# joejep/FOCNeRF

Hardware: AMD Instinct MI355X
Metric: train_samples_per_sec (higher is better)
Workload: dtype f16

## Files before the change

### focnerf_amd/backend.py

```python
import math

import torch

from . import _lib
from ._lib import lib, ptr, stream_of, check, require_cuda, dtype_code, raw_stream


def _f32(*ts):
    for t in ts:
        if t is not None and t.dtype != torch.float32:
            raise RuntimeError(f"focnerf_amd: expected float32 tensor, got {t.dtype}")


def _contig(*ts):
    for t in ts:
        if t is not None and not t.is_contiguous():
            raise RuntimeError("focnerf_amd: tensor must be contiguous")


class _Scratch:

    def __init__(self):
        self._bufs = {}
        self._pinned = []
# ... 66 lines not shown
                                                   ptr(image), stream_of(sigmas)), "composite_rays_train_forward")

    @staticmethod
    def composite_rays_train_backward(grad_weights_sum, grad_image, sigmas, rgbs, deltas, rays, weights_sum, image, M, N, T_thresh, grad_sigmas, grad_rgbs):
        ts = (grad_weights_sum, grad_image, sigmas, rgbs, deltas, weights_sum, image, grad_sigmas, grad_rgbs)
        require_cuda(*ts, rays); _f32(*ts); _contig(*ts, rays)
        check(lib.foc_composite_rays_train_backward(ptr(grad_weights_sum), ptr(grad_image), ptr(sigmas), ptr(rgbs), ptr(deltas), ptr(rays),
                                                    ptr(weights_sum), ptr(image), M, N, T_thresh, ptr(grad_sigmas), ptr(grad_rgbs),
                                                    stream_of(sigmas)), "composite_rays_train_backward")

    @staticmethod
    def march_rays(n_alive, n_step, rays_alive, rays_t, rays_o, rays_d, bound, dt_gamma, max_steps, C, H, grid, nears, fars, xyzs, dirs, deltas, noises):
        ts = (rays_t, rays_o, rays_d, nears, fars, xyzs, dirs, deltas, noises)
        require_cuda(*ts, rays_alive, grid); _f32(*ts); _contig(*ts, rays_alive, grid)
        check(lib.foc_march_rays(n_alive, n_step, ptr(rays_alive), ptr(rays_t), ptr(rays_o), ptr(rays_d), bound, dt_gamma, max_steps, C, H,
                                 ptr(grid), ptr(nears), ptr(fars), ptr(xyzs), ptr(dirs), ptr(deltas), ptr(noises), stream_of(rays_o)), "march_rays")

    @staticmethod
    def composite_rays(n_alive, n_step, T_thresh, rays_alive, rays_t, sigmas, rgbs, deltas, weights_sum, depth, image):
        ts = (rays_t, sigmas, rgbs, deltas, weights_sum, depth, image)
        require_cuda(*ts, rays_alive); _f32(*ts); _contig(*ts, rays_alive)
        check(lib.foc_composite_rays(n_alive, n_step, T_thresh, ptr(rays_alive), ptr(rays_t), ptr(sigmas), ptr(rgbs), ptr(deltas),
                                     ptr(weights_sum), ptr(depth), ptr(image), stream_of(sigmas)), "composite_rays")

    @staticmethod
    def compact_alive(rays_alive, n_alive, out, n_out):
        require_cuda(rays_alive, out, n_out)
        scratch = _scratch.get("compact", 4 * (n_alive // 1024 + 2), rays_alive.device)
        check(lib.foc_compact_alive(ptr(rays_alive), n_alive, ptr(out), ptr(n_out), ptr(scratch), stream_of(rays_alive)), "compact_alive")


class _gridencoder:
    @staticmethod
    def _common(inputs, embeddings, offsets):
        require_cuda(inputs, embeddings, offsets)
        _contig(inputs, embeddings, offsets)
        if inputs.dtype != torch.float32:
            raise RuntimeError("inputs must be a float32 tensor")
        if offsets.dtype != torch.int32:
            raise RuntimeError("offsets must be an int tensor")

    @staticmethod
    def grid_encode_forward(inputs, embeddings, offsets, outputs, B, D, C, L, S, H, dy_dx, gridtype, align_corners, interp, out_bl=False):
        _gridencoder._common(inputs, embeddings, offsets)
        require_cuda(outputs, dy_dx); _contig(outputs, dy_dx)
        dt = dtype_code(embeddings)
        if outputs.dtype != embeddings.dtype or (dy_dx is not None and dy_dx.dtype != embeddings.dtype):
            raise RuntimeError("grid_encode_forward: outputs/dy_dx must share the embeddings dtype")
        fn = lib.foc_grid_encode_forward_bl if out_bl else lib.foc_grid_encode_forward
        check(fn(ptr(inputs), ptr(embeddings), ptr(offsets), ptr(outputs), B, D, C, L, float(S), H, ptr(dy_dx), gridtype, int(bool(align_corners)),
                 interp, dt, None, stream_of(inputs)), "grid_encode_forward")

    @staticmethod
    def planes_to_rows(planes, rows, B, L, unit_bytes):
        require_cuda(planes, rows); _contig(planes, rows)
        check(lib.foc_grid_planes_to_rows(ptr(planes), ptr(rows), B, L, unit_bytes, stream_of(planes)), "grid_planes_to_rows")

    @staticmethod
    def rows_to_planes(rows, planes, B, L, unit_bytes):
        require_cuda(planes, rows); _contig(planes, rows)
        check(lib.foc_grid_rows_to_planes(ptr(rows), ptr(planes), B, L, unit_bytes, stream_of(rows)), "grid_rows_to_planes")

    @staticmethod
    def _host_entry(offsets):
        h = getattr(offsets, "_foc_host", None)
        if h is None or h[0] != offsets._version:
            import ctypes
            arr = offsets.detach().cpu().numpy().astype("int32")
            h = (offsets._version, arr, arr.ctypes.data_as(ctypes.c_void_p), int((arr[1:] - arr[:-1]).max()) if arr.size > 1 else 0)
            offsets._foc_host = h
        return h

    @staticmethod
    def _host_offsets(offsets):
        return _gridencoder._host_entry(offsets)[2]

    @staticmethod
    def _binned_ok(offsets, S, H, L, gridtype):
        finest = math.ceil(2.0 ** (float(S) * (L - 1)) * H - 1.0) + 1
        return gridtype == 0 and finest <= 8190 and _gridencoder._host_entry(offsets)[3] <= 8192 * 64

    _pre = {}

    @staticmethod
    def _pre_state(device):
        idx = device.index if device.index is not None else torch.cuda.current_device()
        st = _gridencoder._pre.get(idx)
        if st is None:
            st = _gridencoder._pre[idx] = dict(ticket=0, key=None)
        return idx, st

    @staticmethod
    def _invalidate_precount(device):
        _, st = _gridencoder._pre_state(device)
        st["ticket"] += 1
        st["key"] = None

    @staticmethod
    def binned_workspace_bytes(offsets, B, D, C, L, S, H, gridtype, dt, count_ahead=False):
        import os
        if os.environ.get("FOCNERF_GRID_ATOMIC", "0") == "1" or (count_ahead and (B == 0 or os.environ.get("FOC_GRID_PRECOUNT", "1") == "0")):
            return 0
        ws_bytes = lib.foc_grid_encode_backward_workspace_bytes(B, D, C, L, dt)
        if not ws_bytes or B * 8 * L >= 2 ** 32 or not _gridencoder._binned_ok(offsets, S, H, L, gridtype):
            return 0
        return ws_bytes

    @staticmethod
    def precount_standalone():
        import os
        return os.environ.get("FOC_GRID_PRECOUNT", "1") == "2"

    @staticmethod
    def _precount_key(inputs, B, L, dt, ws):
        return (inputs.data_ptr(), B, L, dt, ws.data_ptr())

    @staticmethod
    def issue_precount_ticket(inputs, B, L, dt, ws):
        idx, st = _gridencoder._pre_state(inputs.device)
        st["ticket"] += 1
        st["key"] = _gridencoder._precount_key(inputs, B, L, dt, ws)
        return (idx, st["ticket"], st["key"])

    @staticmethod
    def grid_encode_forward_counted(inputs, embeddings, offsets, outputs, B, D, C, L, S, H, gridtype, align_corners, interp, standalone=False):
        _gridencoder._common(inputs, embeddings, offsets)
        require_cuda(outputs); _contig(outputs)
        dt = dtype_code(embeddings)
        ws_bytes = _gridencoder.binned_workspace_bytes(offsets, B, D, C, L, S, H, gridtype, dt, count_ahead=True)
        if not ws_bytes:
            return None
        if outputs.dtype != embeddings.dtype or outputs.numel() != L * B * C:
            raise RuntimeError("grid_encode_forward_counted: outputs must be [L,B,C] of the embeddings' dtype")
        ws = _scratch.get("grid_bwd", ws_bytes, inputs.device)
        host = _gridencoder._host_offsets(offsets)
        if standalone:
            check(lib.foc_grid_encode_backward_count(ptr(inputs), ptr(offsets), B, D, C, L, float(S), H, gridtype, int(bool(align_corners)), interp, dt,
                                                     host, ptr(ws), ws_bytes, stream_of(inputs)), "grid_encode_backward_count")
            check(lib.foc_grid_encode_forward(ptr(inputs), ptr(embeddings), ptr(offsets), ptr(outputs), B, D, C, L, float(S), H, None, gridtype,
                                              int(bool(align_corners)), interp, dt, None, stream_of(inputs)), "grid_encode_forward")
        else:
            check(lib.foc_grid_encode_forward_counted(ptr(inputs), ptr(embeddings), ptr(offsets), ptr(outputs), B, D, C, L, float(S), H, gridtype,
                                                      int(bool(align_corners)), interp, dt, host, ptr(ws), ws_bytes, stream_of(inputs)),
                  "grid_encode_forward_counted")
        return _gridencoder.issue_precount_ticket(inputs, B, L, dt, ws)

    @staticmethod
    def _precount_valid(ticket, inputs, B, L, dt, ws):
        if ticket is None:
            return False
        idx, number, key = ticket
        st = _gridencoder._pre.get(idx)
        return st is not None and st["ticket"] == number and st["key"] == key == _gridencoder._precount_key(inputs, B, L, dt, ws)

    @staticmethod
    def grid_encode_backward(grad, inputs, embeddings, offsets, grad_embeddings, B, D, C, L, S, H, dy_dx, grad_inputs, gridtype, align_corners, interp, grad_bl=False,
                             precount=None):
        _gridencoder._common(inputs, embeddings, offsets)
        require_cuda(grad, grad_embeddings, dy_dx, grad_inputs); _contig(grad, grad_embeddings, dy_dx, grad_inputs)
        dt = dtype_code(grad)
        if grad_embeddings.dtype != grad.dtype:
            raise RuntimeError("grid_encode_backward: grad_embeddings must share grad's dtype")
        ws_bytes = _gridencoder.binned_workspace_bytes(offsets, B, D, C, L, S, H, gridtype, dt)
        if ws_bytes:
            ws = _scratch.get("grid_bwd", ws_bytes, grad.device)
            counted = _gridencoder._precount_valid(precount, inputs, B, L, dt, ws)
            fn = lib.foc_grid_encode_backward_binned_counted if counted else lib.foc_grid_encode_backward_binned
            check(fn(ptr(grad), ptr(inputs), ptr(embeddings), ptr(offsets), ptr(grad_embeddings), B, D, C, L, float(S), H,
                     ptr(dy_dx), ptr(grad_inputs), gridtype, int(bool(align_corners)), interp, dt, int(bool(grad_bl)),
                     _gridencoder._host_offsets(offsets), ptr(ws), ws_bytes, stream_of(inputs)), "grid_encode_backward_binned")
            _gridencoder._invalidate_precount(grad.device)
            return
        check(lib.foc_grid_encode_backward(ptr(grad), ptr(inputs), ptr(embeddings), ptr(offsets), ptr(grad_embeddings), B, D, C, L, float(S), H,
                                           ptr(dy_dx), ptr(grad_inputs), gridtype, int(bool(align_corners)), interp, dt, int(bool(grad_bl)),
                                           None, stream_of(inputs)), "grid_encode_backward")

    @staticmethod
    def grad_total_variation(inputs, embeddings, grad, offsets, weight, B, D, C, L, S, H, gridtype, align_corners):
        require_cuda(inputs, embeddings, grad, offsets); _contig(inputs, embeddings, grad, offsets)
        dt = dtype_code(embeddings)
        if inputs.dtype != embeddings.dtype or grad.dtype != embeddings.dtype:
            raise RuntimeError("grad_total_variation: inputs/grad must share the embeddings dtype")
        check(lib.foc_grad_total_variation(ptr(inputs), ptr(embeddings), ptr(grad), ptr(offsets), weight, B, D, C, L, float(S), H, gridtype,
                                           int(bool(align_corners)), dt, stream_of(inputs)), "grad_total_variation")


class _freqencoder:
    @staticmethod
    def freq_encode_forward(inputs, B, D, deg, C, outputs):
        require_cuda(inputs, outputs); _f32(inputs, outputs); _contig(inputs, outputs)
        check(lib.foc_freq_encode_forward(ptr(inputs), B, D, deg, C, ptr(outputs), stream_of(inputs)), "freq_encode_forward")

    @staticmethod
    def freq_encode_backward(grad, outputs, B, D, deg, C, grad_inputs):
        require_cuda(grad, outputs, grad_inputs); _f32(grad, outputs, grad_inputs); _contig(grad, outputs, grad_inputs)
        check(lib.foc_freq_encode_backward(ptr(grad), ptr(outputs), B, D, deg, C, ptr(grad_inputs), stream_of(grad)), "freq_encode_backward")


def _half(*ts):
    for t in ts:
        if t is not None and t.dtype != torch.float16:
            raise RuntimeError("focnerf_amd: tensor must be a half tensor")


class _ffmlp:
    @staticmethod
    def ffmlp_forward(inputs, weights, B, input_dim, output_dim, hidden_dim, num_layers, activation, output_activation, forward_buffer, outputs):
        require_cuda(inputs, weights, forward_buffer, outputs); _half(inputs, weights, forward_buffer, outputs); _contig(inputs, weights, forward_buffer, outputs)
        check(lib.foc_ffmlp_forward(ptr(inputs), ptr(weights), B, input_dim, output_dim, hidden_dim, num_layers, activation, output_activation,
                                    ptr(forward_buffer), ptr(outputs), stream_of(inputs)), "ffmlp_forward")

    @staticmethod
    def ffmlp_inference(inputs, weights, B, input_dim, output_dim, hidden_dim, num_layers, activation, output_activation, inference_buffer, outputs):
        require_cuda(inputs, weights, outputs); _half(inputs, weights, outputs); _contig(inputs, weights, outputs)
        check(lib.foc_ffmlp_inference(ptr(inputs), ptr(weights), B, input_dim, output_dim, hidden_dim, num_layers, activation, output_activation,
                                      ptr(inference_buffer), ptr(outputs), stream_of(inputs)), "ffmlp_inference")

    @staticmethod
    def ffmlp_backward(grad, inputs, weights, forward_buffer, B, input_dim, output_dim, hidden_dim, num_layers, activation, output_activation,
                       calc_grad_inputs, backward_buffer, grad_inputs, grad_weights):
        ts = (grad, inputs, weights, forward_buffer, backward_buffer, grad_inputs, grad_weights)
        require_cuda(*ts); _half(*ts); _contig(*ts)
        ws_bytes = lib.foc_ffmlp_backward_workspace_bytes(input_dim, hidden_dim, num_layers)
        ws = _scratch.get("ffmlp_ws", ws_bytes, grad.device)
        check(lib.foc_ffmlp_backward(ptr(grad), ptr(inputs), ptr(weights), ptr(forward_buffer), B, input_dim, output_dim, hidden_dim, num_layers,
                                     activation, output_activation, int(bool(calc_grad_inputs)), ptr(backward_buffer), ptr(grad_inputs),
                                     ptr(grad_weights), ptr(ws), ws.numel(), stream_of(grad)), "ffmlp_backward")

    @staticmethod
    def ffmlp_forward_planar(inputs_planar, weights, B, input_dim, output_dim, hidden_dim, num_layers, activation, output_activation, outputs):
        require_cuda(inputs_planar, weights, outputs); _half(inputs_planar, weights, outputs); _contig(inputs_planar, weights, outputs)
        check(lib.foc_ffmlp_forward_planar(ptr(inputs_planar), ptr(weights), B, input_dim, output_dim, hidden_dim, num_layers, activation,
                                           output_activation, ptr(outputs), stream_of(inputs_planar)), "ffmlp_forward_planar")

    @staticmethod
    def ffmlp_backward_planar(grad, inputs_planar, weights, B, input_dim, output_dim, hidden_dim, num_layers, activation, output_activation,
                              calc_grad_inputs, grad_inputs_planar, grad_weights):
        ts = (grad, inputs_planar, weights, grad_inputs_planar, grad_weights)
        require_cuda(*ts); _half(*ts); _contig(*ts)
        ws = _scratch.get("ffmlp_ws", lib.foc_ffmlp_backward_workspace_bytes(input_dim, hidden_dim, num_layers), grad.device)
        check(lib.foc_ffmlp_backward_planar(ptr(grad), ptr(inputs_planar), ptr(weights), B, input_dim, output_dim, hidden_dim, num_layers,
                                            activation, output_activation, int(bool(calc_grad_inputs)), ptr(grad_inputs_planar),
                                            ptr(grad_weights), ptr(ws), ws.numel(), stream_of(grad)), "ffmlp_backward_planar")

    @staticmethod
    def allocate_splitk(size):
        check(lib.foc_allocate_splitk(int(size)), "allocate_splitk")

    @staticmethod
    def free_splitk():
        check(lib.foc_free_splitk(), "free_splitk")
```

### focnerf_amd/csrc/fixedstep.hip

```cpp
#include "common.h"
#include "fs_common.h"
#include <float.h>

__global__ void __launch_bounds__(256) k_fs_sample(const float *__restrict__ rays_o, const float *__restrict__ rays_d, const float *__restrict__ nears,
                                                   const float *__restrict__ fars, const float *__restrict__ aabb, const float *__restrict__ noise,
                                                   uint32_t N, uint32_t T, float bound, float *__restrict__ xyzs, float *__restrict__ enc_in,
                                                   _Float16 *__restrict__ ray_sh, uint32_t ray_block) {
    const uint64_t total = ray_block ? (uint64_t)((N + FS_RAY_BLOCK - 1) / FS_RAY_BLOCK) * FS_RAY_BLOCK * T : (uint64_t)N * T;
    const FsBox box = fs_box(aabb);
    const float two_b = 2 * bound;
    for (uint64_t s = (uint64_t)blockIdx.x * 256 + threadIdx.x; s < total; s += (uint64_t)gridDim.x * 256) {
        uint32_t n, i;
        bool own = true;
        if (ray_block) {
            const uint32_t blk = (uint32_t)(s / ((uint64_t)FS_RAY_BLOCK * T)), in = (uint32_t)(s - (uint64_t)blk * FS_RAY_BLOCK * T);
            i = in / FS_RAY_BLOCK;
            n = blk * FS_RAY_BLOCK + in % FS_RAY_BLOCK;
            own = n < N;
            n = own ? n : N - 1;
        } else {
            n = (uint32_t)(s / T); i = (uint32_t)(s - (uint64_t)n * T);
        }
        const FsGeom g = fs_geom(nears, fars, n, T);
        const float z = fs_z(g, i, T, noise, (uint64_t)n * T + i);
        float x, y, w;
        fs_point(rays_o[n * 3], rays_o[n * 3 + 1], rays_o[n * 3 + 2], rays_d[n * 3], rays_d[n * 3 + 1], rays_d[n * 3 + 2], z, box, x, y, w);
        if (xyzs) { xyzs[s * 3] = x; xyzs[s * 3 + 1] = y; xyzs[s * 3 + 2] = w; }
        if (enc_in) { enc_in[s * 3] = fs_norm(x, bound, two_b); enc_in[s * 3 + 1] = fs_norm(y, bound, two_b); enc_in[s * 3 + 2] = fs_norm(w, bound, two_b); }
        if (ray_sh && i == 0 && own) {
            h8 lo, hi;
            foc_sh16_h(rays_d[n * 3], rays_d[n * 3 + 1], rays_d[n * 3 + 2], lo, hi);
            h8 *dst = reinterpret_cast<h8 *>(ray_sh + (uint64_t)n * 16);
            dst[0] = lo; dst[1] = hi;
        }
    }
}

__global__ void __launch_bounds__(256) k_fs_head_fwd(const _Float16 *__restrict__ h, const float *__restrict__ rays_d, const float *__restrict__ nears,
                                                     const float *__restrict__ fars, const float *__restrict__ noise, uint32_t N, uint32_t T,
                                                     float density_scale, float *__restrict__ sigma_out, float *__restrict__ trans_out,
                                                     float *__restrict__ weights_out, float *__restrict__ weights_sum, float *__restrict__ depth,
                                                     _Float16 *__restrict__ cin, const _Float16 *__restrict__ obj, uint32_t cin_ld) {
    const uint32_t lane = threadIdx.x & 63;
    const uint32_t n = blockIdx.x * 4 + (threadIdx.x >> 6);
    if (n >= N) return;
    const FsGeom g = fs_geom(nears, fars, n, T);
    h8 shlo, shhi;
    h8 ob1 = {0, 0, 0, 0, 0, 0, 0, 0}, ob2 = {0, 0, 0, 0, 0, 0, 0, 0};
    _Float16 ob0 = (_Float16)0;
    if (cin) {
        foc_sh16_h(rays_d[n * 3], rays_d[n * 3 + 1], rays_d[n * 3 + 2], shlo, shhi);
        if (obj) {
            ob0 = obj[0];
#pragma unroll
            for (int k = 0; k < 8; k++) ob1[k] = obj[1 + k];
#pragma unroll
            for (int k = 0; k < 7; k++) ob2[k] = obj[9 + k];
        }
    }
    float Tc = 1.0f, ws = 0, dp = 0;
    for (uint32_t base = 0; base < T; base += 64) {
        const uint32_t i = base + lane;
        const bool valid = i < T;
        const uint64_t s = (uint64_t)n * T + (valid ? i : T - 1);
        h8 r0, r1;
        if (cin) { r0 = *reinterpret_cast<const h8 *>(h + s * 16); r1 = *reinterpret_cast<const h8 *>(h + s * 16 + 8); }
        else r0[0] = h[s * 16];
        const float sigma = expf((float)r0[0]);
        const FsSample p = fs_sample_ld(g, i, valid ? i : T - 1, T, noise, s);
        const float alpha = valid ? 1 - expf((-p.delta * density_scale) * sigma) : 0.0f;
        const float om = valid ? (1 - alpha + 1e-15f) : 1.0f;
        const float Tb = fs_trans_scan(om, lane, Tc);
        const float w = alpha * Tb;
        if (valid) {
            sigma_out[s] = sigma; trans_out[s] = Tb; weights_out[s] = w;
            ws += w; dp += w * p.oz;
            if (cin) {
                h8 c2, c3;
#pragma unroll
                for (int k = 0; k < 7; k++) { c2[k] = r0[k + 1]; c3[k] = r1[k + 1]; }
                c2[7] = r1[0]; c3[7] = ob0;
                h8 *dst = reinterpret_cast<h8 *>(cin + s * cin_ld);
                dst[0] = shlo; dst[1] = shhi; dst[2] = c2; dst[3] = c3;
                if (cin_ld == 48) { dst[4] = ob1; dst[5] = ob2; }
            }
        }
    }
    ws = wave_sum(ws); dp = wave_sum(dp);
    if (lane == 0) { weights_sum[n] = ws; depth[n] = dp; }
}

__global__ void __launch_bounds__(256) k_fs_head_bwd(const _Float16 *__restrict__ h, const float *__restrict__ sigma_in, const float *__restrict__ trans_in,
                                                     const float *__restrict__ nears, const float *__restrict__ fars, const float *__restrict__ noise,
                                                     const float *__restrict__ grad_w, const float *__restrict__ grad_ws, const float *__restrict__ grad_depth,
                                                     const _Float16 *__restrict__ grad_cin, uint32_t N, uint32_t T, float density_scale,
                                                     _Float16 *__restrict__ grad_h, uint32_t cin_ld) {
    const uint32_t lane = threadIdx.x & 63;
    const uint32_t n = blockIdx.x * 4 + (threadIdx.x >> 6);
    if (n >= N) return;
    const FsGeom g = fs_geom(nears, fars, n, T);
    const float gws = grad_ws ? grad_ws[n] : 0.0f, gdp = grad_depth ? grad_depth[n] : 0.0f;
    float S_carry = 0.0f;
    const uint32_t n_chunks = (T + 63) / 64;
    for (uint32_t cidx = n_chunks; cidx-- > 0;) {
        const uint32_t i = cidx * 64 + lane;
        const bool valid = i < T;
        const uint64_t s = (uint64_t)n * T + (valid ? i : T - 1);
        const float sigma = sigma_in[s], Tb = trans_in[s];
        const FsSample p = fs_sample_ld(g, i, valid ? i : T - 1, T, noise, s);
        const float dsigma = fs_head_bwd_step(p, valid, sigma, Tb, (grad_w ? grad_w[s] : 0.0f) + gws, gdp, density_scale, lane, S_carry);
        const float dh0 = dsigma * foc_trunc_exp_bwd((float)h[s * 16]);
        if (valid) {
            h8 o0, o1;
            if (grad_cin) {
                const h8 c2 = *reinterpret_cast<const h8 *>(grad_cin + s * cin_ld + 16), c3 = *reinterpret_cast<const h8 *>(grad_cin + s * cin_ld + 24);
#pragma unroll
                for (int k = 0; k < 7; k++) { o0[k + 1] = c2[k]; o1[k + 1] = c3[k]; }
// ... 206 lines not shown
    const uint32_t n0 = blockIdx.x * FS_BLK_RAYS;
    const uint64_t row0 = fs_block_row(n0, 0, T);
    const bool is_s = tid < 256;
    const uint32_t li = is_s ? tid : tid - 256;
    const uint32_t l_step = is_s ? li >> 2 : li / 12, l_part = is_s ? (li & 3) : li % 12;
    const float *src = is_s ? sigma_in + row0 + l_part * 4 : rgb_in + row0 * 3 + l_part * 4;
    const uint32_t src_ld = is_s ? FS_RAY_BLOCK : FS_RAY_BLOCK * 3;
    float *dst = is_s ? &tile_s[l_step][l_part * 4] : &tile_c[l_step][l_part * 4];
    float4 nx = make_float4(0, 0, 0, 0);
    if (l_step < T) nx = *reinterpret_cast<const float4 *>(src + (uint64_t)l_step * src_ld);
    const uint32_t n = n0 + wv;
    const bool own = n < N;
    const FsGeom g = fs_geom(nears, fars, own ? n : N - 1, T);
    FsRayAcc a = {1.0f, 0, 0, 0, 0, 0};
    for (uint32_t base = 0; base < T; base += 64) {
        dst[0] = nx.x; dst[1] = nx.y; dst[2] = nx.z; dst[3] = nx.w;
        __syncthreads();
        if (base + 64 + l_step < T) nx = *reinterpret_cast<const float4 *>(src + (uint64_t)(base + 64 + l_step) * src_ld);
        if (own)
            fs_infer_tile<PACK>(a, g, n, base + lane, lane, T, tile_s[lane][wv], tile_c[lane][wv * 3], tile_c[lane][wv * 3 + 1], tile_c[lane][wv * 3 + 2],
                                noise, density_scale, thresh, rgb_masked, field4, sigma_rm);
        __syncthreads();
    }
    if (own) fs_infer_finish<PACK>(a, n, lane, bg_ray, bg_scalar, image, depth, weights_sum);
}

struct VtState { uint32_t count, first_enc, bad, pad; };

__device__ __forceinline__ bool vt_turn(const float *__restrict__ d, uint32_t i) {
    const float ax = d[(i + 1) * 3] - d[i * 3], ay = d[(i + 1) * 3 + 1] - d[i * 3 + 1], az = d[(i + 1) * 3 + 2] - d[i * 3 + 2];
    const float bx = d[(i + 2) * 3] - d[(i + 1) * 3], by = d[(i + 2) * 3 + 1] - d[(i + 1) * 3 + 1], bz = d[(i + 2) * 3 + 2] - d[(i + 1) * 3 + 2];
    return (bx * ax + by * ay) + bz * az < 0.0f;
}

__global__ void __launch_bounds__(256) k_vt_find(const float *__restrict__ d, uint32_t N, VtState *__restrict__ st) {
    for (uint32_t i = blockIdx.x * 256 + threadIdx.x; i + 2 < N; i += gridDim.x * 256)
        if (vt_turn(d, i)) { atomicAdd(&st->count, 1u); atomicMax(&st->first_enc, N - i); }
}

__global__ void __launch_bounds__(256) k_vt_check(const float *__restrict__ d, uint32_t N, VtState *__restrict__ st) {
    const uint32_t fe = st->first_enc;
    if (fe == 0u) return;
    const uint32_t W = N - fe + 2u;
    for (uint32_t i = blockIdx.x * 256 + threadIdx.x; i + 2 < N; i += gridDim.x * 256) {
        const bool expect = (i + 2u) % W == 0u || (i + 1u) % W == 0u;
        if (vt_turn(d, i) != expect) st->bad = 1u;
    }
}

__global__ void __launch_bounds__(256) k_vt_perm(uint32_t N, uint32_t th, uint32_t tw, const VtState *__restrict__ st, int64_t *__restrict__ perm) {
    const uint32_t fe = st->first_enc, W = fe ? N - fe + 2u : 0u;
    const uint32_t H = W ? N / W : 0u;
    const bool grid = W >= 16u && N % W == 0u && H >= 8u && st->count == 2u * (H - 1u) && st->bad == 0u;
    for (uint32_t p = blockIdx.x * 256 + threadIdx.x; p < N; p += gridDim.x * 256) {
        uint32_t src = p;
        if (grid) {
            const uint64_t wt = (uint64_t)W * th;
            const uint32_t ty = (uint32_t)(p / wt), rem = (uint32_t)(p - ty * wt);
            const uint32_t rows_here = min(th, H - ty * th);
            const uint32_t tx = min(rem / (rows_here * tw), (W - 1u) / tw), r2 = rem - tx * rows_here * tw;
            const uint32_t cols_here = min(tw, W - tx * tw);
            src = (ty * th + r2 / cols_here) * W + tx * tw + r2 % cols_here;
        }
        perm[p] = (int64_t)src;
    }
}

extern "C" {

int foc_fixed_sample(const float *rays_o, const float *rays_d, const float *nears, const float *fars, const float *aabb, const float *noise,
                     uint32_t N, uint32_t T, float bound, float *xyzs, float *enc_in, void *ray_sh, uint32_t ray_block, void *stream) {
    FocDeviceGuard foc_guard_(stream, rays_o);
    if (N == 0) return FOC_OK;
    FOC_REQUIRE(rays_o && rays_d && nears && fars && aabb && (xyzs || enc_in), FOC_E_INVALID, "fixed_sample: null pointer");
    FOC_REQUIRE(T >= 2, FOC_E_INVALID, "fixed_sample: T must be >= 2");
    FOC_REQUIRE(ray_block == 0 || ray_block == FS_RAY_BLOCK, FOC_E_INVALID, "fixed_sample: ray_block must be 0 (ray-major) or %u (got %u)", FS_RAY_BLOCK, ray_block);
    const uint64_t rows = ray_block ? (uint64_t)foc_div_up(N, FS_RAY_BLOCK) * FS_RAY_BLOCK * T : (uint64_t)N * T;
    hipLaunchKernelGGL(k_fs_sample, dim3(foc_grid_1d(rows, 256, 256 * 16)), dim3(256), 0, (hipStream_t)stream, rays_o, rays_d, nears, fars, aabb,
                       noise, N, T, bound, xyzs, enc_in, (_Float16 *)ray_sh, ray_block);
    FOC_CHECK_LAUNCH("fixed_sample");
    return FOC_OK;
}

int foc_fixed_head_forward(const void *h, const float *rays_d, const float *nears, const float *fars, const float *noise, uint32_t N, uint32_t T,
                           float density_scale, float *sigma, float *trans, float *weights, float *weights_sum, float *depth, void *cin,
                           const void *obj_feat, uint32_t cin_width, void *stream) {
    FocDeviceGuard foc_guard_(stream, h);
    if (N == 0) return FOC_OK;
    FOC_REQUIRE(h && rays_d && nears && fars && sigma && trans && weights && weights_sum && depth, FOC_E_INVALID, "fixed_head_forward: null pointer");
    FOC_REQUIRE(T >= 2, FOC_E_INVALID, "fixed_head_forward: T must be >= 2");
    FOC_REQUIRE(cin_width == 32 || cin_width == 48, FOC_E_INVALID, "fixed_head_forward: cin_width must be 32 or 48 (got %u)", cin_width);
    FOC_REQUIRE(!obj_feat || cin_width == 48, FOC_E_INVALID, "fixed_head_forward: an object feature needs the 48-wide colour input");
    hipLaunchKernelGGL(k_fs_head_fwd, dim3(foc_div_up(N, 4)), dim3(256), 0, (hipStream_t)stream, (const _Float16 *)h, rays_d, nears, fars, noise, N, T,
                       density_scale, sigma, trans, weights, weights_sum, depth, (_Float16 *)cin, (const _Float16 *)obj_feat, cin_width);
    FOC_CHECK_LAUNCH("fixed_head_forward");
    return FOC_OK;
}

int foc_fixed_head_backward(const void *h, const float *sigma, const float *trans, const float *nears, const float *fars, const float *noise,
                            const float *grad_w, const float *grad_ws, const float *grad_depth, const void *grad_cin, uint32_t N, uint32_t T,
                            float density_scale, void *grad_h, uint32_t cin_width, void *stream) {
    FocDeviceGuard foc_guard_(stream, h);
    if (N == 0) return FOC_OK;
    FOC_REQUIRE(h && sigma && trans && nears && fars && grad_h, FOC_E_INVALID, "fixed_head_backward: null pointer");
    FOC_REQUIRE(T >= 2, FOC_E_INVALID, "fixed_head_backward: T must be >= 2");
    FOC_REQUIRE(cin_width == 32 || cin_width == 48, FOC_E_INVALID, "fixed_head_backward: cin_width must be 32 or 48 (got %u)", cin_width);
    hipLaunchKernelGGL(k_fs_head_bwd, dim3(foc_div_up(N, 4)), dim3(256), 0, (hipStream_t)stream, (const _Float16 *)h, sigma, trans, nears, fars, noise,
                       grad_w, grad_ws, grad_depth, (const _Float16 *)grad_cin, N, T, density_scale, (_Float16 *)grad_h, cin_width);
    FOC_CHECK_LAUNCH("fixed_head_backward");
    return FOC_OK;
}

int foc_fixed_composite_forward(const void *c, const float *weights, const float *bg_ray, float bg_scalar, uint32_t N, uint32_t T, float thresh,
                                float *image, void *stream) {
    FocDeviceGuard foc_guard_(stream, c);
    if (N == 0) return FOC_OK;
    FOC_REQUIRE(c && weights && image, FOC_E_INVALID, "fixed_composite_forward: null pointer");
    hipLaunchKernelGGL(k_fs_composite_fwd, dim3(foc_div_up(N, 4)), dim3(256), 0, (hipStream_t)stream, (const _Float16 *)c, weights, bg_ray, bg_scalar, N, T,
                       thresh, image);
    FOC_CHECK_LAUNCH("fixed_composite_forward");
    return FOC_OK;
}

int foc_fixed_composite_backward(const float *grad_image, const void *c, const float *weights, const float *bg_ray, float bg_scalar, uint32_t N,
                                 uint32_t T, float thresh, void *grad_c, float *grad_w, void *stream) {
    FocDeviceGuard foc_guard_(stream, grad_image);
    if (N == 0) return FOC_OK;
    FOC_REQUIRE(grad_image && c && weights && grad_c && grad_w, FOC_E_INVALID, "fixed_composite_backward: null pointer");
    hipLaunchKernelGGL(k_fs_composite_bwd, dim3(foc_grid_1d((uint64_t)N * T, 256, 256 * 16)), dim3(256), 0, (hipStream_t)stream, grad_image,
                       (const _Float16 *)c, weights, bg_ray, bg_scalar, N, T, thresh, (_Float16 *)grad_c, grad_w);
    FOC_CHECK_LAUNCH("fixed_composite_backward");
    return FOC_OK;
}

static int fixed_tail_forward(const char *who, const void *h, const void *c, const float *nears, const float *fars, const float *noise, const float *bg_ray,
                              float bg_scalar, uint32_t N, uint32_t T, float density_scale, float thresh, float *sigma, float *trans, float *weights,
                              float *weights_sum, float *depth, float *image, uint32_t c_width, float *ray_sumsq, float *ray_dist, float *ray_wm, void *stream) {
    FocDeviceGuard foc_guard_(stream, h);
    if (N == 0) return FOC_OK;
    FOC_REQUIRE(c_width == 16 || c_width == 4, FOC_E_INVALID, "%s: c_width must be 16 or 4 (got %u)", who, c_width);
    FOC_REQUIRE(h && c && nears && fars && sigma && trans && weights && weights_sum && depth && image, FOC_E_INVALID, "%s: null pointer", who);
    FOC_REQUIRE(T >= 2, FOC_E_INVALID, "%s: T must be >= 2", who);
    auto kern = ray_dist ? (noise ? k_fs_tail_fwd<true, true> : k_fs_tail_fwd<false, true>) : (noise ? k_fs_tail_fwd<true, false> : k_fs_tail_fwd<false, false>);
    hipLaunchKernelGGL(kern, dim3(foc_div_up(N, 4)), dim3(256), 0, (hipStream_t)stream, (const _Float16 *)h, (const _Float16 *)c, nears, fars, noise,
                       bg_ray, bg_scalar, N, T, density_scale, thresh, sigma, trans, weights, weights_sum, depth, image, c_width, ray_sumsq, ray_dist, ray_wm);
    FOC_CHECK_LAUNCH(who);
    return FOC_OK;
}

int foc_fixed_tail_forward(const void *h, const void *c, const float *nears, const float *fars, const float *noise, const float *bg_ray, float bg_scalar,
                           uint32_t N, uint32_t T, float density_scale, float thresh, float *sigma, float *trans, float *weights, float *weights_sum,
                           float *depth, float *image, uint32_t c_width, float *ray_sumsq, void *stream) {
    return fixed_tail_forward("fixed_tail_forward", h, c, nears, fars, noise, bg_ray, bg_scalar, N, T, density_scale, thresh, sigma, trans, weights, weights_sum,
                              depth, image, c_width, ray_sumsq, nullptr, nullptr, stream);
}

int foc_fixed_tail_forward_dist(const void *h, const void *c, const float *nears, const float *fars, const float *noise, const float *bg_ray, float bg_scalar,
                                uint32_t N, uint32_t T, float density_scale, float thresh, float *sigma, float *trans, float *weights, float *weights_sum,
                                float *depth, float *image, uint32_t c_width, float *ray_sumsq, float *ray_dist, float *ray_wm, void *stream) {
    FOC_REQUIRE((ray_dist && ray_wm) || N == 0, FOC_E_INVALID, "fixed_tail_forward_dist: null ray_dist / ray_wm");
    return fixed_tail_forward("fixed_tail_forward_dist", h, c, nears, fars, noise, bg_ray, bg_scalar, N, T, density_scale, thresh, sigma, trans, weights,
                              weights_sum, depth, image, c_width, ray_sumsq, ray_dist, ray_wm, stream);
}

static int fixed_tail_backward(const char *who, const float *grad_image, const float *grad_ws, const float *grad_depth, const void *c, const float *sigma,
                               const float *trans, const float *weights, const float *nears, const float *fars, const float *noise, const float *bg_ray,
// ... 99 lines not shown
```

### focnerf_amd/csrc/fs_common.h

```cpp
#pragma once
#include "common.h"
#include "sample_math.h"

struct FsGeom { float near, far, span, sample_dist, step; };

#define FS_RAY_BLOCK 64u
__host__ __device__ __forceinline__ uint64_t fs_block_row(uint32_t n, uint32_t i, uint32_t T) {
    return (uint64_t)(n / FS_RAY_BLOCK) * FS_RAY_BLOCK * T + (uint64_t)i * FS_RAY_BLOCK + n % FS_RAY_BLOCK;
}

__device__ __forceinline__ FsGeom fs_geom(const float *__restrict__ nears, const float *__restrict__ fars, uint32_t n, uint32_t T) {
    FsGeom g;
    g.near = nears[n]; g.far = fars[n];
    g.span = g.far - g.near;
    g.sample_dist = g.span / (float)T;
    g.step = 1.0f / (float)(T - 1);
    return g;
}
__device__ __forceinline__ float fs_z0(const FsGeom &g, uint32_t i, uint32_t T) {
    const float lin = (i < T / 2) ? (g.step * (float)i) : fmaf(-g.step, (float)(T - 1 - i), 1.0f);
    return g.near + g.span * lin;
}
__device__ __forceinline__ float fs_jitter(const FsGeom &g, float z, float u) { return z + (u - 0.5f) * g.sample_dist; }
__device__ __forceinline__ float fs_z(const FsGeom &g, uint32_t i, uint32_t T, const float *__restrict__ noise, uint64_t s) {
    float z = fs_z0(g, i, T);
    if (noise) z = fs_jitter(g, z, noise[s]);
    return z;
}
__device__ __forceinline__ float fs_zu(const FsGeom &g, uint32_t i, uint32_t T, bool jitter, float u) {
    float z = fs_z0(g, i, T);
    if (jitter) z = fs_jitter(g, z, u);
    return z;
}

struct FsSample { float z, delta, oz; };
__device__ __forceinline__ FsSample fs_sample(const FsGeom &g, uint32_t i, uint32_t ic, uint32_t T, bool jitter, float u0, float u1) {
    FsSample p;
    p.z = fs_zu(g, ic, T, jitter, u0);
    p.delta = g.sample_dist;
    if (i + 1 < T) p.delta = fs_zu(g, i + 1, T, jitter, u1) - p.z;
    p.oz = (p.z - g.near) / g.span;
    p.oz = p.oz < 0.0f ? 0.0f : (p.oz > 1.0f ? 1.0f : p.oz);
    return p;
}
__device__ __forceinline__ FsSample fs_sample_ld(const FsGeom &g, uint32_t i, uint32_t ic, uint32_t T, const float *__restrict__ noise, uint64_t s) {
    const bool jitter = noise != nullptr;
    return fs_sample(g, i, ic, T, jitter, jitter ? noise[s] : 0.0f, jitter && i + 1 < T ? noise[s + 1] : 0.0f);
}

__device__ __forceinline__ float fs_trans_scan(float om, uint32_t lane, float &Tc) {
    float P;
    const float Tb = Tc * wave_prod_scan(om, lane, P);
    Tc *= __shfl(P, 63, 64);
    return Tb;
}

__device__ __forceinline__ float wave_suffix_incl_sum(float v, int lane) {
#pragma unroll
    for (int o = 1; o < 64; o <<= 1) {
        const float u = __shfl_down(v, o, 64);
        if (lane + o < 64) v += u;
    }
    return v;
}
__device__ __forceinline__ float fs_head_bwd_step(const FsSample &p, bool valid, float sigma, float Tb, float gi, float gdp, float density_scale, uint32_t lane,
                                                  float &S_carry) {
    const float ex = expf((-p.delta * density_scale) * sigma);
    const float alpha = 1 - ex;
    const float om = 1 - alpha + 1e-15f;
    if (gdp != 0.0f) gi += gdp * p.oz;
    const float gw_i = valid ? gi * (alpha * Tb) : 0.0f;
    const float incl = wave_suffix_incl_sum(gw_i, (int)lane);
    const float S_i = S_carry + (incl - gw_i);
    const float dalpha = gi * Tb - S_i / om;
    S_carry += __shfl(incl, 0, 64);
    return dalpha * (p.delta * density_scale) * ex;
}

struct FsDist { float W, WM, acc; };
__device__ __forceinline__ float fs_dist_m(const FsGeom &g, const FsSample &p) { return (p.z - g.near) + 0.5f * p.delta; }
__device__ __forceinline__ void fs_dist_fwd_step(FsDist &d, float w, float m, float delta, uint32_t lane) {
    const float wm = w * m;
    const float iw = wave_incl_sum(w, (int)lane), iwm = wave_incl_sum(wm, (int)lane);
    float ew = __shfl_up(iw, 1, 64), ewm = __shfl_up(iwm, 1, 64);
    if (lane == 0) { ew = 0.0f; ewm = 0.0f; }
    const float Wb = d.W + ew, WMb = d.WM + ewm;
    d.acc += (1.0f / 3.0f) * delta * (w * w) + 2.0f * (w * (m * Wb - WMb));
    d.W += __shfl(iw, 63, 64); d.WM += __shfl(iwm, 63, 64);
}
__device__ __forceinline__ float fs_dist_bwd_step(FsDist &d, float w, float m, float delta, float W_total, float WM_total, uint32_t lane) {
    const float wm = w * m;
    const float iw = wave_suffix_incl_sum(w, (int)lane), iwm = wave_suffix_incl_sum(wm, (int)lane);
    float ew = __shfl_down(iw, 1, 64), ewm = __shfl_down(iwm, 1, 64);
    if (lane == 63) { ew = 0.0f; ewm = 0.0f; }
    const float Wa = d.W + ew, WMa = d.WM + ewm;
    const float Wb = (W_total - Wa) - w, WMb = (WM_total - WMa) - wm;
    d.W += __shfl(iw, 0, 64); d.WM += __shfl(iwm, 0, 64);
    return (2.0f / 3.0f) * delta * w + 2.0f * (m * (Wb - Wa) + (WMa - WMb));
}

// ... 52 lines not shown
```

### focnerf_amd/csrc/gridencoder.hip

```cpp
#include "common.h"
#include <math.h>
#include <stdlib.h>

#include "ge_common.h"

#define GB_SEG_SHIFT 13u
#define GB_SEG (1u << GB_SEG_SHIFT)
#define GB_MAX_SEGS 64u
#define GB_CHUNK 32768u

struct GbHeader {
    uint32_t counts[GE_MAX_LEVELS * GB_MAX_SEGS];
    uint32_t base[GE_MAX_LEVELS * GB_MAX_SEGS + 1];
    uint32_t cursor[GE_MAX_LEVELS * GB_MAX_SEGS];
    uint32_t chunk_prefix[GE_MAX_LEVELS * GB_MAX_SEGS + 1];
};

struct GbSizes { uint32_t size[GE_MAX_LEVELS]; };

template <typename T> struct GbRec;
template <> struct GbRec<__half> { static constexpr uint32_t bytes = 8; };
template <> struct GbRec<float> { static constexpr uint32_t bytes = 12; };

__device__ __forceinline__ void gb_weighted_grads(const uint32_t (&pg)[3], const float (&pf)[3], float g0, float g1, float (&pv)[16]) {
    float ws[8];
#pragma unroll
    for (uint32_t i = 0; i < 8; i++) {
        float w = 1;
        uint32_t pgl[3];
        ge_corner(GeDimCT<3>(), i, pf, pg, w, pgl);
        ws[i] = w;
    }
#pragma unroll
    for (int i = 0; i < 8; i++) { pv[2 * i] = ws[i] * g0; pv[2 * i + 1] = ws[i] * g1; }
}

#define GB_MERGE_MAX_RES 480u
template <int CTRL>
__device__ __forceinline__ uint32_t gb_dpp(uint32_t v) { return (uint32_t)__builtin_amdgcn_update_dpp(0, (int)v, CTRL, 0xf, 0xf, true); }
struct GbRun { uint32_t f0, f1, f2, f3; float k0, k1, k2, k3; bool tail; };
__device__ __forceinline__ GbRun gb_run_flags(bool inside, const uint32_t (&pos_grid)[3]) {
    const uint32_t r = threadIdx.x & 15u;
    const uint32_t key = inside ? (pos_grid[0] | (pos_grid[1] << 10) | (pos_grid[2] << 20)) : 0xFFFFFFFFu;
    const uint32_t prev = gb_dpp<0x111>(key);
    const uint32_t head = (r == 0u || key != prev || !inside) ? 1u : 0u;
    GbRun run;
    run.f0 = head;
    run.f1 = run.f0 | gb_dpp<0x111>(run.f0);
    run.f2 = run.f1 | gb_dpp<0x112>(run.f1);
    run.f3 = run.f2 | gb_dpp<0x114>(run.f2);
    const uint32_t next_head = gb_dpp<0x101>(head);
    run.tail = inside && (r == 15u || next_head != 0u);
    run.k0 = run.f0 ? 0.0f : 1.0f; run.k1 = run.f1 ? 0.0f : 1.0f; run.k2 = run.f2 ? 0.0f : 1.0f; run.k3 = run.f3 ? 0.0f : 1.0f;
    return run;
}
__device__ __forceinline__ float gb_run_sum(float v, const GbRun &run) {
    float u;
#ifdef FOC_GB_MERGE_SELECT
    u = __uint_as_float(gb_dpp<0x111>(__float_as_uint(v))); v = run.f0 ? v : v + u;
    u = __uint_as_float(gb_dpp<0x112>(__float_as_uint(v))); v = run.f1 ? v : v + u;
    u = __uint_as_float(gb_dpp<0x114>(__float_as_uint(v))); v = run.f2 ? v : v + u;
    u = __uint_as_float(gb_dpp<0x118>(__float_as_uint(v))); v = run.f3 ? v : v + u;
#else
    u = __uint_as_float(gb_dpp<0x111>(__float_as_uint(v))); v = fmaf(u, run.k0, v);
    u = __uint_as_float(gb_dpp<0x112>(__float_as_uint(v))); v = fmaf(u, run.k1, v);
    u = __uint_as_float(gb_dpp<0x114>(__float_as_uint(v))); v = fmaf(u, run.k2, v);
    u = __uint_as_float(gb_dpp<0x118>(__float_as_uint(v))); v = fmaf(u, run.k3, v);
#endif
    return v;
}
#ifndef FOC_GB_MERGE_SELECT
#define GB_FMAC16(CTRL)                                                                                                                  \
    asm volatile("s_nop 1\n\t"                                                                                                           \
                 "v_fmac_f32_dpp %0, %0, %16 " CTRL " row_mask:0xf bank_mask:0xf bound_ctrl:1\n\t"                                       \
                 "v_fmac_f32_dpp %1, %1, %16 " CTRL " row_mask:0xf bank_mask:0xf bound_ctrl:1\n\t"                                       \
                 "v_fmac_f32_dpp %2, %2, %16 " CTRL " row_mask:0xf bank_mask:0xf bound_ctrl:1\n\t"                                       \
                 "v_fmac_f32_dpp %3, %3, %16 " CTRL " row_mask:0xf bank_mask:0xf bound_ctrl:1\n\t"                                       \
                 "v_fmac_f32_dpp %4, %4, %16 " CTRL " row_mask:0xf bank_mask:0xf bound_ctrl:1\n\t"                                       \
                 "v_fmac_f32_dpp %5, %5, %16 " CTRL " row_mask:0xf bank_mask:0xf bound_ctrl:1\n\t"                                       \
                 "v_fmac_f32_dpp %6, %6, %16 " CTRL " row_mask:0xf bank_mask:0xf bound_ctrl:1\n\t"                                       \
                 "v_fmac_f32_dpp %7, %7, %16 " CTRL " row_mask:0xf bank_mask:0xf bound_ctrl:1\n\t"                                       \
                 "v_fmac_f32_dpp %8, %8, %16 " CTRL " row_mask:0xf bank_mask:0xf bound_ctrl:1\n\t"                                       \
                 "v_fmac_f32_dpp %9, %9, %16 " CTRL " row_mask:0xf bank_mask:0xf bound_ctrl:1\n\t"                                       \
                 "v_fmac_f32_dpp %10, %10, %16 " CTRL " row_mask:0xf bank_mask:0xf bound_ctrl:1\n\t"                                     \
                 "v_fmac_f32_dpp %11, %11, %16 " CTRL " row_mask:0xf bank_mask:0xf bound_ctrl:1\n\t"                                     \
                 "v_fmac_f32_dpp %12, %12, %16 " CTRL " row_mask:0xf bank_mask:0xf bound_ctrl:1\n\t"                                     \
                 "v_fmac_f32_dpp %13, %13, %16 " CTRL " row_mask:0xf bank_mask:0xf bound_ctrl:1\n\t"                                     \
                 "v_fmac_f32_dpp %14, %14, %16 " CTRL " row_mask:0xf bank_mask:0xf bound_ctrl:1\n\t"                                     \
                 "v_fmac_f32_dpp %15, %15, %16 " CTRL " row_mask:0xf bank_mask:0xf bound_ctrl:1"                                          \
                 : "+v"(v[0]), "+v"(v[1]), "+v"(v[2]), "+v"(v[3]), "+v"(v[4]), "+v"(v[5]), "+v"(v[6]), "+v"(v[7]), "+v"(v[8]), "+v"(v[9]),   \
                   "+v"(v[10]), "+v"(v[11]), "+v"(v[12]), "+v"(v[13]), "+v"(v[14]), "+v"(v[15])                                           \
                 : "v"(k))
#endif
__device__ __forceinline__ void gb_run_sum16(float (&v)[16], const GbRun &run) {
#ifdef FOC_GB_MERGE_SELECT
#pragma unroll
    for (int i = 0; i < 16; i++) v[i] = gb_run_sum(v[i], run);
#else
    float k;
    if (__builtin_amdgcn_ballot_w64(run.f0 == 0u) != 0ull) {
        k = run.k0; GB_FMAC16("row_shr:1");
        if (__builtin_amdgcn_ballot_w64(run.f1 == 0u) != 0ull) {
            k = run.k1; GB_FMAC16("row_shr:2");
            if (__builtin_amdgcn_ballot_w64(run.f2 == 0u) != 0ull) {
                k = run.k2; GB_FMAC16("row_shr:4");
                if (__builtin_amdgcn_ballot_w64(run.f3 == 0u) != 0ull) { k = run.k3; GB_FMAC16("row_shr:8"); }
            }
        }
    }
#endif
}

#define GB_PM_TILE 1024u
#define GB_PMS_WG 1024u

__global__ void __launch_bounds__(256) k_gbin_scans(GbHeader *__restrict__ hdr, uint32_t *__restrict__ wg_hist, uint32_t n_wg, uint32_t L) {
    __shared__ uint32_t s_wave[2][4];
    const uint32_t lane = threadIdx.x & 63, wave = threadIdx.x >> 6;
    const uint32_t n = L * GB_MAX_SEGS;
    if (blockIdx.x == n) {
        const uint32_t per = (n + 255) / 256;
        const uint32_t lo = threadIdx.x * per, hi = min(n, lo + per);
        uint32_t recs = 0, chks = 0;
        for (uint32_t i = lo; i < hi; i++) { const uint32_t c = hdr->counts[i]; recs += c; chks += (c + GB_CHUNK - 1) / GB_CHUNK; }
        const uint32_t ir = (uint32_t)wave_incl_sum_i((int)recs, (int)lane), ic = (uint32_t)wave_incl_sum_i((int)chks, (int)lane);
        if (lane == 63) { s_wave[0][wave] = ir; s_wave[1][wave] = ic; }
        __syncthreads();
        uint32_t r = ir - recs, k = ic - chks;
        for (uint32_t w = 0; w < wave; w++) { r += s_wave[0][w]; k += s_wave[1][w]; }
        for (uint32_t i = lo; i < hi; i++) {
            const uint32_t c = hdr->counts[i];
            hdr->base[i] = r; hdr->chunk_prefix[i] = k;
            r += c; k += (c + GB_CHUNK - 1) / GB_CHUNK;
        }
        if (threadIdx.x == 255) { hdr->base[n] = r; hdr->chunk_prefix[n] = k; }
        return;
    }
    const uint32_t slot = blockIdx.x;
    uint32_t *col = wg_hist + (uint64_t)slot * n_wg;
    const uint32_t per = (n_wg + 255) / 256;
    const uint32_t lo = min(n_wg, threadIdx.x * per), hi = min(n_wg, lo + per);
    uint32_t local = 0;
    for (uint32_t i = lo; i < hi; i++) local += col[i];
    const uint32_t incl = (uint32_t)wave_incl_sum_i((int)local, (int)lane);
    if (lane == 63) s_wave[0][wave] = incl;
    __syncthreads();
    uint32_t run = incl - local;
    for (uint32_t k = 0; k < wave; k++) run += s_wave[0][k];
    for (uint32_t i = lo; i < hi; i++) { const uint32_t c = col[i]; col[i] = run; run += c; }
}

template <uint32_t THREADS>
__device__ __forceinline__ void gb_count_tile(uint32_t *hist, uint32_t tile, uint32_t n_wg, const float *__restrict__ inputs, const int32_t *__restrict__ offsets,
                                              GbHeader *__restrict__ hdr, uint32_t *__restrict__ wg_hist, uint32_t B, uint32_t L, const GeLevels &lv,
                                              uint32_t gridtype, bool align_corners, uint32_t interp, uint32_t l_begin, uint32_t l_end) {
    static_assert(GB_PM_TILE % THREADS == 0 && THREADS % 64 == 0, "whole waves, whole tile");
    const uint32_t slot_lo = l_begin * GB_MAX_SEGS, slot_hi = l_end * GB_MAX_SEGS;
    for (uint32_t i = slot_lo + threadIdx.x; i < slot_hi; i += THREADS) hist[i] = 0;
    __syncthreads();
    for (uint32_t it = 0; it < GB_PM_TILE / THREADS; it++) {
        const uint32_t b = tile * GB_PM_TILE + it * THREADS + threadIdx.x;
        float x[3] = {0.f, 0.f, 0.f};
        const bool inside = b < B && !ge_load_point(GeDimCT<3>(), inputs, b, x);
        for (uint32_t level = l_begin; level < l_end; level++) {
            const uint32_t resolution = lv.resolution[level];
            uint32_t pg[3]; float pf[3];
            ge_cell(GeDimCT<3>(), x, lv.scale[level], align_corners, interp, pg, pf);
            bool emit = inside;
            if (resolution <= lv.merge_max_res) emit = gb_run_flags(inside, pg).tail;
            if (emit) {
                const uint32_t hashmap_size = (uint32_t)offsets[level + 1] - (uint32_t)offsets[level];
                uint32_t rows[8];
                bool hashed;
                ge_rows3(pg, hashmap_size, resolution, gridtype, align_corners, rows, &hashed);
                if (hashed) {
#pragma unroll
                    for (int j = 0; j < 4; j++) atomicAdd(&hist[level * GB_MAX_SEGS + (rows[2 * j] >> GB_SEG_SHIFT)], 1u);
                } else {
#pragma unroll
                    for (int j = 0; j < 4; j++) {
                        const uint32_t s0 = rows[2 * j] >> GB_SEG_SHIFT, s1 = rows[2 * j + 1] >> GB_SEG_SHIFT;
                        atomicAdd(&hist[level * GB_MAX_SEGS + s0], 1u);
                        if (s0 != s1) atomicAdd(&hist[level * GB_MAX_SEGS + s1], 1u);
                    }
                }
            }
        }
    }
    __syncthreads();
    for (uint32_t i = slot_lo + threadIdx.x; i < slot_hi; i += THREADS) {
        const uint32_t hcount = hist[i];
        if (hcount) (void)__hip_atomic_fetch_add(&hdr->counts[i], hcount, __ATOMIC_RELAXED, __HIP_MEMORY_SCOPE_AGENT);
        wg_hist[(uint64_t)i * n_wg + tile] = hcount;
    }
}

__global__ void __launch_bounds__(GB_PMS_WG) k_gbin_count_pt(const float *__restrict__ inputs, const int32_t *__restrict__ offsets, GbHeader *__restrict__ hdr,
                                                             uint32_t *__restrict__ wg_hist, uint32_t B, uint32_t L, GeLevels lv, uint32_t gridtype,
                                                             bool align_corners, uint32_t interp) {
    __shared__ uint32_t hist[GE_MAX_LEVELS * GB_MAX_SEGS];
    gb_count_tile<GB_PMS_WG>(hist, blockIdx.x, gridDim.x, inputs, offsets, hdr, wg_hist, B, L, lv, gridtype, align_corners, interp, 0u, L);
}

template <typename T>
__global__ void __launch_bounds__(256) k_grid_fwd_counted(const float *__restrict__ inputs, const T *__restrict__ grid, const int32_t *__restrict__ offsets,
                                                          T *__restrict__ outputs, uint32_t B, uint32_t L, GeLevels lv, uint32_t gridtype, bool align_corners,
                                                          uint32_t interp, uint32_t chunks, uint32_t pairs, GbHeader *__restrict__ hdr,
                                                          uint32_t *__restrict__ wg_hist, uint32_t n_tiles, uint32_t period, uint32_t w0, uint32_t lc, uint32_t csplit) {
    __shared__ uint32_t hist[GE_MAX_LEVELS * GB_MAX_SEGS];
    const uint32_t n_count = n_tiles * csplit;
    uint32_t f = blockIdx.x;
    if (blockIdx.x >= w0) {
        const uint32_t g = blockIdx.x - w0, q = g / period, r = g - q * period;
        if (r == period - 1u && q < n_count) {
            const uint32_t part = q % csplit;
            gb_count_tile<256>(hist, q / csplit, n_tiles, inputs, offsets, hdr, wg_hist, B, L, lv, gridtype, align_corners, interp, (part * L) / csplit, ((part + 1u) * L) / csplit);
            return;
        }
        f = blockIdx.x - min(q, n_count);
    }
    uint32_t chunk, l0, l1;
    ge_walk(f, chunks, lc, chunk, l0, l1);
    const uint32_t b = chunk * 256 + threadIdx.x;
    if (l0 >= L || b >= B) return;
    float x[3];
    const bool oob = ge_load_point(GeDimCT<3>(), inputs, b, x);
    for (uint32_t level = l0; level < l1; level++) {
        const uint32_t off0 = (uint32_t)offsets[level];
        const uint32_t hashmap_size = (uint32_t)offsets[level + 1] - off0;
        ge_forward_level<T, GeDimCT<3>, 2>(GeDimCT<3>(), x, oob, grid, off0, hashmap_size, lv.scale[level], lv.resolution[level], outputs + ((uint64_t)level * B + b) * 2,
                                  (T *)nullptr, gridtype, align_corners, interp, pairs);
    }
}

template <typename T>
__global__ void __launch_bounds__(GB_PMS_WG, (sizeof(T) == 2 ? 8 : 4)) k_gbin_scatter_pms(
    const T *__restrict__ grad, const float *__restrict__ inputs, const int32_t *__restrict__ offsets, const GbHeader *__restrict__ hdr,
    const uint32_t *__restrict__ wg_base, void *__restrict__ recs, uint64_t max_recs, uint32_t B, uint32_t L, GeLevels lv, uint32_t gridtype,
    bool align_corners, uint32_t interp, bool grad_bl, uint32_t fact_mask, GbSizes sz, uint32_t n_tiles, uint32_t n_whole, uint32_t split) {
    uint32_t tile = blockIdx.x, l_begin = 0u, l_end = L;
    if (blockIdx.x >= n_whole) {
        const uint32_t r = blockIdx.x - n_whole, part = r % split;
        tile = n_whole + r / split;
        l_begin = (part * L) / split; l_end = ((part + 1u) * L) / split;
    }
    static_assert(GB_PM_TILE == GB_PMS_WG, "one point per thread");
    constexpr uint32_t NREC = GB_PM_TILE * 5u;
    constexpr uint32_t VW = sizeof(T) == 2 ? 1 : 2;
    __shared__ uint32_t cur[2][GB_MAX_SEGS];
    __shared__ uint32_t pre[2][GB_MAX_SEGS + 1];
    __shared__ uint32_t gb[2][GB_MAX_SEGS];
    __shared__ uint32_t s_rows[NREC];
    __shared__ uint32_t s_val[2 * VW][NREC];
    const uint32_t n_wg = n_tiles;
    const uint32_t b = tile * GB_PM_TILE + threadIdx.x;
    float x[3] = {0.f, 0.f, 0.f};
    const bool inside = b < B && !ge_load_point(GeDimCT<3>(), inputs, b, x);
    constexpr uint32_t GW = sizeof(T) == 2 ? 1 : 2;
    __shared__ uint32_t s_grad[2][GW][GB_PM_TILE];
    auto fetch_grad = [&](uint32_t level) {
        if (level < l_end) {
            const uint32_t *gbase = reinterpret_cast<const uint32_t *>(grad);
#pragma unroll 4
            for (uint32_t k = 0; k < GB_PM_TILE / 64u; k++) {
                const uint32_t pt = tile * GB_PM_TILE + k * 64u + threadIdx.x;
                const uint32_t pq = pt < B ? pt : 0u;
                const uint32_t *src = grad_bl ? gbase + ((uint64_t)pq * L + level) * GW : gbase + ((uint64_t)level * B + pq) * GW;
#pragma unroll
                for (uint32_t w = 0; w < GW; w++) {
                    const uint32_t dst = (uint32_t)__builtin_amdgcn_readfirstlane(
                        (int)(uint32_t)(uintptr_t)(__attribute__((address_space(3))) uint32_t *)&s_grad[level & 1u][w][k * 64u]);
                    uint32_t keep;
                    asm volatile("s_mov_b32 %0, m0\n\ts_mov_b32 m0, %2\n\ts_nop 0\n\tglobal_load_lds_dword %1, off\n\ts_mov_b32 m0, %0"
                                 : "=&s"(keep) : "v"(src + w), "s"(dst) : "memory");
                }
            }
        }
    };
    uint32_t nsb = 0, nw0 = 0, nw1 = 0;
    auto fetch_bases = [&](uint32_t level) {
        if (threadIdx.x < GB_MAX_SEGS && level < l_end) {
            const uint32_t slot = level * GB_MAX_SEGS + threadIdx.x;
            const uint32_t sb = hdr->base[slot];
            const uint32_t wi = slot * n_wg + tile;
            nsb = sb;
            nw0 = wg_base[wi];
            nw1 = *(tile + 1 < n_wg ? &wg_base[wi + 1u] : &hdr->counts[slot]);
        }
    };
    auto setup_tables = [&](uint32_t pbn) {
        const uint32_t nb0 = nsb + nw0;
        const uint32_t hc = nw1 - nw0;
        const uint32_t incl = (uint32_t)wave_incl_sum_i((int)hc, (int)threadIdx.x);
        pre[pbn][threadIdx.x] = incl - hc;
        cur[pbn][threadIdx.x] = incl - hc;
        gb[pbn][threadIdx.x] = nb0 - (incl - hc);
        if (threadIdx.x == GB_MAX_SEGS - 1) pre[pbn][GB_MAX_SEGS] = incl;
    };
    fetch_bases(l_begin);
    if (threadIdx.x < GB_MAX_SEGS) { if (l_begin < l_end) setup_tables(l_begin & 1u); fetch_bases(l_begin + 1u); fetch_grad(l_begin); }
    for (uint32_t level_v = l_begin; level_v < l_end; level_v++) {
        {
        const uint32_t level = (uint32_t)__builtin_amdgcn_readfirstlane((int)level_v);
        const uint32_t pb = level & 1u;
        if (threadIdx.x < GB_MAX_SEGS) __builtin_amdgcn_s_waitcnt(0x0F70);
        foc_lds_barrier();
        if (threadIdx.x < GB_MAX_SEGS && level + 1u < l_end) { setup_tables(pb ^ 1u); fetch_bases(level + 2u); fetch_grad(level + 1u); }
        float g[2];
        if constexpr (sizeof(T) == 2) {
            const uint32_t gw = s_grad[pb][0][threadIdx.x];
            g[0] = __half2float(__ushort_as_half((unsigned short)(gw & 0xFFFFu)));
            g[1] = __half2float(__ushort_as_half((unsigned short)(gw >> 16)));
        } else {
            g[0] = __uint_as_float(s_grad[pb][0][threadIdx.x]); g[1] = __uint_as_float(s_grad[pb][GW - 1][threadIdx.x]);
        }
        if (!inside) { g[0] = 0.0f; g[1] = 0.0f; }
        const bool fact = sizeof(T) == 2 && ((fact_mask >> level) & 1u) != 0u;
        if (fact) {
            uint32_t pg[3]; float pf[3];
            ge_cell(GeDimCT<3>(), x, lv.scale[level], align_corners, interp, pg, pf);
            if (inside) {
                const uint32_t mask = sz.size[level] - 1u;
                const uint32_t ty0 = pg[1] * 2654435761u, ty1 = ty0 + 2654435761u, tz0 = pg[2] * 805459861u, tz1 = tz0 + 805459861u;
                const uint32_t jb = (uint32_t)__builtin_ctz(~pg[0]);
                const uint32_t fxq = min((uint32_t)rintf(pf[0] * 32768.0f), 32767u);
                const uint32_t meta = (jb << 13) | (fxq << 17);
#pragma unroll 1
                for (int j = 0; j < 4; j++) {
                    const uint32_t row = (pg[0] ^ ((j & 1) ? ty1 : ty0) ^ ((j >> 1) ? tz1 : tz0)) & mask;
                    const float w = ((j & 1) ? pf[1] : 1 - pf[1]) * ((j >> 1) ? pf[2] : 1 - pf[2]);
                    typedef _Float16 gb_h2 __attribute__((ext_vector_type(2)));
                    const gb_h2 hv = {(_Float16)ge_opaque(w * g[0]), (_Float16)ge_opaque(w * g[1])};
                    const uint32_t seg = row >> GB_SEG_SHIFT;
                    const uint32_t pos = atomicAdd(&cur[pb][seg], 1u);
                    if (pos < NREC) {
                        s_rows[pos] = (row & (GB_SEG - 1u)) | meta;
                        s_val[0][pos] = *reinterpret_cast<const uint32_t *>(&hv);
                        s_val[VW][pos] = seg;
                    }
                }
            }
        } else {
            const uint32_t resolution = lv.resolution[level];
            uint32_t pg[3]; float pf[3];
            ge_cell(GeDimCT<3>(), x, lv.scale[level], align_corners, interp, pg, pf);
            uint32_t pv0[8], pv1[8];
            bool emit = inside;
            float pv[16];
            gb_weighted_grads(pg, pf, g[0], g[1], pv);
            if (resolution <= lv.merge_max_res) {
                const GbRun run = gb_run_flags(inside, pg);
                emit = run.tail;
                gb_run_sum16(pv, run);
            }
#pragma unroll
            for (int i = 0; i < 8; i++) {
                const float v0 = pv[2 * i], v1 = pv[2 * i + 1];
                if constexpr (sizeof(T) == 2) {
                    typedef _Float16 gb_h2 __attribute__((ext_vector_type(2)));
                    const gb_h2 hv = {(_Float16)ge_opaque(v0), (_Float16)ge_opaque(v1)};
                    pv0[i] = *reinterpret_cast<const uint32_t *>(&hv);
                } else { pv0[i] = __float_as_uint(v0); pv1[i] = __float_as_uint(v1); }
            }
            if (emit) {
                const uint32_t hashmap_size = sz.size[level];
                uint32_t rows[8];
                bool hashed;
                ge_rows3(pg, hashmap_size, resolution, gridtype, align_corners, rows, &hashed);
                auto place = [&](uint32_t seg, uint32_t r0, uint32_t r1, int i0, int i1) {
                    const uint32_t pos = atomicAdd(&cur[pb][seg], 1u);
                    if (pos >= NREC) return;
                    s_rows[pos] = (r0 & (GB_SEG - 1u)) | ((r1 & (GB_SEG - 1u)) << 13) | (seg << 26);
                    s_val[0][pos] = pv0[i0];
                    s_val[VW][pos] = i1 >= 0 ? pv0[i1 >= 0 ? i1 : 0] : 0u;
                    if constexpr (sizeof(T) != 2) { s_val[1][pos] = pv1[i0]; s_val[VW + 1][pos] = i1 >= 0 ? pv1[i1 >= 0 ? i1 : 0] : 0u; }
                };
                if (hashed) {
#pragma unroll
                    for (int j = 0; j < 4; j++) place(rows[2 * j] >> GB_SEG_SHIFT, rows[2 * j], rows[2 * j + 1], 2 * j, 2 * j + 1);
                } else {
#pragma unroll
                    for (int j = 0; j < 4; j++) {
                        const uint32_t r0 = rows[2 * j], r1 = rows[2 * j + 1];
                        const uint32_t s0 = r0 >> GB_SEG_SHIFT, s1 = r1 >> GB_SEG_SHIFT;
                        if (s0 == s1) place(s0, r0, r1, 2 * j, 2 * j + 1);
                        else { place(s0, r0, r0, 2 * j, -1); place(s1, r1, r1, 2 * j + 1, -1); }
                    }
                }
            }
        }
        foc_lds_barrier();
        const uint32_t total = min(pre[pb][GB_MAX_SEGS], NREC);
        uint32_t *rec_rows = reinterpret_cast<uint32_t *>(recs);
        uint32_t *rec_vals = rec_rows + ((max_recs + 3) & ~(uint64_t)3);
        if (fact) {
            if constexpr (sizeof(T) == 2) {
                for (uint32_t j = threadIdx.x - 64u; j < total; j += GB_PMS_WG - 64u) {
                    const uint32_t at = gb[pb][s_val[1][j] & (GB_MAX_SEGS - 1u)] + j;
                    if (at >= max_recs) continue;
                    reinterpret_cast<uint2 *>(rec_vals)[at] = make_uint2(s_rows[j], s_val[0][j]);
                }
            }
        } else
        for (uint32_t j = threadIdx.x - 64u; j < total; j += GB_PMS_WG - 64u) {
            const uint32_t rw = s_rows[j];
            const uint32_t at = gb[pb][rw >> 26] + j;
            if (at >= max_recs) continue;
            rec_rows[at] = rw;
            if constexpr (sizeof(T) == 2) reinterpret_cast<uint2 *>(rec_vals)[at] = make_uint2(s_val[0][j], s_val[1][j]);
            else reinterpret_cast<uint4 *>(rec_vals)[at] = make_uint4(s_val[0][j], s_val[1][j], s_val[2][j], s_val[3][j]);
        }
        }
    }
}

__device__ __forceinline__ unsigned long long gb_half_to_fixed(uint32_t h) {
    const uint32_t e = (h >> 10) & 31u, m = h & 1023u;
    const unsigned long long mag = e ? ((unsigned long long)(1024u | m) << (e - 1u)) : (unsigned long long)m;
    return (h & 0x8000u) ? (0ull - mag) : mag;
}

#define GB_RTHREADS 1024u
template <typename T, int DET>
__global__ void __launch_bounds__(GB_RTHREADS) k_gbin_reduce(const GbHeader *__restrict__ hdr, const void *__restrict__ recs, uint64_t max_recs,
                                                             const int32_t *__restrict__ offsets, T *__restrict__ grad_grid, uint32_t L, uint32_t fact_mask,
                                                             unsigned long long *__restrict__ det_sum, uint32_t *__restrict__ det_bad) {
    __shared__ double acc[GB_SEG * 2];
    unsigned long long *acci = reinterpret_cast<unsigned long long *>(acc);
    __shared__ uint32_t s_bad[GB_SEG / 32];
    __shared__ uint32_t s_slot, s_lo, s_hi, s_multi;
    const uint32_t n = L * GB_MAX_SEGS;
    const uint32_t total_chunks = hdr->chunk_prefix[n];
    const uint32_t chunk_id = blockIdx.x;
    if (chunk_id >= total_chunks) return;
    {
    if (threadIdx.x == 0) { s_slot = 0u; s_lo = 0u; s_hi = 0u; s_multi = 0u; }
    __syncthreads();
    for (uint32_t i = threadIdx.x; i < n; i += GB_RTHREADS) {
        const uint32_t p0 = hdr->chunk_prefix[i], p1 = hdr->chunk_prefix[i + 1];
        const uint32_t cnt = hdr->counts[i];
        const uint64_t b0 = hdr->base[i];
        if (p0 <= chunk_id && chunk_id < p1) {
            const uint32_t c = chunk_id - p0;
            s_slot = i;
            if constexpr (DET != 0) s_multi = p1 - p0 > 1u ? 1u : 0u;
            s_lo = (uint32_t)min(b0 + (uint64_t)c * GB_CHUNK, max_recs);
            s_hi = (uint32_t)min(b0 + min(cnt, (c + 1) * GB_CHUNK), max_recs);
        }
    }
    for (uint32_t i = threadIdx.x; i < GB_SEG * 2; i += GB_RTHREADS) acc[i] = 0.0;
    if (threadIdx.x < GB_SEG / 32) s_bad[threadIdx.x] = 0u;
    __syncthreads();
    const uint32_t slot = s_slot, lo = s_lo, hi = s_hi;
    constexpr uint32_t UNR = 4;
    const uint32_t *rec_rows = reinterpret_cast<const uint32_t *>(recs);
    const uint32_t *rec_vals = rec_rows + ((max_recs + 3) & ~(uint64_t)3);
    constexpr uint32_t NONE = 0xFFFFFFFFu;
    if constexpr (sizeof(T) == 2) {
        const uint2 *vv = reinterpret_cast<const uint2 *>(rec_vals);
        auto fixed = [](float f, uint32_t &wlo, uint32_t &whi) {
            const float sc = f * 16.0f;
            int32_t Hi;
            asm("v_cvt_flr_i32_f32 %0, %1" : "=v"(Hi) : "v"(sc));
            wlo = ((uint32_t)Hi << 20) | (uint32_t)(__builtin_amdgcn_fractf(sc) * 1048576.0f);
            whi = (uint32_t)(Hi >> 12);
        };
        auto add_fast = [&](uint32_t row, uint32_t hv) {
            const __half2 h2 = *reinterpret_cast<const __half2 *>(&hv);
            uint32_t l0, h0, l1, h1;
            fixed(__low2float(h2), l0, h0);
            fixed(__high2float(h2), l1, h1);
            atomicAdd(&acci[row], ((unsigned long long)h0 << 32) | l0);
            atomicAdd(&acci[GB_SEG + row], ((unsigned long long)h1 << 32) | l1);
        };
        auto add_slow = [&](uint32_t row, uint32_t hv) {
            if ((hv & 0x7C00u) == 0x7C00u || (hv & 0x7C000000u) == 0x7C000000u) {
                atomicOr(&s_bad[row >> 5], 1u << (row & 31u));
                return;
            }
            add_fast(row, hv);
        };
        constexpr uint32_t BATCH = GB_RTHREADS * UNR;
        auto pipeline = [&](auto load_full, auto load_tail, auto process) {
            uint32_t cr[UNR], nr[UNR]; uint2 cv[UNR], nv[UNR];
            uint32_t base = lo;
            if (base + BATCH <= hi) load_full(base, cr, cv); else load_tail(base, cr, cv);
            while (base + 3u * BATCH <= hi) {
                load_full(base + BATCH, nr, nv);
                process(cr, cv);
                load_full(base + 2u * BATCH, cr, cv);
                process(nr, nv);
                base += 2u * BATCH;
            }
            while (base + 2u * BATCH <= hi) {
                load_full(base + BATCH, nr, nv);
                process(cr, cv);
#pragma unroll
                for (uint32_t u = 0; u < UNR; u++) { cr[u] = nr[u]; cv[u] = nv[u]; }
                base += BATCH;
            }
            if (base + BATCH < hi) { load_tail(base + BATCH, nr, nv); process(cr, cv); process(nr, nv); }
            else if (base < hi) process(cr, cv);
        };
        if ((fact_mask >> (slot / GB_MAX_SEGS)) & 1u) {
            auto fixedf = [](float f, uint32_t &wlo, uint32_t &whi) {
                const float sc = f * 16.0f;
                int32_t Hi;
                asm("v_cvt_flr_i32_f32 %0, %1" : "=v"(Hi) : "v"(sc));
                wlo = ((uint32_t)Hi << 20) | (uint32_t)(__builtin_amdgcn_fractf(sc) * 1048576.0f);
                whi = (uint32_t)(Hi >> 12);
            };
            auto add2 = [&](uint32_t row, float a, float b) {
                uint32_t l0, h0, l1, h1;
                fixedf(a, l0, h0);
                fixedf(b, l1, h1);
                atomicAdd(&acci[row], ((unsigned long long)h0 << 32) | l0);
                atomicAdd(&acci[GB_SEG + row], ((unsigned long long)h1 << 32) | l1);
            };
            pipeline(
                [&](uint32_t base, uint32_t (&)[UNR], uint2 (&v)[UNR]) {
#pragma unroll
                    for (uint32_t u = 0; u < UNR; u++) v[u] = vv[base + threadIdx.x + u * GB_RTHREADS];
                },
// ... 171 lines not shown
#pragma unroll
        for (uint32_t l = 0; l < GE_MAX_LEVELS; l++) if (l < L) rows[(uint64_t)b * L + l] = v[l];
    }
}

template <typename U>
__global__ void __launch_bounds__(256) k_rows_to_planes(const U *__restrict__ rows, U *__restrict__ planes, uint32_t B, uint32_t L) {
    for (uint32_t b = blockIdx.x * 256 + threadIdx.x; b < B; b += gridDim.x * 256) {
        U v[GE_MAX_LEVELS];
#pragma unroll
        for (uint32_t l = 0; l < GE_MAX_LEVELS; l++) if (l < L) v[l] = rows[(uint64_t)b * L + l];
#pragma unroll
        for (uint32_t l = 0; l < GE_MAX_LEVELS; l++) if (l < L) planes[(uint64_t)l * B + b] = v[l];
    }
}

static int ge_call(GeOp op, const GeCall &a) {
    switch (a.D) {
        case 2: return ge_dispatch<GeDimCT<2>>(op, a);
        case 3: return ge_dispatch<GeDimCT<3>>(op, a);
        case 4: case 5: return ge_nd_dispatch(op, a);
        default: foc_set_error("GridEncoding: D must be 2, 3, 4 or 5 (got %u)", a.D); return FOC_E_INVALID;
    }
}

static int ge_forward(const float *inputs, const void *embeddings, const int32_t *offsets, void *outputs, uint32_t B, uint32_t D,
                      uint32_t C, uint32_t L, float S, uint32_t H, void *dy_dx, uint32_t gridtype, int align_corners, uint32_t interp,
                      int dtype, bool bl, void *stream) {
    if (B == 0) return FOC_OK;
    FOC_REQUIRE(inputs && embeddings && offsets && outputs, FOC_E_INVALID, "grid_encode_forward: null pointer");
    FOC_REQUIRE(dtype == FOC_F32 || dtype == FOC_F16, FOC_E_DTYPE, "grid_encode_forward: dtype must be FOC_F32 or FOC_F16");
    FOC_REQUIRE(L >= 1 && L <= GE_MAX_LEVELS, FOC_E_INVALID, "grid_encode_forward: L must be in [1,%d]", GE_MAX_LEVELS);
    FOC_REQUIRE(gridtype <= 1 && interp <= 1, FOC_E_INVALID, "grid_encode_forward: bad gridtype/interp");
    GeCall a = {};
    a.dtype = dtype; a.D = D; a.C = C; a.B = B; a.L = L; a.gridtype = gridtype; a.interp = interp; a.ac = align_corners != 0; a.bl = bl;
    a.inputs = inputs; a.emb = embeddings; a.offsets = offsets; a.out = outputs; a.dy_dx = dy_dx; a.st = (hipStream_t)stream;
    ge_make_levels(L, S, H, a.lv);
    return ge_call(GE_FORWARD, a);
}


static uint64_t gb_max_recs(uint32_t B, uint32_t L) { return (uint64_t)B * 5u * L; }
static uint64_t gb_rec_array_bytes(uint64_t m, int dtype) { return ((m + 3) & ~(uint64_t)3) * 4 + m * (dtype == FOC_F16 ? 8 : 16); }
static uint32_t gb_max_chunks(uint32_t B, uint32_t L) { return (uint32_t)(((uint64_t)B * 5u * L + GB_CHUNK - 1) / GB_CHUNK) + L * GB_MAX_SEGS; }
static int gb_det_mode(int dtype) {
    const int det = foc_opt(FOC_OPT_DETERMINISTIC);
    return dtype == FOC_F16 && det ? (det == 2 ? 2 : 1) : 0;
}
static uint64_t gb_det_images(uint32_t B, uint32_t L, int det) { return det == 2 ? gb_max_chunks(B, L) : det ? L * GB_MAX_SEGS : 0u; }
static uint64_t gb_base_workspace_bytes(uint32_t B, uint32_t L, int dtype) {
    const uint64_t hdr = (sizeof(GbHeader) + 255) & ~(uint64_t)255;
    const uint64_t m = gb_max_recs(B, L);
    const uint64_t wg = (uint64_t)foc_div_up(B, GB_PM_TILE) * L * GB_MAX_SEGS * 4;
    return (hdr + gb_rec_array_bytes(m, dtype) + 256 + wg + 256 + 255) & ~(uint64_t)255;
}
static uint64_t gb_workspace_bytes(uint32_t B, uint32_t L, int dtype, int det) {
    const uint64_t hdr = (sizeof(GbHeader) + 255) & ~(uint64_t)255;
    const uint64_t m = gb_max_recs(B, L);
    const uint64_t wg = (uint64_t)foc_div_up(B, GB_PM_TILE) * L * GB_MAX_SEGS * 4;
    if (det) return gb_base_workspace_bytes(B, L, dtype) + gb_det_images(B, L, det) * (GB_SEG * 2 * 8 + GB_SEG / 8);
    return hdr + gb_rec_array_bytes(m, dtype) + 256 + wg + 256;
}
static uint64_t gb_recs_bytes(uint32_t B, uint32_t L, int dtype) {
    const uint64_t m = gb_max_recs(B, L);
    return (gb_rec_array_bytes(m, dtype) + 255) & ~(uint64_t)255;
}

static int gb_count(const float *inputs, const int32_t *offsets, uint32_t B, uint32_t L, const GeLevels &lv, uint32_t gridtype, bool ac, uint32_t interp,
                    int dtype, void *workspace, hipStream_t st) {
    GbHeader *hdr = reinterpret_cast<GbHeader *>(workspace);
    void *recs = reinterpret_cast<char *>(workspace) + ((sizeof(GbHeader) + 255) & ~(uint64_t)255);
    if (foc_zero_async(hdr->counts, sizeof(hdr->counts), st) != hipSuccess) { foc_set_error("grid_encode_backward: memset failed"); return FOC_E_LAUNCH; }
    const uint32_t n_wg = foc_div_up(B, GB_PM_TILE);
    uint32_t *wg_hist = reinterpret_cast<uint32_t *>(reinterpret_cast<char *>(recs) + gb_recs_bytes(B, L, dtype));
    hipLaunchKernelGGL(k_gbin_count_pt, dim3(n_wg), dim3(GB_PMS_WG), 0, st, inputs, offsets, hdr, wg_hist, B, L, lv, gridtype, ac, interp);
    FOC_CHECK_LAUNCH("grid_encode_backward(count)");
    hipLaunchKernelGGL(k_gbin_scans, dim3(L * GB_MAX_SEGS + 1), dim3(256), 0, st, hdr, wg_hist, n_wg, L);
    FOC_CHECK_LAUNCH("grid_encode_backward(scans)");
    return FOC_OK;
}

template <typename T>
static int gb_forward_counted(const float *inputs, const void *emb, const int32_t *offsets, void *outputs, uint32_t B, uint32_t L, const GeLevels &lv,
                              uint32_t gridtype, bool ac, uint32_t interp, void *workspace, hipStream_t st) {
    GbHeader *hdr = reinterpret_cast<GbHeader *>(workspace);
    void *recs = reinterpret_cast<char *>(workspace) + ((sizeof(GbHeader) + 255) & ~(uint64_t)255);
    if (foc_zero_async(hdr->counts, sizeof(hdr->counts), st) != hipSuccess) { foc_set_error("grid_encode_forward_counted: memset failed"); return FOC_E_LAUNCH; }
    const uint32_t n_tiles = foc_div_up(B, GB_PM_TILE), chunks = foc_div_up(B, 256);
    const uint32_t lc = ge_small_levels(L, lv);
    const uint32_t groups = lc >= 2u ? L - lc + 1u : L;
    const uint32_t fwd_blocks = chunks * groups;
    const uint32_t lo = groups >= 4 ? groups / 2 : 0, hi = groups >= 4 ? groups - 1 : groups;
    const uint32_t csplit = L >= 4u ? 4u : 1u, n_count = n_tiles * csplit;
    const uint32_t w0 = lo * chunks, fit = ((hi - lo) * chunks) / n_count + 1u, period = (fit & 1u) ? fit : fit - 1u;
    uint32_t *wg_hist = reinterpret_cast<uint32_t *>(reinterpret_cast<char *>(recs) + gb_recs_bytes(B, L, sizeof(T) == 2 ? FOC_F16 : FOC_F32));
    hipLaunchKernelGGL((k_grid_fwd_counted<T>), dim3(fwd_blocks + n_count), dim3(256), 0, st, inputs, (const T *)emb, offsets, (T *)outputs, B, L, lv, gridtype, ac,
                       interp, chunks, sizeof(T) == 2 ? ge_pairs_mode(emb, nullptr, sizeof(T), 3, 2, gridtype, ac, interp) : 0u, hdr, wg_hist, n_tiles, period, w0, lc, csplit);
    FOC_CHECK_LAUNCH("grid_encode_forward_counted");
    hipLaunchKernelGGL(k_gbin_scans, dim3(L * GB_MAX_SEGS + 1), dim3(256), 0, st, hdr, wg_hist, n_tiles, L);
    FOC_CHECK_LAUNCH("grid_encode_forward_counted(scans)");
    return FOC_OK;
}

static uint32_t gb_fact_mask(uint32_t L, const GeLevels &lv, const int32_t *offsets_host, uint32_t gridtype, bool ac, int dtype) {
    const int on = foc_opt(FOC_OPT_GB_FACTORED);
    if (!on || dtype != FOC_F16 || gridtype != 0u) return 0u;
    uint32_t m = 0;
    for (uint32_t l = 0; l < L && l < 32u; l++) {
        const uint32_t size = (uint32_t)(offsets_host[l + 1] - offsets_host[l]);
        const uint32_t r1 = ac ? lv.resolution[l] : lv.resolution[l] + 1u;
        uint32_t stride = 1u;
        for (int d = 0; d < 3; d++) if (stride <= size) stride *= r1;
        const bool hashed = stride > size;
        if (hashed && (size & (size - 1u)) == 0u && size >= GB_SEG && lv.resolution[l] > lv.merge_max_res) m |= 1u << l;
    }
    return m;
}

static uint32_t gb_scatter_resident(size_t elem) { return foc_num_cus() * (elem == 2 ? 2u : 1u); }

template <typename T>
static int gb_run(const void *grad, const float *inputs, const int32_t *offsets, void *grad_emb, uint32_t B, uint32_t L, const GeLevels &lv,
                  uint32_t gridtype, bool ac, uint32_t interp, bool bl, void *workspace, bool counted, uint32_t fact_mask, const GbSizes &sz, int det, hipStream_t st) {
    GbHeader *hdr = reinterpret_cast<GbHeader *>(workspace);
    void *recs = reinterpret_cast<char *>(workspace) + ((sizeof(GbHeader) + 255) & ~(uint64_t)255);
    const uint64_t max_recs = gb_max_recs(B, L);
    const uint32_t n_tiles = foc_div_up(B, GB_PM_TILE);
    uint32_t *wg_hist = reinterpret_cast<uint32_t *>(reinterpret_cast<char *>(recs) + gb_recs_bytes(B, L, sizeof(T) == 2 ? FOC_F16 : FOC_F32));
    if (!counted) {
        const int rc = gb_count(inputs, offsets, B, L, lv, gridtype, ac, interp, sizeof(T) == 2 ? FOC_F16 : FOC_F32, workspace, st);
        if (rc) return rc;
    }
    const uint32_t resident = gb_scatter_resident(sizeof(T));
    const uint32_t n_tail = n_tiles % resident, n_whole = n_tiles - n_tail;
    uint32_t split = 1u;
    const uint32_t split_max = (uint32_t)max(1, foc_opt(FOC_OPT_GB_TAIL_SPLIT));
    while (n_tail && split * 2u <= L && n_tail * split * 2u <= resident && split * 2u <= split_max) split *= 2u;
    hipLaunchKernelGGL((k_gbin_scatter_pms<T>), dim3(n_whole + n_tail * split), dim3(GB_PMS_WG), 0, st, (const T *)grad, inputs, offsets, hdr, wg_hist, recs, max_recs, B, L, lv,
                       gridtype, ac, interp, bl, fact_mask, sz, n_tiles, n_whole, split);
    FOC_CHECK_LAUNCH("grid_encode_backward(scatter)");
    const uint32_t ub = gb_max_chunks(B, L);
    if constexpr (sizeof(T) == 2) {
        if (det) {
            const uint64_t images = gb_det_images(B, L, det);
            unsigned long long *det_sum = reinterpret_cast<unsigned long long *>(reinterpret_cast<char *>(workspace) + gb_base_workspace_bytes(B, L, FOC_F16));
            uint32_t *det_bad = reinterpret_cast<uint32_t *>(det_sum + images * (GB_SEG * 2));
            const uint32_t fin = L * GB_MAX_SEGS * GB_DET_PARTS;
            if (det == 1) {
                hipLaunchKernelGGL(k_gbin_det_zero, dim3(fin), dim3(GB_RTHREADS), 0, st, hdr, det_sum, det_bad, L);
                FOC_CHECK_LAUNCH("grid_encode_backward(deterministic zero)");
                hipLaunchKernelGGL((k_gbin_reduce<T, 1>), dim3(ub), dim3(GB_RTHREADS), 0, st, hdr, recs, max_recs, offsets, (T *)grad_emb, L, fact_mask, det_sum, det_bad);
                FOC_CHECK_LAUNCH("grid_encode_backward(reduce)");
                hipLaunchKernelGGL((k_gbin_det_finish<1>), dim3(fin), dim3(GB_RTHREADS), 0, st, hdr, det_sum, det_bad, ub, offsets, (__half *)grad_emb, L);
            } else {
                hipLaunchKernelGGL((k_gbin_reduce<T, 2>), dim3(ub), dim3(GB_RTHREADS), 0, st, hdr, recs, max_recs, offsets, (T *)grad_emb, L, fact_mask, det_sum, det_bad);
                FOC_CHECK_LAUNCH("grid_encode_backward(reduce)");
                hipLaunchKernelGGL((k_gbin_det_finish<2>), dim3(fin), dim3(GB_RTHREADS), 0, st, hdr, det_sum, det_bad, ub, offsets, (__half *)grad_emb, L);
            }
            FOC_CHECK_LAUNCH("grid_encode_backward(deterministic finish)");
            return FOC_OK;
        }
    }
    hipLaunchKernelGGL((k_gbin_reduce<T, 0>), dim3(ub), dim3(GB_RTHREADS), 0, st, hdr, recs, max_recs, offsets, (T *)grad_emb, L, fact_mask,
                       (unsigned long long *)nullptr, (uint32_t *)nullptr);
    FOC_CHECK_LAUNCH("grid_encode_backward(reduce)");
    return FOC_OK;
}

extern "C" {

// ... 24 lines not shown
int foc_grid_planes_to_rows(const void *planes, void *rows, uint32_t B, uint32_t L, uint32_t unit_bytes, void *stream) {
    FocDeviceGuard foc_guard_(stream, planes);
    if (B == 0) return FOC_OK;
    FOC_REQUIRE(planes && rows, FOC_E_INVALID, "grid_planes_to_rows: null pointer");
    FOC_REQUIRE(L >= 1 && L <= GE_MAX_LEVELS && (unit_bytes == 4 || unit_bytes == 8), FOC_E_INVALID, "grid_planes_to_rows: L in [1,%d], 4- or 8-byte units", GE_MAX_LEVELS);
    hipStream_t st = (hipStream_t)stream;
    if (unit_bytes == 4) hipLaunchKernelGGL((k_planes_to_rows<uint32_t>), dim3(foc_grid_1d(B, 256)), dim3(256), 0, st, (const uint32_t *)planes, (uint32_t *)rows, B, L);
    else hipLaunchKernelGGL((k_planes_to_rows<uint2>), dim3(foc_grid_1d(B, 256)), dim3(256), 0, st, (const uint2 *)planes, (uint2 *)rows, B, L);
    FOC_CHECK_LAUNCH("grid_planes_to_rows");
    return FOC_OK;
}

int foc_grid_rows_to_planes(const void *rows, void *planes, uint32_t B, uint32_t L, uint32_t unit_bytes, void *stream) {
    FocDeviceGuard foc_guard_(stream, rows);
    if (B == 0) return FOC_OK;
    FOC_REQUIRE(planes && rows, FOC_E_INVALID, "grid_rows_to_planes: null pointer");
    FOC_REQUIRE(L >= 1 && L <= GE_MAX_LEVELS && (unit_bytes == 4 || unit_bytes == 8), FOC_E_INVALID, "grid_rows_to_planes: L in [1,%d], 4- or 8-byte units", GE_MAX_LEVELS);
    hipStream_t st = (hipStream_t)stream;
    if (unit_bytes == 4) hipLaunchKernelGGL((k_rows_to_planes<uint32_t>), dim3(foc_grid_1d(B, 256)), dim3(256), 0, st, (const uint32_t *)rows, (uint32_t *)planes, B, L);
    else hipLaunchKernelGGL((k_rows_to_planes<uint2>), dim3(foc_grid_1d(B, 256)), dim3(256), 0, st, (const uint2 *)rows, (uint2 *)planes, B, L);
    FOC_CHECK_LAUNCH("grid_rows_to_planes");
    return FOC_OK;
}

int foc_grid_encode_backward(const void *grad, const float *inputs, const void *embeddings, const int32_t *offsets, void *grad_embeddings,
                             uint32_t B, uint32_t D, uint32_t C, uint32_t L, float S, uint32_t H, const void *dy_dx, void *grad_inputs,
                             uint32_t gridtype, int align_corners, uint32_t interp, int dtype, int grad_is_bl,
                             const int32_t *offsets_host, void *stream) {
    FocDeviceGuard foc_guard_(stream, grad);
    (void)offsets_host; (void)embeddings;
    if (B == 0) return FOC_OK;
    FOC_REQUIRE(grad && inputs && offsets && grad_embeddings, FOC_E_INVALID, "grid_encode_backward: null pointer");
    FOC_REQUIRE(dtype == FOC_F32 || dtype == FOC_F16, FOC_E_DTYPE, "grid_encode_backward: dtype must be FOC_F32 or FOC_F16");
    FOC_REQUIRE(L >= 1 && L <= GE_MAX_LEVELS, FOC_E_INVALID, "grid_encode_backward: L must be in [1,%d]", GE_MAX_LEVELS);
    FOC_REQUIRE(gridtype <= 1 && interp <= 1, FOC_E_INVALID, "grid_encode_backward: bad gridtype/interp");
    FOC_REQUIRE(!foc_opt(FOC_OPT_DETERMINISTIC), FOC_E_INVALID, "grid_encode_backward: FOC_DETERMINISTIC is set and this entry point scatters with float atomics "
                "(arrival order); deterministic mode serves fp16 hash grids with D=3, C=2 through foc_grid_encode_backward_binned");
    GeCall a = {};
    a.dtype = dtype; a.D = D; a.C = C; a.B = B; a.L = L; a.gridtype = gridtype; a.interp = interp; a.ac = align_corners != 0; a.bl = grad_is_bl != 0;
    a.inputs = inputs; a.offsets = offsets; a.out = grad_embeddings; a.grad = grad; a.dy_dx = const_cast<void *>(dy_dx); a.grad_inputs = grad_inputs;
    a.st = (hipStream_t)stream;
    ge_make_levels(L, S, H, a.lv);
    return ge_call(GE_BACKWARD, a);
}

uint64_t foc_grid_encode_backward_workspace_bytes(uint32_t B, uint32_t D, uint32_t C, uint32_t L, int dtype) {
    if (D != 3 || C != 2 || L > GE_MAX_LEVELS) return 0;
    return gb_workspace_bytes(B, L, dtype, gb_det_mode(dtype));
}

static int gb_check(uint32_t B, uint32_t D, uint32_t C, uint32_t L, float S, uint32_t H, uint32_t gridtype, uint32_t interp, int dtype,
                    const int32_t *offsets_host, uint64_t workspace_bytes, int det = 0) {
    FOC_REQUIRE(dtype == FOC_F32 || dtype == FOC_F16, FOC_E_DTYPE, "grid_encode_backward_binned: dtype must be FOC_F32 or FOC_F16");
    FOC_REQUIRE(D == 3 && C == 2, FOC_E_INVALID, "grid_encode_backward_binned: only D=3, C=2 (got D=%u C=%u)", D, C);
    FOC_REQUIRE(L >= 1 && L <= GE_MAX_LEVELS && gridtype <= 1 && interp <= 1, FOC_E_INVALID, "grid_encode_backward_binned: bad L/gridtype/interp");
    FOC_REQUIRE(workspace_bytes >= gb_workspace_bytes(B, L, dtype, det), FOC_E_INVALID, det ? "grid_encode_backward_binned: workspace too small (FOC_DETERMINISTIC adds "
                "the int64 images: foc_grid_encode_backward_workspace_bytes)" : "grid_encode_backward_binned: workspace too small");
    FOC_REQUIRE((uint64_t)B * 8u * L < (1ull << 32), FOC_E_INVALID, "grid_encode_backward_binned: B*8*L must stay below 2^32 records");
    for (uint32_t l = 0; l < L; l++)
        FOC_REQUIRE((uint32_t)(offsets_host[l + 1] - offsets_host[l]) <= GB_SEG * GB_MAX_SEGS, FOC_E_INVALID,
                    "grid_encode_backward_binned: level %u has more than %u rows", l, GB_SEG * GB_MAX_SEGS);
    FOC_REQUIRE(gridtype == 0, FOC_E_INVALID, "grid_encode_backward_binned: hash grids only (gridtype 0); use foc_grid_encode_backward");
    GeLevels lv;
    ge_make_levels(L, S, H, lv);
    for (uint32_t l = 0; l < L; l++)
        FOC_REQUIRE(lv.resolution[l] <= GB_SEG - 2u, FOC_E_INVALID, "grid_encode_backward_binned: level %u has resolution %u (> %u)", l,
                    lv.resolution[l], GB_SEG - 2u);
    return FOC_OK;
}

int foc_grid_encode_backward_count(const float *inputs, const int32_t *offsets, uint32_t B, uint32_t D, uint32_t C, uint32_t L, float S, uint32_t H,
                                   uint32_t gridtype, int align_corners, uint32_t interp, int dtype, const int32_t *offsets_host, void *workspace,
                                   uint64_t workspace_bytes, void *stream) {
    FocDeviceGuard foc_guard_(stream, inputs);
    if (B == 0) return FOC_OK;
    FOC_REQUIRE(inputs && offsets && workspace && offsets_host, FOC_E_INVALID, "grid_encode_backward_count: null pointer");
    const int rc = gb_check(B, D, C, L, S, H, gridtype, interp, dtype, offsets_host, workspace_bytes);
    if (rc) return rc;
    GeLevels lv;
    ge_make_levels(L, S, H, lv);
    return gb_count(inputs, offsets, B, L, lv, gridtype, align_corners != 0, interp, dtype, workspace, (hipStream_t)stream);
}

int foc_grid_encode_forward_counted(const float *inputs, const void *embeddings, const int32_t *offsets, void *outputs, uint32_t B, uint32_t D, uint32_t C,
                                    uint32_t L, float S, uint32_t H, uint32_t gridtype, int align_corners, uint32_t interp, int dtype,
                                    const int32_t *offsets_host, void *workspace, uint64_t workspace_bytes, void *stream) {
    FocDeviceGuard foc_guard_(stream, inputs);
    if (B == 0) return FOC_OK;
    FOC_REQUIRE(inputs && embeddings && offsets && outputs && workspace && offsets_host, FOC_E_INVALID, "grid_encode_forward_counted: null pointer");
    const int rc = gb_check(B, D, C, L, S, H, gridtype, interp, dtype, offsets_host, workspace_bytes);
    if (rc) return rc;
    GeLevels lv;
    ge_make_levels(L, S, H, lv);
    hipStream_t st = (hipStream_t)stream;
    if (dtype == FOC_F32) return gb_forward_counted<float>(inputs, embeddings, offsets, outputs, B, L, lv, gridtype, align_corners != 0, interp, workspace, st);
    return gb_forward_counted<__half>(inputs, embeddings, offsets, outputs, B, L, lv, gridtype, align_corners != 0, interp, workspace, st);
}

static int gb_entry(const void *grad, const float *inputs, const int32_t *offsets, void *grad_embeddings,
                    uint32_t B, uint32_t D, uint32_t C, uint32_t L, float S, uint32_t H, const void *dy_dx, void *grad_inputs,
                    uint32_t gridtype, int align_corners, uint32_t interp, int dtype, int grad_is_bl,
                    const int32_t *offsets_host, void *workspace, uint64_t workspace_bytes, bool counted, void *stream) {
    if (B == 0) return FOC_OK;
    FOC_REQUIRE(grad && inputs && offsets && grad_embeddings && workspace && offsets_host, FOC_E_INVALID, "grid_encode_backward_binned: null pointer");
    const int det_on = foc_opt(FOC_OPT_DETERMINISTIC);
    FOC_REQUIRE(!(det_on && dtype == FOC_F32), FOC_E_INVALID, "grid_encode_backward_binned: FOC_DETERMINISTIC is set and the fp32-table reduce sums in an "
                "order that depends on timing (its LDS sum is a double atomic); deterministic mode serves fp16 tables");
    const int det = dtype == FOC_F16 && det_on ? (det_on == 2 ? 2 : 1) : 0;
    {
        const int rc0 = gb_check(B, D, C, L, S, H, gridtype, interp, dtype, offsets_host, workspace_bytes, det);
        if (rc0) return rc0;
    }
    GeLevels lv;
    ge_make_levels(L, S, H, lv);
    hipStream_t st = (hipStream_t)stream;
    const bool ac = align_corners != 0, bl = grad_is_bl != 0;
    const uint32_t fact_mask = gb_fact_mask(L, lv, offsets_host, gridtype, ac, dtype);
    GbSizes sz;
    for (uint32_t l = 0; l < GE_MAX_LEVELS; l++) sz.size[l] = l < L ? (uint32_t)(offsets_host[l + 1] - offsets_host[l]) : 0u;
    int rc = dtype == FOC_F32 ? gb_run<float>(grad, inputs, offsets, grad_embeddings, B, L, lv, gridtype, ac, interp, bl, workspace, counted, 0u, sz, 0, st)
                              : gb_run<__half>(grad, inputs, offsets, grad_embeddings, B, L, lv, gridtype, ac, interp, bl, workspace, counted, fact_mask, sz, det, st);
    if (rc) return rc;
    if (dy_dx && grad_inputs)
        return dtype == FOC_F32 ? ge_input_backward_launch<float, GeDimCT<3>, 2>(grad, dy_dx, grad_inputs, B, 3u, L, bl, st)
                                : ge_input_backward_launch<__half, GeDimCT<3>, 2>(grad, dy_dx, grad_inputs, B, 3u, L, bl, st);
    return FOC_OK;
}

int foc_grid_encode_backward_binned(const void *grad, const float *inputs, const void *embeddings, const int32_t *offsets, void *grad_embeddings,
                                    uint32_t B, uint32_t D, uint32_t C, uint32_t L, float S, uint32_t H, const void *dy_dx, void *grad_inputs,
                                    uint32_t gridtype, int align_corners, uint32_t interp, int dtype, int grad_is_bl,
                                    const int32_t *offsets_host, void *workspace, uint64_t workspace_bytes, void *stream) {
    FocDeviceGuard foc_guard_(stream, grad);
    (void)embeddings;
    return gb_entry(grad, inputs, offsets, grad_embeddings, B, D, C, L, S, H, dy_dx, grad_inputs, gridtype, align_corners, interp, dtype, grad_is_bl,
                    offsets_host, workspace, workspace_bytes, false, stream);
}

int foc_grid_encode_backward_binned_counted(const void *grad, const float *inputs, const void *embeddings, const int32_t *offsets, void *grad_embeddings,
                                            uint32_t B, uint32_t D, uint32_t C, uint32_t L, float S, uint32_t H, const void *dy_dx, void *grad_inputs,
                                            uint32_t gridtype, int align_corners, uint32_t interp, int dtype, int grad_is_bl,
                                            const int32_t *offsets_host, void *workspace, uint64_t workspace_bytes, void *stream) {
    FocDeviceGuard foc_guard_(stream, grad);
    (void)embeddings;
    return gb_entry(grad, inputs, offsets, grad_embeddings, B, D, C, L, S, H, dy_dx, grad_inputs, gridtype, align_corners, interp, dtype, grad_is_bl,
                    offsets_host, workspace, workspace_bytes, true, stream);
}

int foc_grad_total_variation(const void *inputs, const void *embeddings, void *grad, const int32_t *offsets, float weight, uint32_t B,
                             uint32_t D, uint32_t C, uint32_t L, float S, uint32_t H, uint32_t gridtype, int align_corners, int dtype,
                             void *stream) {
    FocDeviceGuard foc_guard_(stream, inputs);
    if (B == 0) return FOC_OK;
    FOC_REQUIRE(inputs && embeddings && grad && offsets, FOC_E_INVALID, "grad_total_variation: null pointer");
    FOC_REQUIRE(dtype == FOC_F32 || dtype == FOC_F16, FOC_E_DTYPE, "grad_total_variation: dtype must be FOC_F32 or FOC_F16");
    FOC_REQUIRE(L >= 1 && L <= GE_MAX_LEVELS, FOC_E_INVALID, "grad_total_variation: L must be in [1,%d]", GE_MAX_LEVELS);
    FOC_REQUIRE(!foc_opt(FOC_OPT_DETERMINISTIC), FOC_E_INVALID, "grad_total_variation: FOC_DETERMINISTIC is set and this entry point scatters with float atomics (arrival order)");
    GeCall a = {};
    a.dtype = dtype; a.D = D; a.C = C; a.B = B; a.L = L; a.gridtype = gridtype; a.ac = align_corners != 0;
    a.inputs = inputs; a.emb = embeddings; a.offsets = offsets; a.out = grad; a.weight = weight; a.st = (hipStream_t)stream;
    ge_make_levels(L, S, H, a.lv);
    return ge_call(GE_TV, a);
}

}
```

### focnerf_amd/csrc/raymarching.hip

```cpp
#include "common.h"
#include "occ_cell.h"
#include "sample_math.h"
#include "ragged.h"
#include <float.h>

#define RM_SQRT3 1.7320508075688772f
#define RM_RPI   0.3183098861837907f

__device__ __forceinline__ float rm_sign(float x) { return copysignf(1.0f, x); }

__device__ __forceinline__ void rm_near_far(float ox, float oy, float oz, float dx, float dy, float dz, float a0, float a1, float a2, float a3, float a4, float a5,
                                            float min_near, float &near_out, float &far_out) {
    const float rdx = 1 / dx, rdy = 1 / dy, rdz = 1 / dz;
    float near = (a0 - ox) * rdx, far = (a3 - ox) * rdx, t;
    if (near > far) { t = near; near = far; far = t; }
    float near_y = (a1 - oy) * rdy, far_y = (a4 - oy) * rdy;
    if (near_y > far_y) { t = near_y; near_y = far_y; far_y = t; }
    bool miss = (near > far_y || near_y > far);
    if (!miss) {
        if (near_y > near) near = near_y;
        if (far_y < far) far = far_y;
        float near_z = (a2 - oz) * rdz, far_z = (a5 - oz) * rdz;
        if (near_z > far_z) { t = near_z; near_z = far_z; far_z = t; }
        miss = (near > far_z || near_z > far);
        if (!miss) {
            if (near_z > near) near = near_z;
            if (far_z < far) far = far_z;
            if (near < min_near) near = min_near;
        }
    }
    near_out = miss ? FLT_MAX : near;
    far_out = miss ? FLT_MAX : far;
}

__global__ void __launch_bounds__(256) k_near_far_from_aabb(const float *__restrict__ rays_o, const float *__restrict__ rays_d,
                                     const float *__restrict__ aabb, uint32_t N, float min_near,
                                     float *__restrict__ nears, float *__restrict__ fars) {
    const float a0 = aabb[0], a1 = aabb[1], a2 = aabb[2], a3 = aabb[3], a4 = aabb[4], a5 = aabb[5];
    for (uint32_t n = blockIdx.x * blockDim.x + threadIdx.x; n < N; n += gridDim.x * blockDim.x) {
        float near, far;
        rm_near_far(rays_o[n * 3], rays_o[n * 3 + 1], rays_o[n * 3 + 2], rays_d[n * 3], rays_d[n * 3 + 1], rays_d[n * 3 + 2], a0, a1, a2, a3, a4, a5, min_near, near, far);
        nears[n] = near;
        fars[n] = far;
    }
}

__global__ void __launch_bounds__(256) k_sph_from_ray(const float *__restrict__ rays_o, const float *__restrict__ rays_d, float radius,
                               uint32_t N, float *__restrict__ coords) {
    for (uint32_t n = blockIdx.x * blockDim.x + threadIdx.x; n < N; n += gridDim.x * blockDim.x) {
        const float ox = rays_o[n * 3], oy = rays_o[n * 3 + 1], oz = rays_o[n * 3 + 2];
        const float dx = rays_d[n * 3], dy = rays_d[n * 3 + 1], dz = rays_d[n * 3 + 2];
        const float A = fmaf(dz, dz, fmaf(dy, dy, dx * dx));
        const float B = fmaf(oz, dz, fmaf(oy, dy, ox * dx));
        const float C = fmaf(-radius, radius, fmaf(oz, oz, fmaf(oy, oy, ox * ox)));
        const float t = (-B + sqrtf(fmaf(B, B, -(A * C)))) / A;
        const float x = fmaf(t, dx, ox), y = fmaf(t, dy, oy), z = fmaf(t, dz, oz);
        const float theta = atan2f(sqrtf(fmaf(z, z, x * x)), y);
        const float phi = atan2f(z, x);
        coords[n * 2] = fmaf(2 * theta, RM_RPI, -1.0f);
        coords[n * 2 + 1] = phi * RM_RPI;
    }
}

__global__ void __launch_bounds__(256) k_morton3D(const int32_t *__restrict__ coords, uint32_t N, int32_t *__restrict__ indices) {
    for (uint32_t n = blockIdx.x * blockDim.x + threadIdx.x; n < N; n += gridDim.x * blockDim.x)
        indices[n] = (int32_t)rm_morton3D((uint32_t)coords[n * 3], (uint32_t)coords[n * 3 + 1], (uint32_t)coords[n * 3 + 2]);
}
__global__ void __launch_bounds__(256) k_morton3D_invert(const int32_t *__restrict__ indices, uint32_t N, int32_t *__restrict__ coords) {
    for (uint32_t n = blockIdx.x * blockDim.x + threadIdx.x; n < N; n += gridDim.x * blockDim.x) {
        const int32_t ind = indices[n];
        coords[n * 3] = (int32_t)rm_morton3D_invert((uint32_t)(ind >> 0));
        coords[n * 3 + 1] = (int32_t)rm_morton3D_invert((uint32_t)(ind >> 1));
        coords[n * 3 + 2] = (int32_t)rm_morton3D_invert((uint32_t)(ind >> 2));
    }
}

__global__ void __launch_bounds__(256) k_packbits_x4(const float4 *__restrict__ grid4, uint32_t N4, float thresh,
                              uint32_t *__restrict__ bitfield4) {
    for (uint32_t n = blockIdx.x * blockDim.x + threadIdx.x; n < N4; n += gridDim.x * blockDim.x) {
        uint32_t bits = 0;
#pragma unroll
        for (int q = 0; q < 8; q++) {
            const float4 v = grid4[(uint64_t)n * 8 + q];
            bits |= (v.x > thresh ? 1u : 0u) << (q * 4 + 0);
            bits |= (v.y > thresh ? 1u : 0u) << (q * 4 + 1);
            bits |= (v.z > thresh ? 1u : 0u) << (q * 4 + 2);
            bits |= (v.w > thresh ? 1u : 0u) << (q * 4 + 3);
        }
        bitfield4[n] = bits;
    }
}
__global__ void __launch_bounds__(256) k_packbits_tail(const float *__restrict__ grid, uint32_t n0, uint32_t N, float thresh,
                                uint8_t *__restrict__ bitfield) {
    for (uint32_t n = n0 + blockIdx.x * blockDim.x + threadIdx.x; n < N; n += gridDim.x * blockDim.x) {
        uint32_t bits = 0;
#pragma unroll
        for (int i = 0; i < 8; i++) bits |= (grid[(uint64_t)n * 8 + i] > thresh ? 1u : 0u) << i;
        bitfield[n] = (uint8_t)bits;
    }
}

struct RmCell { float x, y, z, dt, mip_bound; int nx, ny, nz; };

struct RmParams {
    float bound, dt_gamma, dt_min, dt_max, rH, H3, Hf, Cf, Hm1;
    uint32_t H;
    float norm_inv;
    int rederive;
    int gamma_pow2;
};
__device__ __forceinline__ float rm_out(const RmParams &p, float x) { return p.norm_inv != 0.0f ? (x + p.bound) * p.norm_inv : x; }

struct RmRay { float ox, oy, oz, dx, dy, dz, rdx, rdy, rdz; };
template <typename I>
__device__ __forceinline__ RmRay rm_load_ray(const float *__restrict__ rays_o, const float *__restrict__ rays_d, I i) {
    RmRay r;
// ... 1152 lines not shown
```

### focnerf_amd/csrc/sample_math.h

```cpp
#pragma once
#include "common.h"

typedef _Float16 h8 __attribute__((ext_vector_type(8)));

__device__ __forceinline__ void foc_sh16(float x, float y, float z, float (&o)[16]) {
    const float xy = x * y, xz = x * z, yz = y * z, x2 = x * x, y2 = y * y, z2 = z * z;
    o[0] = 0.28209479177387814f;
    o[1] = -0.48860251190291987f * y;
    o[2] = 0.48860251190291987f * z;
    o[3] = -0.48860251190291987f * x;
    o[4] = 1.0925484305920792f * xy;
    o[5] = -1.0925484305920792f * yz;
    o[6] = 0.94617469575755997f * z2 - 0.31539156525251999f;
    o[7] = -1.0925484305920792f * xz;
    o[8] = 0.54627421529603959f * x2 - 0.54627421529603959f * y2;
    o[9] = 0.59004358992664352f * y * (-3.0f * x2 + y2);
    o[10] = 2.8906114426405538f * xy * z;
    o[11] = 0.45704579946446572f * y * (1.0f - 5.0f * z2);
    o[12] = 0.3731763325901154f * z * (5.0f * z2 - 3.0f);
    o[13] = 0.45704579946446572f * x * (1.0f - 5.0f * z2);
    o[14] = 1.4453057213202769f * z * (x2 - y2);
    o[15] = 0.59004358992664352f * x * (-x2 + 3.0f * y2);
}
__device__ __forceinline__ void foc_sh16_h(float x, float y, float z, h8 &lo, h8 &hi) {
    float sh[16];
    foc_sh16(x, y, z, sh);
#pragma unroll
    for (int k = 0; k < 8; k++) { lo[k] = foc_f2h(sh[k]); hi[k] = foc_f2h(sh[8 + k]); }
}

__device__ __forceinline__ float foc_sigmoid_h(float x) { return (float)(_Float16)(1.0f / (1.0f + expf(-x))); }

__device__ __forceinline__ float foc_clamp15(float x) { return x < -15.0f ? -15.0f : (x > 15.0f ? 15.0f : x); }
__device__ __forceinline__ float foc_trunc_exp_bwd(float x) { return expf(foc_clamp15(x)); }
__device__ __forceinline__ float foc_trunc_exp_bwd(float x, float e) {
    const float xc = foc_clamp15(x);
    return xc != x ? expf(xc) : e;
}
struct FocExp15 { float lo, hi; };
__device__ __forceinline__ FocExp15 foc_exp15() {
    float a = -15.0f, b = 15.0f;
    asm volatile("" : "+v"(a));
    asm volatile("" : "+v"(b));
    return FocExp15{expf(a), expf(b)};
}
__device__ __forceinline__ float foc_trunc_exp_bwd_of_sigma(float sigma, const FocExp15 &e) { return fminf(fmaxf(sigma, e.lo), e.hi); }

struct FocBg { float b0, b1, b2; };
__device__ __forceinline__ FocBg foc_bg(const float *__restrict__ bg_ray, float bg_scalar, uint32_t k) {
    return FocBg{bg_ray ? bg_ray[k * 3] : bg_scalar, bg_ray ? bg_ray[k * 3 + 1] : bg_scalar, bg_ray ? bg_ray[k * 3 + 2] : bg_scalar};
}
```

### focnerf_amd/field.py

```python
import os
from dataclasses import dataclass
from typing import Optional

import torch
from torch.autograd import Function
from torch.amp import custom_bwd, custom_fwd

from .backend import _gridencoder, _ffmlp
from .ffmlp import FFMLP, PackedMLP, single_pass_backward
from .gridencoder import GridEncoder, GridSpec


def fused_mlp(model, name):
    get = getattr(model, "fused_mlp", None)
    return get(name) if get is not None else getattr(model, name, None)


@dataclass(frozen=True)
class MlpShape:
    input_dim: int
    hidden_dim: int
    num_layers: int
    activation: int
    output_activation: int
# ... 103 lines not shown

def _raw_stream_of(device):
    from ._lib import raw_stream
    return raw_stream(device.index if device.index is not None else torch.cuda.current_device())


_half_scope = None


class half_cache_scope:

    def __enter__(self):
        global _half_scope
        self._outer = _half_scope
        if _half_scope is None:
            _half_scope = {}
        return self

    def __exit__(self, *exc):
        global _half_scope
        _half_scope = self._outer
        return False


def _half_of(param):
    if param.dtype == torch.half:
        return param.contiguous()
    if _half_scope is None:
        return param.detach().to(torch.half).contiguous()
    hit = _half_scope.get(id(param))
    if hit is not None and hit[0] is param and hit[1].device == param.device:
        if hit[2] is not None and _raw_stream_of(param.device) != hit[3]:
            torch.cuda.current_stream(param.device).wait_event(hit[2])
        return hit[1]
    h = param.detach().to(torch.half).contiguous()
    ev = st = None
    if h.is_cuda:
        st = _raw_stream_of(h.device)
        ev = torch.cuda.Event()
        ev.record(torch.cuda.current_stream(h.device))
    _half_scope[id(param)] = (param, h, ev, st)
    return h


def scope_cached(key, owner, make):
    if _half_scope is None:
        return make()
    hit = _half_scope.get(key)
    if hit is not None and hit[0] is owner:
        if hit[2] is not None and _raw_stream_of(hit[1].device) != hit[3]:
            torch.cuda.current_stream(hit[1].device).wait_event(hit[2])
        return hit[1]
    v = make()
    ev = st = None
    if v.is_cuda:
        st = _raw_stream_of(v.device)
        ev = torch.cuda.Event()
        ev.record(torch.cuda.current_stream(v.device))
    _half_scope[key] = (owner, v, ev, st)
    return v


def _check_colour_branch(colour, B):
    cweights, shape, ray_sh, T, c_width, obj_feat = colour[:6]
    T = int(T)
    if not (ray_sh.dtype == torch.half and ray_sh.dim() == 2 and ray_sh.shape[1] == 16 and ray_sh.is_contiguous() and T > 0
            and B == ray_sh.shape[0] * T):
        raise RuntimeError(f"hashgrid_mlp colour branch: ray_sh must be a contiguous half [B / T, 16] tensor with B = {B}, T = {T}; got "
                           f"{tuple(ray_sh.shape)} {ray_sh.dtype}{'' if ray_sh.is_contiguous() else ' (strided)'}")
    if c_width not in (4, 16):
        raise RuntimeError(f"hashgrid_mlp colour branch: c_width must be 4 or 16, got {c_width}")
    if shape.input_dim not in (32, 48) or (obj_feat is not None) != (shape.input_dim == 48) or (obj_feat is not None and obj_feat.numel() != 16):
        raise RuntimeError(f"hashgrid_mlp colour branch: a {shape.input_dim}-wide colour input takes "
                           f"{'a 16-element object feature' if shape.input_dim == 48 else 'no object feature'}, got "
                           f"{'none' if obj_feat is None else f'{obj_feat.numel()} elements'}")
    if cweights.numel() != 64 * (shape.input_dim + 64 * (shape.num_layers - 1) + 16):
        raise RuntimeError(f"hashgrid_mlp colour branch: the colour weights hold {cweights.numel()} elements, a {shape.input_dim}-wide "
                           f"{shape.num_layers}-layer network has {64 * (shape.input_dim + 64 * (shape.num_layers - 1) + 16)}")


class _hashgrid_mlp(Function):
    @staticmethod
    @custom_fwd(device_type="cuda")
    def forward(ctx, x, embeddings, weights, offsets, grid, sigma, training, colour=None):
        x = x.contiguous().float()
        B = x.shape[0]
        if colour is not None:
            _check_colour_branch(colour, B)
        S, H, (gridtype, align_corners, interp) = grid.log2_scale, grid.base_resolution, grid.tail()
        L = offsets.shape[0] - 1
        emb = _half_of(embeddings)
        w = _half_of(weights)
        enc = torch.empty(L, B, 2, device=x.device, dtype=torch.half)
        ticket = _gridencoder.grid_encode_forward_counted(x, emb, offsets, enc, B, 3, 2, L, S, H, gridtype, align_corners, interp,
                                                          standalone=_gridencoder.precount_standalone()) if training else None
        if ticket is None:
            _gridencoder.grid_encode_forward(x, emb, offsets, enc, B, 3, 2, L, S, H, None, gridtype, align_corners, interp)
        h = torch.empty(B, 16, device=x.device, dtype=torch.half)
        c = None
        if colour is not None:
            from ._lib import ptr, stream_of, check
            cweights, cshape, ray_sh, T, c_width, obj_feat = colour[:6]
            pad = float(colour[6]) if len(colour) > 6 else 0.0
            wc = _half_of(cweights)
            obj16 = object_feature_half(obj_feat, "hashgrid_mlp colour branch")
            c = torch.empty(B, c_width, device=x.device, dtype=torch.half)
            args = (ptr(enc), ptr(w), sigma.num_layers, ptr(ray_sh), int(T), ptr(wc), int(cshape.num_layers), 64, int(sigma.activation), B, ptr(h),
                    ptr(c), int(c_width), ptr(obj16))
            fn, extra = pad_twin("foc_field_forward_train", pad, obj16 is not None)
            check(fn(*args, *extra, stream_of(enc)), "field_forward_train")
        else:
            _ffmlp.ffmlp_forward_planar(enc, w, B, sigma.input_dim, 16, sigma.hidden_dim, sigma.num_layers, sigma.activation, sigma.output_activation, h)
        if training:
            ctx.save_for_backward(x, emb, w, offsets, enc)
            ctx.cfg = (grid, sigma, B, L)
            ctx.ticket = ticket
        if c is None:
            return h
        ctx.mark_non_differentiable(c)
        ctx.set_materialize_grads(False)
        return h, c

    @staticmethod
    @custom_bwd(device_type="cuda")
    def backward(ctx, grad_h, _grad_c=None):
        x, emb, w, offsets, enc = ctx.saved_tensors
        grid, sigma, B, L = ctx.cfg
        if grad_h is None:
            return (None,) * 8
        grad_h = grad_h.contiguous().half()
        g_enc = torch.empty_like(enc)
        g_w = torch.empty_like(w)
        _ffmlp.ffmlp_backward_planar(grad_h, enc, w, B, sigma.input_dim, 16, sigma.hidden_dim, sigma.num_layers, sigma.activation,
                                     sigma.output_activation, True, g_enc, g_w)
        g_emb = torch.zeros_like(emb)
        _gridencoder.grid_encode_backward(g_enc, x, emb, offsets, g_emb, B, 3, 2, L, grid.log2_scale, grid.base_resolution, None, None, *grid.tail(),
                                          grad_bl=False, precount=ctx.ticket)
        return None, g_emb, g_w, None, None, None, None, None


@torch.no_grad()
def field_infer(model, xn, dirs, dir_div=1, dir_block=0, obj_feat=None):
    from ._lib import ptr, stream_of, check
    enc, sn, cn = model.encoder, fused_mlp(model, "sigma_net"), fused_mlp(model, "color_net")
    grid = enc.spec()
    xn = xn.contiguous().float()
    dirs = dirs.contiguous().float()
    M = xn.shape[0]
    L = enc.offsets.shape[0] - 1
    emb, ws, wc = _half_of(enc.embeddings), _half_of(sn.weights), _half_of(cn.weights)
    planes = torch.empty(L, M, 2, device=xn.device, dtype=torch.half)
    _gridencoder.grid_encode_forward(xn, emb, enc.offsets, planes, M, 3, 2, L, grid.log2_scale, grid.base_resolution, None, *grid.tail())
    sigma = torch.empty(M, dtype=torch.float32, device=xn.device)
    rgb = torch.empty(M, 3, dtype=torch.float32, device=xn.device)
    obj16 = None
    if getattr(model, "uses_object_feature", False):
        if obj_feat is None:
            raise RuntimeError("field_infer: an object-conditioned network needs its encoded object feature")
        obj16 = object_feature_half(obj_feat, "field_infer")
    args = (ptr(planes), 1, ptr(dirs), int(dir_div), int(dir_block), dirs.shape[0], ptr(ws), sn.num_layers, ptr(wc), cn.num_layers, 64, sn.activation, M,
            ptr(sigma), ptr(rgb), ptr(obj16))
    fn, extra = pad_twin("foc_nerf_field_inference", float(getattr(model, "colour_input_pad", 0.0)), obj16 is not None)
    check(fn(*args, *extra, stream_of(xn)), "nerf_field_inference")
    return sigma, rgb


def hashgrid_mlp(encoder, mlp, x, bound=1, colour=None):
    prefix = list(x.shape[:-1])
    xn = (x if bound is None else (x + bound) / (2 * bound)).view(-1, 3)
    h = _hashgrid_mlp.apply(xn, encoder.embeddings, mlp.weights, encoder.offsets, encoder.spec(), MlpShape.of(mlp), mlp.training and torch.is_grad_enabled(),
                            colour)
    if colour is not None:
        h, c = h
        return h.view(prefix + [16]), c
    return h.view(prefix + [16])
```

### focnerf_amd/fixedstep.py

```python
import torch
from torch.autograd import Function

from . import raymarching
from ._lib import lib, ptr, stream_of, check
from .gridencoder import grid_encode


RAY_BLOCK = 64


def ray_block_default():
    import os
    return RAY_BLOCK if os.environ.get("FOC_RAY_BLOCK", str(RAY_BLOCK)) != "0" else 0


def blocked_rows(N, T, ray_block):
    return N * T if not ray_block else -(-N // ray_block) * ray_block * T


def fixed_sample(rays_o, rays_d, nears, fars, aabb, noise, T, bound, want_xyzs=False, want_ray_sh=False, ray_block=0):
    N = rays_o.shape[0]
    dev = rays_o.device
    rows = blocked_rows(N, T, ray_block)
    enc_in = torch.empty(rows, 3, dtype=torch.float32, device=dev)
    xyzs = torch.empty(rows, 3, dtype=torch.float32, device=dev) if want_xyzs else None
    ray_sh = torch.empty(N, 16, dtype=torch.float16, device=dev) if want_ray_sh else None
    check(lib.foc_fixed_sample(ptr(rays_o), ptr(rays_d), ptr(nears), ptr(fars), ptr(aabb), ptr(noise), N, T, float(bound), ptr(xyzs), ptr(enc_in),
                               ptr(ray_sh), int(ray_block), stream_of(rays_o)), "fixed_sample")
    if want_ray_sh:
        return enc_in, xyzs, ray_sh
    return enc_in, xyzs


def ray_sh_rows(rays_d):
    rays_d = rays_d.contiguous().float()
    N, dev = rays_d.shape[0], rays_d.device
    zeros, ones = torch.zeros(N, device=dev), torch.ones(N, device=dev)
    aabb = torch.tensor([-1., -1., -1., 1., 1., 1.], device=dev)
    return fixed_sample(torch.zeros_like(rays_d), rays_d, zeros, ones, aabb, None, 2, 1.0, want_ray_sh=True)[2]


class _density_head(Function):

    @staticmethod
    def forward(ctx, h, rays_d, nears, fars, noise, N, T, density_scale, obj_feat=None):
        from .field import object_feature_half
        h = h.contiguous()
        assert h.dtype == torch.float16 and h.shape == (N * T, 16)
        dev = h.device
        M = N * T
        sigma = torch.empty(M, dtype=torch.float32, device=dev)
        trans = torch.empty(M, dtype=torch.float32, device=dev)
        weights = torch.empty(M, dtype=torch.float32, device=dev)
        ws = torch.empty(N, dtype=torch.float32, device=dev)
        depth = torch.empty(N, dtype=torch.float32, device=dev)
        width = 32 if obj_feat is None else 48
        obj_feat = object_feature_half(obj_feat, "_density_head")
        cin = torch.empty(M, width, dtype=torch.float16, device=dev)
        check(lib.foc_fixed_head_forward(ptr(h), ptr(rays_d), ptr(nears), ptr(fars), ptr(noise), N, T, float(density_scale), ptr(sigma), ptr(trans),
                                         ptr(weights), ptr(ws), ptr(depth), ptr(cin), ptr(obj_feat), width, stream_of(h)), "fixed_head_forward")
        ctx.save_for_backward(h, sigma, trans, nears, fars, noise if noise is not None else torch.empty(0, device=dev))
        ctx.has_noise = noise is not None
        ctx.dims = (N, T, float(density_scale))
        ctx.width = width
        ctx.mark_non_differentiable(sigma)
        ctx.set_materialize_grads(False)
        return weights, ws, depth, sigma, cin

    @staticmethod
    def backward(ctx, g_weights, g_ws, g_depth, g_sigma, g_cin):
        h, sigma, trans, nears, fars, noise = ctx.saved_tensors
        N, T, ds = ctx.dims
        noise = noise if ctx.has_noise else None
        g_weights = g_weights.contiguous().float() if g_weights is not None else None
        g_ws = g_ws.contiguous().float() if g_ws is not None else None
        g_depth = g_depth.contiguous().float() if g_depth is not None else None
        g_cin = g_cin.contiguous().half() if g_cin is not None else None
        grad_h = torch.empty_like(h)
        check(lib.foc_fixed_head_backward(ptr(h), ptr(sigma), ptr(trans), ptr(nears), ptr(fars), ptr(noise), ptr(g_weights), ptr(g_ws), ptr(g_depth),
                                          ptr(g_cin), N, T, ds, ptr(grad_h), ctx.width, stream_of(h)), "fixed_head_backward")
        g_obj = None
        if ctx.width == 48 and ctx.needs_input_grad[8] and g_cin is not None:
            g_obj = g_cin[:, 31:47].float().sum(0)
        return grad_h, None, None, None, None, None, None, None, g_obj


class _fixed_composite(Function):

    @staticmethod
    def forward(ctx, c, weights, bg_ray, bg_scalar, N, T, thresh, weights_sum=None):
        c = c.contiguous()
        weights = weights.contiguous()
        assert c.dtype == torch.float16 and c.shape == (N * T, 16) and weights.dtype == torch.float32
        image = torch.empty(N, 3, dtype=torch.float32, device=c.device)
        check(lib.foc_fixed_composite_forward(ptr(c), ptr(weights), ptr(bg_ray), float(bg_scalar), N, T, float(thresh), ptr(image), stream_of(c)),
              "fixed_composite_forward")
        ctx.bg_grad = bg_ray is not None and ctx.needs_input_grad[2]
        if ctx.bg_grad and weights_sum is None:
            raise RuntimeError("_fixed_composite: a background that needs a gradient needs weights_sum")
        empty = torch.empty(0, device=c.device)
        ctx.save_for_backward(c, weights, bg_ray if bg_ray is not None else empty, weights_sum.detach() if ctx.bg_grad else empty)
        ctx.has_bg = bg_ray is not None
        ctx.dims = (N, T, float(thresh), float(bg_scalar))
        return image

    @staticmethod
    def backward(ctx, g_image):
        c, weights, bg_ray, weights_sum = ctx.saved_tensors
        N, T, thresh, bg_scalar = ctx.dims
        bg_ray = bg_ray if ctx.has_bg else None
        g_image = g_image.contiguous().float()
        grad_c = torch.empty_like(c)
        grad_w = torch.empty_like(weights)
        check(lib.foc_fixed_composite_backward(ptr(g_image), ptr(c), ptr(weights), ptr(bg_ray), bg_scalar, N, T, thresh, ptr(grad_c), ptr(grad_w),
# ... 67 lines not shown
        obj16 = obj16 if has_obj else None
        N, T, ds, thresh, bg_scalar, num_layers, activation, input_pad = ctx.dims
        noise = noise if has_noise else None
        bg_ray = bg_ray if has_bg else None
        dev, M = h.device, N * T
        st = stream_of(h)
        g_image = g_image.contiguous().float() if g_image is not None else torch.zeros(N, 3, dtype=torch.float32, device=dev)
        g_ws = g_ws.contiguous().float() if g_ws is not None else None
        g_depth = g_depth.contiguous().float() if g_depth is not None else None
        g_sumsq = g_sumsq.contiguous().float() if g_sumsq is not None else None
        grad_c = torch.empty_like(c)
        grad_h0 = torch.empty(M, dtype=torch.float16, device=dev)
        if g_dist is not None:
            g_dist = g_dist.contiguous().float()
            check(lib.foc_fixed_tail_backward_dist(ptr(g_image), ptr(g_ws), ptr(g_depth), ptr(c), ptr(sigma), ptr(trans), ptr(weights), ptr(ws), ptr(nears),
                                                   ptr(fars), ptr(noise), ptr(bg_ray), bg_scalar, N, T, ds, thresh, ptr(grad_c), ptr(grad_h0), _C_WIDTH,
                                                   ptr(g_sumsq), ptr(wm), None, ptr(g_dist), st), "fixed_tail_backward_dist")
        else:
            check(lib.foc_fixed_tail_backward(ptr(g_image), ptr(g_ws), ptr(g_depth), ptr(c), ptr(sigma), ptr(trans), ptr(weights), ptr(nears), ptr(fars),
                                              ptr(noise), ptr(bg_ray), bg_scalar, N, T, ds, thresh, ptr(grad_c), ptr(grad_h0), _C_WIDTH, ptr(g_sumsq), st),
                  "fixed_tail_backward")
        grad_h = torch.empty_like(h)
        g_w = torch.empty_like(w16)
        wsb = _scratch.get("ffmlp_ws", lib.foc_ffmlp_backward_workspace_bytes(48 if has_obj else 32, 64, num_layers), dev)
        g_obj32 = torch.empty(16, dtype=torch.float32, device=dev) if has_obj and ctx.needs_input_grad[14] else None
        args = (ptr(grad_c), ptr(h), ptr(ray_sh), T, ptr(grad_h0), ptr(w16), M, 64, num_layers, activation, ptr(grad_h), ptr(g_w), ptr(wsb),
                wsb.numel(), _C_WIDTH, ptr(obj16), ptr(g_obj32))
        fn, extra = pad_twin("foc_color_head_backward", input_pad, has_obj)
        check(fn(*args, *extra, st), "color_head_backward")
        g_obj = g_obj32.to(obj_dtype).view(obj_shape) if g_obj32 is not None else None
        g_bg = g_image * (1 - ws).unsqueeze(-1) if ctx.bg_grad else None
        return (grad_h, g_w, None, None, None, None, g_bg) + (None,) * 7 + (g_obj, None, None, None, None, None)


class _masked_norm(Function):

    @staticmethod
    def forward(ctx, sumsq, outside):
        crit = torch.sqrt((sumsq * outside).sum())
        ctx.save_for_backward(crit, outside)
        return crit

    @staticmethod
    def backward(ctx, g):
        crit, outside = ctx.saved_tensors
        coef = torch.where(crit > 0, g / (2 * crit), torch.zeros_like(crit))
        return outside * coef, None


def _unfused_distortion(weights, nears, fars, noise, N, T):
    from .loss import ray_distortion
    span = (fars - nears).unsqueeze(-1)
    z = span * torch.linspace(0.0, 1.0, T, device=weights.device).unsqueeze(0)
    if noise is not None:
        z = z + (noise.view(N, T) - 0.5) * (span / T)
    delta = torch.cat([z[:, 1:] - z[:, :-1], span / T], dim=-1)
    live = (fars > nears).unsqueeze(-1)
    zero = torch.zeros_like(z)
    return ray_distortion(torch.where(live, weights.view(N, T), zero), torch.where(live, z + 0.5 * delta, zero), torch.where(live, delta, zero))


def _background(bg_color, N, dev):
    if bg_color is None:
        return None, 1.0
    if torch.is_tensor(bg_color):
        if bg_color.numel() > 1:
            return bg_color.to(dev, torch.float32).reshape(-1, 3).expand(N, 3).contiguous(), 0.0
        return None, float(bg_color)
    return None, float(bg_color)


def render_fixed_steps(model, rays_o, rays_d, yolo_details=None, num_steps=512, bg_color=None, perturb=False, weight_thresh=1e-10,
                       return_fields=None, _out=None, distortion=False, **kwargs):
    import time
    if return_fields is None:
        return_fields = not model.training
    t_start = time.time()
    prefix = rays_o.shape[:-1]
    rays_o = rays_o.contiguous().view(-1, 3).float()
    rays_d = rays_d.contiguous().view(-1, 3).float()
    N, T = rays_o.shape[0], int(num_steps)
    dev = rays_o.device
    aabb = model.aabb_train if model.training else model.aabb_infer
    nears, fars = raymarching.near_far_from_aabb(rays_o, rays_d, aabb, model.min_near)
    noise = torch.rand(N * T, dtype=torch.float32, device=dev) if perturb else None
    from .field import field_plan, field_infer
    plan = field_plan(model)
    if getattr(model, "bg_radius", 0) > 0:
        bg_color = model._background_colour(rays_o, rays_d, bg_color)
    want_tail = plan.tail and model.training and torch.is_grad_enabled()
    fused_infer = not torch.is_grad_enabled() and plan.infer
    if distortion and not torch.is_grad_enabled():
        raise ValueError("render_fixed_steps: distortion=True needs the training route (gradients enabled): the inference paths form no "
                         "differentiable weights; call it under torch.enable_grad() with model.train()")
    rb = ray_block_default() if fused_infer else 0
    enc_in, _, ray_sh = fixed_sample(rays_o, rays_d, nears, fars, aabb, noise, T, model.bound, want_ray_sh=True) if want_tail else \
        fixed_sample(rays_o, rays_d, nears, fars, aabb, noise, T, model.bound, ray_block=rb) + (None,)

    if fused_infer:
        obj_feat = model.encode_object_feature(yolo_details, dev) if plan.uses_object_feature else None
        sigma, rgb = field_infer(model, enc_in, rays_d, dir_div=T, dir_block=rb, obj_feat=obj_feat)
        bg_ray, bg_scalar = _background(bg_color, N, dev)
        direct = (_out is not None and _out[0].dtype == torch.float32 and _out[1].dtype == torch.float32 and _out[0].is_contiguous()
                  and _out[1].is_contiguous() and _out[0].numel() == N and _out[1].numel() == 3 * N and _out[0].device == dev)
        depth, image = (_out[0].view(N), _out[1].view(N, 3)) if direct else (torch.empty(N, dtype=torch.float32, device=dev),
                                                                              torch.empty(N, 3, dtype=torch.float32, device=dev))
        weights_sum = torch.empty(N, dtype=torch.float32, device=dev)
        rgb_masked = densities = None
        if return_fields:
            if direct and len(_out) == 4 and all(t.dtype == torch.float32 and t.is_contiguous() and t.device == dev for t in _out[2:]) \
                    and _out[2].numel() == N * T and _out[3].numel() == 3 * N * T and rb:
                densities, rgb_masked = _out[2].view(N * T), _out[3].view(N * T, 3)
            else:
                rgb_masked = torch.empty(N * T, 3, dtype=torch.float32, device=dev)
                densities = torch.empty(N * T, dtype=torch.float32, device=dev) if rb else None
        check(lib.foc_fixed_render_inference(ptr(sigma), ptr(rgb), ptr(nears), ptr(fars), ptr(noise), ptr(bg_ray), float(bg_scalar), N, T,
                                             float(model.density_scale), float(weight_thresh), ptr(image), ptr(depth), ptr(weights_sum), ptr(rgb_masked),
                                             rb, ptr(densities), stream_of(sigma)), "fixed_render_inference")
        t_mid = time.time()
        results = {'depth': depth.view(*prefix), 'image': image.view(*prefix, 3), 'weights_sum': weights_sum, 'criterion_outside_mask': None,
                   'timing': [t_mid - t_start, time.time() - t_mid]}
        if return_fields:
            results['densities'] = (densities if rb else sigma).view(N, T, 1)
            results['rgbs'] = rgb_masked.view(N, T, 3)
        return results

    enc = model.encoder
    from .field import hashgrid_mlp, fused_mlp
    c_pre = obj_feat = None
    cweights = fused_mlp(model, "color_net").weights if want_tail else None
    with torch.autocast("cuda", dtype=torch.float16):
        if plan.uses_object_feature:
            obj_feat = model.encode_object_feature(yolo_details, dev)
        if plan.field:
            colour = wc16 = None
            if want_tail and plan.train_forward:
                from .field import _half_of
                wc16 = _half_of(cweights)
                colour = (wc16, plan.colour, ray_sh, T, _C_WIDTH, obj_feat, plan.colour_input_pad)
            h = hashgrid_mlp(enc, fused_mlp(model, "sigma_net"), enc_in, None, colour)
            if colour is not None:
                h, c_pre = h
        else:
            feats = grid_encode(enc_in, enc.embeddings, enc.offsets, enc.per_level_scale, enc.base_resolution, False, enc.gridtype_id,
                                enc.align_corners, enc.interp_id)
            h = fused_mlp(model, "sigma_net")(feats)
        if h.shape[1] != 16:
            raise RuntimeError("render_fixed_steps expects a 16-wide sigma head (1 + geo_feat_dim = 16)")
        fused_tail = want_tail
        want_crit = model.training and yolo_details is not None and yolo_details[0] is not None
        criterion_outside_mask = None
        if fused_tail:
            cn = fused_mlp(model, "color_net")
            bg_ray, bg_scalar = _background(bg_color, N, dev)
            outs = _render_tail.apply(h, cweights, ray_sh, nears, fars, noise, bg_ray, bg_scalar, N, T, model.density_scale, weight_thresh,
                                      cn.num_layers, cn.activation, obj_feat, want_crit and yolo_details[0].numel() == N, c_pre,
                                      wc16 if c_pre is not None else None, plan.colour_input_pad, *((True,) if distortion else ()))
            image, weights_sum, depth, sigma, weights, c = outs[:6]
            ray_dist = outs[-1] if distortion else None
            if len(outs) - bool(distortion) == 7:
                criterion_outside_mask = _masked_norm.apply(outs[6], (~yolo_details[0].reshape(N)).to(torch.float32))
        else:
            weights, weights_sum, depth, sigma, cin = _density_head.apply(h, rays_d, nears, fars, noise, N, T, model.density_scale, obj_feat)
            if plan.colour_input_pad != 0:
                cin = torch.cat([cin[:, :-1], cin.new_full((cin.shape[0], 1), plan.colour_input_pad)], dim=1)
            if distortion:
                ray_dist = _unfused_distortion(weights, nears, fars, noise, N, T)
        if want_crit and criterion_outside_mask is None:
            from .activation import trunc_exp
            criterion_outside_mask = torch.norm(trunc_exp(h[:, 0]).view(N, T)[~yolo_details[0].squeeze(0)] - 0)
        if not fused_tail:
            c = fused_mlp(model, "color_net").forward_padded(cin)
    t_mid = time.time()

    if not fused_tail:
        bg_ray, bg_scalar = _background(bg_color, N, dev)
        image = _fixed_composite.apply(c, weights, bg_ray, bg_scalar, N, T, weight_thresh, weights_sum)

    results = {'depth': depth.view(*prefix), 'image': image.view(*prefix, 3), 'weights_sum': weights_sum,
               'criterion_outside_mask': criterion_outside_mask, 'timing': [t_mid - t_start, time.time() - t_mid]}
    if distortion:
        results['distortion'] = ray_dist.view(*prefix)
    if return_fields:
        from .head import rgb_head
        c16 = c.detach()
        if c16.shape[1] != 16:
            c16 = torch.nn.functional.pad(c16, (0, 16 - c16.shape[1]))
        rgb = rgb_head(c16) * (weights > weight_thresh).unsqueeze(-1)
        results['densities'] = sigma.view(N, T, 1)
        results['rgbs'] = rgb.view(N, T, 3)
    return results


@torch.no_grad()
def render_field4(model, rays_o, rays_d, num_steps=512, weight_thresh=1e-10, yolo_details=None, out=None, occupancy=None, placement=None,
                  scene_aabb=None, channels="rgb"):
    from .field import field_plan, field_infer
    from .normals import check_channels, field_normals
    if placement is None and scene_aabb is not None:
        raise ValueError("render_field4: scene_aabb belongs to a placement; without one the object is rendered in its own box")
    if placement is not None and occupancy is None:
        raise ValueError("render_field4: placement needs occupancy= (the placed path is the occupancy-culled one): pass "
                         "fixedcull.Occupancy.of(model) for a cuda_ray network or fixedcull.Occupancy.estimate(model) for any other")
    rays_o = rays_o.contiguous().view(-1, 3).float()
    rays_d = rays_d.contiguous().view(-1, 3).float()
    N, T = rays_o.shape[0], int(num_steps)
    dev = rays_o.device
    if out is None:
        out = torch.empty(N, T, 4, dtype=torch.float32, device=dev)
    assert out.shape == (N, T, 4) and out.dtype == torch.float32 and out.is_contiguous()
    plan = field_plan(model)
    want_normal = check_channels("render_field4", channels, plan)
    if placement is not None:
        from .fixedcull import render_field4_placed
        return render_field4_placed(model, plan, rays_o, rays_d, T, weight_thresh, yolo_details, out, occupancy, placement, scene_aabb, channels)
    if occupancy is not None:
        from .fixedcull import render_field4_culled
        return render_field4_culled(model, plan, rays_o, rays_d, T, weight_thresh, yolo_details, out, occupancy, channels)
    if want_normal and not (plan.infer and model.bg_radius <= 0):
        raise ValueError("render_field4: channels='normal' needs a network the fused inference serves (field_plan(model).infer) without a "
                         "background model")
    if plan.infer and model.bg_radius <= 0:
        aabb = model.aabb_train if model.training else model.aabb_infer
# ... 18 lines not shown
```

### include/focnerf.h

```cpp
#ifndef FOCNERF_H
#define FOCNERF_H

#include <stddef.h>
#include <stdint.h>

#ifdef __cplusplus
extern "C" {
#endif

#define FOC_OK            0
#define FOC_E_INVALID     1
#define FOC_E_DTYPE       2
#define FOC_E_LAUNCH      3

#define FOC_F32 0
#define FOC_F16 1

#define FOC_ABI_VERSION 2
int         foc_abi_version(void);
const char *foc_last_error(void);
int foc_set_option(const char *name, int value);
int foc_get_option(const char *name, int *value);
int foc_guard_pick_device(int stream_is_null, int stream_device, int pointer_device, int current_device);
const char *foc_arch(void);
// ... 57 lines not shown
int foc_march_rays_two_phase_sample_major(uint32_t n_alive, uint32_t n_step, int flags);
int foc_composite_compact(uint32_t n_alive, uint32_t n_step, float T_thresh, int32_t *rays_alive, float *rays_t,
                          const float *sigmas, const float *rgbs, const float *deltas, float *weights_sum, float *depth,
                          float *image, int32_t *out, int32_t *n_out, int32_t *block_counts, int32_t *deaths, uint32_t deaths_base,
                          uint32_t deaths_len, int sample_major, void *stream);
uint64_t foc_occ_render_step_scratch_bytes(uint32_t n_rays);
int foc_occ_render_step(uint32_t n_alive, uint32_t n_step, const int32_t *rays_alive, int32_t *rays_alive_out, int32_t *count,
                        float *rays_t, const float *rays_o, const float *rays_d, float bound, float dt_gamma, uint32_t max_steps,
                        uint32_t C, uint32_t H, const uint8_t *grid, const float *nears, const float *fars, const float *noises,
                        float *samples, void *planes, float *sigma, float *rgb,
                        const void *embeddings, const int32_t *offsets, const int32_t *offsets_host, uint32_t L, float S, uint32_t base_res,
                        const void *sigma_weights, uint32_t sigma_layers, const void *color_weights, uint32_t color_layers, uint32_t activation,
                        const void *obj_feat, float T_thresh, float *weights_sum, float *depth, float *image, void *scratch, uint32_t flags,
                        int32_t *deaths, uint32_t deaths_base, uint32_t deaths_len, void *stream);
int foc_occ_render_step_pad31(uint32_t n_alive, uint32_t n_step, const int32_t *rays_alive, int32_t *rays_alive_out, int32_t *count,
                              float *rays_t, const float *rays_o, const float *rays_d, float bound, float dt_gamma, uint32_t max_steps,
                              uint32_t C, uint32_t H, const uint8_t *grid, const float *nears, const float *fars, const float *noises,
                              float *samples, void *planes, float *sigma, float *rgb,
                              const void *embeddings, const int32_t *offsets, const int32_t *offsets_host, uint32_t L, float S, uint32_t base_res,
                              const void *sigma_weights, uint32_t sigma_layers, const void *color_weights, uint32_t color_layers, uint32_t activation,
                              const void *obj_feat, float T_thresh, float *weights_sum, float *depth, float *image, void *scratch, uint32_t flags,
                              int32_t *deaths, uint32_t deaths_base, uint32_t deaths_len, float input_pad, void *stream);
int foc_occ_render_step_pad(uint32_t n_alive, uint32_t n_step, const int32_t *rays_alive, int32_t *rays_alive_out, int32_t *count,
                            float *rays_t, const float *rays_o, const float *rays_d, float bound, float dt_gamma, uint32_t max_steps,
                            uint32_t C, uint32_t H, const uint8_t *grid, const float *nears, const float *fars, const float *noises,
                            float *samples, void *planes, float *sigma, float *rgb,
                            const void *embeddings, const int32_t *offsets, const int32_t *offsets_host, uint32_t L, float S, uint32_t base_res,
                            const void *sigma_weights, uint32_t sigma_layers, const void *color_weights, uint32_t color_layers, uint32_t activation,
                            const void *obj_feat, float T_thresh, float *weights_sum, float *depth, float *image, void *scratch, uint32_t flags,
                            int32_t *deaths, uint32_t deaths_base, uint32_t deaths_len, float input_pad, void *stream);
int foc_occ_render_step_normals(uint32_t n_alive, uint32_t n_step, const int32_t *rays_alive, int32_t *rays_alive_out, int32_t *count,
                                float *rays_t, const float *rays_o, const float *rays_d, float bound, float dt_gamma, uint32_t max_steps,
                                uint32_t C, uint32_t H, const uint8_t *grid, const float *nears, const float *fars, const float *noises,
                                float *samples, void *planes, float *sigma, float *rgb,
                                const void *embeddings, const int32_t *offsets, const int32_t *offsets_host, uint32_t L, float S, uint32_t base_res,
                                const void *sigma_weights, uint32_t sigma_layers, const void *color_weights, uint32_t color_layers, uint32_t activation,
                                const void *obj_feat, float T_thresh, float *weights_sum, float *depth, float *image, void *scratch, uint32_t flags,
                                int32_t *deaths, uint32_t deaths_base, uint32_t deaths_len, float input_pad, uint32_t pad_column, uint32_t mode,
                                float *normal_rgb, float *normal_acc, void *stream);

int foc_compact_alive(const int32_t *rays_alive, uint32_t n_alive, int32_t *out, int32_t *n_out,
                      int32_t *scratch, void *stream);


int foc_grid_encode_forward(const float *inputs, const void *embeddings, const int32_t *offsets,
                            void *outputs, uint32_t B, uint32_t D, uint32_t C, uint32_t L,
                            float S, uint32_t H, void *dy_dx, uint32_t gridtype,
                            int align_corners, uint32_t interp, int dtype,
                            const int32_t *offsets_host, void *stream);

int foc_grid_encode_forward_bl(const float *inputs, const void *embeddings, const int32_t *offsets,
                               void *outputs, uint32_t B, uint32_t D, uint32_t C, uint32_t L,
                               float S, uint32_t H, void *dy_dx, uint32_t gridtype,
                               int align_corners, uint32_t interp, int dtype,
                               const int32_t *offsets_host, void *stream);
int foc_grid_planes_to_rows(const void *planes, void *rows, uint32_t B, uint32_t L, uint32_t unit_bytes, void *stream);
int foc_grid_forward_index_path(uint32_t level_rows, uint32_t resolution, uint32_t level_offset_rows);
int foc_grid_rows_to_planes(const void *rows, void *planes, uint32_t B, uint32_t L, uint32_t unit_bytes, void *stream);

int foc_grid_encode_backward(const void *grad, const float *inputs, const void *embeddings,
                             const int32_t *offsets, void *grad_embeddings,
                             uint32_t B, uint32_t D, uint32_t C, uint32_t L, float S, uint32_t H,
                             const void *dy_dx, void *grad_inputs, uint32_t gridtype,
                             int align_corners, uint32_t interp, int dtype, int grad_is_bl,
                             const int32_t *offsets_host, void *stream);

uint64_t foc_grid_encode_backward_workspace_bytes(uint32_t B, uint32_t D, uint32_t C, uint32_t L, int dtype);
int foc_grid_encode_backward_binned(const void *grad, const float *inputs, const void *embeddings,
                                    const int32_t *offsets, void *grad_embeddings,
                                    uint32_t B, uint32_t D, uint32_t C, uint32_t L, float S, uint32_t H,
                                    const void *dy_dx, void *grad_inputs, uint32_t gridtype,
                                    int align_corners, uint32_t interp, int dtype, int grad_is_bl,
                                    const int32_t *offsets_host, void *workspace, uint64_t workspace_bytes,
                                    void *stream);

int foc_grid_encode_forward_counted(const float *inputs, const void *embeddings, const int32_t *offsets, void *outputs,
                                    uint32_t B, uint32_t D, uint32_t C, uint32_t L, float S, uint32_t H,
                                    uint32_t gridtype, int align_corners, uint32_t interp, int dtype,
                                    const int32_t *offsets_host, void *workspace, uint64_t workspace_bytes, void *stream);
int foc_grid_encode_backward_count(const float *inputs, const int32_t *offsets, uint32_t B, uint32_t D, uint32_t C,
                                   uint32_t L, float S, uint32_t H, uint32_t gridtype, int align_corners,
                                   uint32_t interp, int dtype, const int32_t *offsets_host, void *workspace,
                                   uint64_t workspace_bytes, void *stream);
int foc_grid_encode_backward_binned_counted(const void *grad, const float *inputs, const void *embeddings,
                                            const int32_t *offsets, void *grad_embeddings,
                                            uint32_t B, uint32_t D, uint32_t C, uint32_t L, float S, uint32_t H,
                                            const void *dy_dx, void *grad_inputs, uint32_t gridtype,
                                            int align_corners, uint32_t interp, int dtype, int grad_is_bl,
                                            const int32_t *offsets_host, void *workspace, uint64_t workspace_bytes,
                                            void *stream);

int foc_grad_total_variation(const void *inputs, const void *embeddings, void *grad,
                             const int32_t *offsets, float weight,
                             uint32_t B, uint32_t D, uint32_t C, uint32_t L, float S, uint32_t H,
                             uint32_t gridtype, int align_corners, int dtype, void *stream);


int foc_freq_encode_forward(const float *inputs, uint32_t B, uint32_t D, uint32_t deg, uint32_t C,
                            float *outputs, void *stream);
int foc_freq_encode_backward(const float *grad, const float *outputs, uint32_t B, uint32_t D,
                             uint32_t deg, uint32_t C, float *grad_inputs, void *stream);


int foc_ffmlp_forward(const void *inputs, const void *weights, uint32_t B, uint32_t input_dim,
                      uint32_t output_dim, uint32_t hidden_dim, uint32_t num_layers,
                      uint32_t activation, uint32_t output_activation,
                      void *forward_buffer, void *outputs, void *stream);

int foc_ffmlp_inference(const void *inputs, const void *weights, uint32_t B, uint32_t input_dim,
                        uint32_t output_dim, uint32_t hidden_dim, uint32_t num_layers,
                        uint32_t activation, uint32_t output_activation,
                        void *inference_buffer, void *outputs, void *stream);

int foc_ffmlp_backward(const void *grad, const void *inputs, const void *weights,
                       const void *forward_buffer, uint32_t B, uint32_t input_dim,
                       uint32_t output_dim, uint32_t hidden_dim, uint32_t num_layers,
                       uint32_t activation, uint32_t output_activation, int calc_grad_inputs,
                       void *backward_buffer, void *grad_inputs, void *grad_weights,
                       void *workspace, uint64_t workspace_bytes, void *stream);
uint64_t foc_ffmlp_backward_workspace_bytes(uint32_t input_dim, uint32_t hidden_dim, uint32_t num_layers);

int foc_ffmlp_forward_planar(const void *inputs_planar, const void *weights, uint32_t B, uint32_t input_dim,
                             uint32_t output_dim, uint32_t hidden_dim, uint32_t num_layers,
                             uint32_t activation, uint32_t output_activation, void *outputs, void *stream);
int foc_ffmlp_backward_planar(const void *grad, const void *inputs_planar, const void *weights, uint32_t B,
                              uint32_t input_dim, uint32_t output_dim, uint32_t hidden_dim, uint32_t num_layers,
                              uint32_t activation, uint32_t output_activation, int calc_grad_inputs,
                              void *grad_inputs_planar, void *grad_weights, void *workspace, uint64_t workspace_bytes, void *stream);

int foc_nerf_field_inference(const void *enc, int enc_planar, const float *dirs, uint32_t dir_div,
                             uint32_t dir_block, uint32_t n_dirs, const void *sigma_weights, uint32_t sigma_layers, const void *color_weights,
                             uint32_t color_layers, uint32_t hidden_dim, uint32_t activation, uint32_t B,
                             float *sigma, float *rgb, const void *obj_feat, void *stream);
int foc_nerf_field_inference_pad(const void *enc, int enc_planar, const float *dirs, uint32_t dir_div,
                                 uint32_t dir_block, uint32_t n_dirs, const void *sigma_weights, uint32_t sigma_layers, const void *color_weights,
                                 uint32_t color_layers, uint32_t hidden_dim, uint32_t activation, uint32_t B,
                                 float *sigma, float *rgb, const void *obj_feat, float input_pad, void *stream);
int foc_nerf_field_inference_pad31(const void *enc, int enc_planar, const float *dirs, uint32_t dir_div,
                                   uint32_t dir_block, uint32_t n_dirs, const void *sigma_weights, uint32_t sigma_layers, const void *color_weights,
                                   uint32_t color_layers, uint32_t hidden_dim, uint32_t activation, uint32_t B,
                                   float *sigma, float *rgb, const void *obj_feat, float input_pad, void *stream);

int foc_field_normals(const float *xn, uint32_t M, const void *embeddings, const uint32_t *offsets, uint32_t D, uint32_t C, uint32_t L,
                      float S, uint32_t H, uint32_t gridtype, int align_corners, uint32_t interp, int dtype, const int32_t *offsets_host,
                      const void *sigma_weights, uint32_t sigma_layers, uint32_t hidden_dim, uint32_t activation, const float *rot9,
                      float *sigma, float *grad_raw, float *normal_rgb, void *grad_enc, void *stream);
int foc_normal_map_finish(const float *normal_acc, const float *weights_sum, uint32_t N, float *normal, float *normal_rgb, void *stream);

int foc_color_head_forward(const void *h, const void *ray_sh, uint32_t samples_per_ray, const void *weights,
                           uint32_t B, uint32_t hidden_dim, uint32_t num_layers, uint32_t activation,
                           void *outputs, uint32_t out_width, const void *obj_feat, void *stream);
int foc_color_head_backward(const void *grad, const void *h, const void *ray_sh, uint32_t samples_per_ray,
                            const void *grad_h0, const void *weights, uint32_t B, uint32_t hidden_dim,
                            uint32_t num_layers, uint32_t activation, void *grad_h, void *grad_weights,
                            void *workspace, uint64_t workspace_bytes, uint32_t out_width, const void *obj_feat, float *grad_obj, void *stream);
int foc_color_head_forward_pad(const void *h, const void *ray_sh, uint32_t samples_per_ray, const void *weights,
                               uint32_t B, uint32_t hidden_dim, uint32_t num_layers, uint32_t activation,
                               void *outputs, uint32_t out_width, const void *obj_feat, float input_pad, void *stream);
int foc_color_head_backward_pad(const void *grad, const void *h, const void *ray_sh, uint32_t samples_per_ray,
                                const void *grad_h0, const void *weights, uint32_t B, uint32_t hidden_dim,
                                uint32_t num_layers, uint32_t activation, void *grad_h, void *grad_weights,
                                void *workspace, uint64_t workspace_bytes, uint32_t out_width, const void *obj_feat, float *grad_obj,
                                float input_pad, void *stream);
int foc_color_head_forward_pad31(const void *h, const void *ray_sh, uint32_t samples_per_ray, const void *weights,
                                 uint32_t B, uint32_t hidden_dim, uint32_t num_layers, uint32_t activation,
                                 void *outputs, uint32_t out_width, const void *obj_feat, float input_pad, void *stream);
int foc_color_head_backward_pad31(const void *grad, const void *h, const void *ray_sh, uint32_t samples_per_ray,
                                  const void *grad_h0, const void *weights, uint32_t B, uint32_t hidden_dim,
                                  uint32_t num_layers, uint32_t activation, void *grad_h, void *grad_weights,
                                  void *workspace, uint64_t workspace_bytes, uint32_t out_width, const void *obj_feat, float *grad_obj,
                                  float input_pad, void *stream);

int foc_field_forward_train(const void *planes, const void *sigma_weights, uint32_t sigma_layers, const void *ray_sh, uint32_t samples_per_ray,
                            const void *color_weights, uint32_t color_layers, uint32_t hidden_dim, uint32_t activation, uint32_t B,
                            void *h, void *c, uint32_t out_width, const void *obj_feat, void *stream);
int foc_field_forward_train_pad(const void *planes, const void *sigma_weights, uint32_t sigma_layers, const void *ray_sh, uint32_t samples_per_ray,
                                const void *color_weights, uint32_t color_layers, uint32_t hidden_dim, uint32_t activation, uint32_t B,
                                void *h, void *c, uint32_t out_width, const void *obj_feat, float input_pad, void *stream);
int foc_field_forward_train_pad31(const void *planes, const void *sigma_weights, uint32_t sigma_layers, const void *ray_sh, uint32_t samples_per_ray,
                                  const void *color_weights, uint32_t color_layers, uint32_t hidden_dim, uint32_t activation, uint32_t B,
                                  void *h, void *c, uint32_t out_width, const void *obj_feat, float input_pad, void *stream);

int foc_allocate_splitk(uint64_t size);
int foc_free_splitk(void);


int foc_combine_select(const float *dens, const float *rgb, float *max_dens, float *best_rgb,
                       uint64_t n, void *stream);

int foc_combine_pack_keys(const float *dens, uint32_t rank, uint64_t *keys, uint64_t n, void *stream);
int foc_combine_unpack(const uint64_t *keys, uint32_t rank, const float *rgb,
                       float *max_dens, float *masked_rgb, uint64_t n, void *stream);

int foc_composite_fixed_steps(const float *sigmas, const float *rgbs, const float *nears,
                              const float *fars, uint32_t N, uint32_t T, float bg,
                              float *image4, float *depth, void *stream);

#define FOC_COMBINE_MAX_OBJECTS 16

int foc_combine_select_composite(const float *const *fields4, uint32_t K, const float *nears, const float *fars,
                                 uint32_t N, uint32_t T, const float *bgs, uint32_t n_bg, float *image4, float *depth,
                                 float *merged4, void *stream);

int foc_combine_select4(const float *field4, float *acc4, uint64_t n, void *stream);

int foc_combine_select_composite_attr(const float *const *fields4, uint32_t K, const uint8_t *const *id_planes,
                                      const uint32_t *ids, uint32_t n_obj, const float *nears, const float *fars,
                                      uint32_t N, uint32_t T, const float *bgs, uint32_t n_bg, float *image4, float *depth,
                                      float *merged4, float *obj_weights, float *obj_depth, int32_t *instance,
                                      uint8_t *winner, void *stream);

typedef struct FocCulledField {
    const uint64_t *mask;
    const uint32_t *offsets;
    const float *sigma_c;
    const float *rgb_c;
    uint32_t m_occ;
    float density_scale;
    float thresh;
    float sigma_gain;
} FocCulledField;
int foc_combine_select_composite_culled(const FocCulledField *objs, uint32_t K, uint32_t struct_bytes, const uint32_t *ids,
                                        uint32_t n_obj, const float *nears, const float *fars, uint32_t N, uint32_t T,
                                        const float *bgs, uint32_t n_bg, float *image4, float *depth, float *merged4,
                                        float *obj_weights, float *obj_depth, int32_t *instance, uint8_t *winner, void *stream);

int foc_combine_select4_ids(const float *field4, uint32_t id, float *acc4, uint8_t *acc_ids, uint64_t n, void *stream);

int foc_mo_select(const void *sigma_new, const void *feat_new, void *sigma_best, void *feat_best, uint64_t n,
                  uint32_t feat_width, uint32_t elem_bytes, void *stream);


int foc_fixed_sample(const float *rays_o, const float *rays_d, const float *nears, const float *fars,
                     const float *aabb, const float *noise, uint32_t N, uint32_t T, float bound,
                     float *xyzs, float *enc_in, void *ray_sh, uint32_t ray_block, void *stream);

int foc_fixed_head_forward(const void *h, const float *rays_d, const float *nears, const float *fars,
                           const float *noise, uint32_t N, uint32_t T, float density_scale,
                           float *sigma, float *trans, float *weights, float *weights_sum, float *depth,
                           void *cin, const void *obj_feat, uint32_t cin_width, void *stream);
int foc_fixed_head_backward(const void *h, const float *sigma, const float *trans, const float *nears,
                            const float *fars, const float *noise, const float *grad_w, const float *grad_ws,
                            const float *grad_depth, const void *grad_cin, uint32_t N, uint32_t T,
                            float density_scale, void *grad_h, uint32_t cin_width, void *stream);

int foc_fixed_tail_forward(const void *h, const void *c, const float *nears, const float *fars, const float *noise,
                           const float *bg_ray, float bg_scalar, uint32_t N, uint32_t T, float density_scale, float thresh,
                           float *sigma, float *trans, float *weights, float *weights_sum, float *depth, float *image,
                           uint32_t c_width, float *ray_sumsq, void *stream);
int foc_fixed_tail_backward(const float *grad_image, const float *grad_ws, const float *grad_depth, const void *c,
                            const float *sigma, const float *trans, const float *weights, const float *nears,
                            const float *fars, const float *noise, const float *bg_ray, float bg_scalar, uint32_t N,
                            uint32_t T, float density_scale, float thresh, void *grad_c, void *grad_h0, uint32_t c_width,
                            const float *grad_sumsq, void *stream);

int foc_occ_tail_forward(const void *h, const void *c, uint32_t c_width, const float *deltas, const int32_t *rays,
                         uint32_t M, uint32_t N, float T_thresh, float density_scale, const float *bg_ray, float bg_scalar,
                         const float *nears, const float *fars, float *weights_sum, float *image_raw, float *image,
                         float *depth, void *stream);
int foc_occ_tail_backward(const float *grad_image, const float *grad_ws, const void *h, const void *c, uint32_t c_width,
                          const float *deltas, const int32_t *rays, const int32_t *counter, const float *weights_sum,
                          const float *image_raw, uint32_t M, uint32_t N, float T_thresh, float density_scale,
                          const float *bg_ray, float bg_scalar, void *grad_c, void *grad_h0, void *stream);
int foc_occ_tail_forward_sumsq(const void *h, const void *c, uint32_t c_width, const float *deltas, const int32_t *rays,
                               uint32_t M, uint32_t N, float T_thresh, float density_scale, const float *bg_ray, float bg_scalar,
                               const float *nears, const float *fars, float *weights_sum, float *image_raw, float *image,
                               float *depth, float *ray_sumsq, void *stream);
int foc_occ_tail_backward_sumsq(const float *grad_image, const float *grad_ws, const void *h, const void *c, uint32_t c_width,
                                const float *deltas, const int32_t *rays, const int32_t *counter, const float *weights_sum,
                                const float *image_raw, uint32_t M, uint32_t N, float T_thresh, float density_scale,
                                const float *bg_ray, float bg_scalar, void *grad_c, void *grad_h0, const float *grad_sumsq, void *stream);

int foc_fixed_tail_forward_dist(const void *h, const void *c, const float *nears, const float *fars, const float *noise,
                                const float *bg_ray, float bg_scalar, uint32_t N, uint32_t T, float density_scale, float thresh,
                                float *sigma, float *trans, float *weights, float *weights_sum, float *depth, float *image,
                                uint32_t c_width, float *ray_sumsq, float *ray_dist, float *ray_wm, void *stream);
int foc_fixed_tail_backward_dist(const float *grad_image, const float *grad_ws, const float *grad_depth, const void *c,
                                 const float *sigma, const float *trans, const float *weights, const float *weights_sum, const float *nears,
                                 const float *fars, const float *noise, const float *bg_ray, float bg_scalar, uint32_t N,
                                 uint32_t T, float density_scale, float thresh, void *grad_c, void *grad_h0, uint32_t c_width,
                                 const float *grad_sumsq, const float *ray_wm, const float *ray_dist, const float *grad_dist, void *stream);
int foc_occ_tail_forward_dist(const void *h, const void *c, uint32_t c_width, const float *deltas, const int32_t *rays,
                              uint32_t M, uint32_t N, float T_thresh, float density_scale, const float *bg_ray, float bg_scalar,
                              const float *nears, const float *fars, float *weights_sum, float *image_raw, float *image,
                              float *depth, float *ray_sumsq, float *ray_dist, float *ray_wm, void *stream);
int foc_occ_tail_backward_dist(const float *grad_image, const float *grad_ws, const void *h, const void *c, uint32_t c_width,
                               const float *deltas, const int32_t *rays, const int32_t *counter, const float *weights_sum,
                               const float *image_raw, uint32_t M, uint32_t N, float T_thresh, float density_scale,
                               const float *bg_ray, float bg_scalar, void *grad_c, void *grad_h0, const float *grad_sumsq,
                               const float *ray_wm, const float *ray_dist, const float *grad_dist, void *stream);
int foc_occ_tail_forward_depth(const void *h, const void *c, uint32_t c_width, const float *deltas, const int32_t *rays,
                               uint32_t M, uint32_t N, float T_thresh, float density_scale, const float *bg_ray, float bg_scalar,
                               const float *nears, const float *fars, float *weights_sum, float *image_raw, float *image,
                               float *depth, float *ray_sumsq, float *ray_dist, float *ray_wm, float *depth_raw, void *stream);
int foc_occ_tail_backward_depth(const float *grad_image, const float *grad_ws, const void *h, const void *c, uint32_t c_width,
                                const float *deltas, const int32_t *rays, const int32_t *counter, const float *weights_sum,
                                const float *image_raw, uint32_t M, uint32_t N, float T_thresh, float density_scale,
                                const float *bg_ray, float bg_scalar, void *grad_c, void *grad_h0, const float *grad_sumsq,
                                const float *ray_wm, const float *ray_dist, const float *grad_dist, const float *nears,
                                const float *fars, const float *depth_raw, const float *grad_depth, void *stream);

typedef struct FocOccTrainNode {
    uint32_t struct_bytes;
    uint32_t n_rays, max_steps, cascade, grid_size, cap, pad_align;
    float bound, dt_gamma, min_near;
    const float *rays_o, *rays_d, *aabb, *jitter;
    const uint8_t *bitfield;
    float *nears, *fars, *enc_in, *deltas;
    void *sh_rows;
    int32_t *rays, *counter, *march_scratch;
    uint32_t levels, base_resolution, gridtype, interp;
    int32_t align_corners, table_dtype;
    float per_level_scale_log2;
    const void *embeddings;
    const int32_t *offsets, *offsets_host;
    void *planes, *grid_workspace;
    uint64_t grid_workspace_bytes;
    uint32_t sigma_input_dim, sigma_hidden, sigma_layers, sigma_activation, sigma_output_activation;
// ... 88 lines not shown
int foc_mark_untrained_grid(const float *poses, uint32_t B, float fx, float fy, float cx, float cy, float bound,
                            uint32_t cascade, uint32_t H, float *density_grid, int32_t *count, void *stream);
int foc_grid_cells_xyz(uint32_t cascade, uint32_t H, float bound, const float *jitter, float *xyzs, void *stream);
uint64_t foc_grid_update_sample_workspace_bytes(uint32_t cascade, uint32_t H);
int foc_grid_update_sample(const float *density_grid, uint32_t cascade, uint32_t H, float bound, uint32_t N,
                           const int32_t *rand_coords, const float *rand_pick, const float *jitter,
                           int32_t *indices, float *xyzs, void *workspace, uint64_t workspace_bytes, void *stream);
uint64_t foc_grid_update_apply_workspace_bytes(uint32_t cascade, uint32_t H);
int foc_grid_update_apply(float *density_grid, uint32_t cascade, uint32_t H, const float *sigmas, const int32_t *indices,
                          uint32_t Mc, float density_scale, float decay, float density_thresh, uint8_t *bitfield,
                          float *mean_out, void *workspace, uint64_t workspace_bytes, void *stream);

int foc_background_forward(const float *rays_o, const float *rays_d, const float *coords, float radius, uint32_t N, const float *embeddings,
                           const int32_t *offsets, float per_level_scale_log2, uint32_t base_resolution, const void *weights, void *rgb,
                           void *stream);
uint64_t foc_background_backward_workspace_bytes(uint32_t N);
int foc_background_backward(const void *grad_rgb, const float *rays_o, const float *rays_d, const float *coords, float radius, uint32_t N,
                            const float *embeddings, const int32_t *offsets, float per_level_scale_log2, uint32_t base_resolution,
                            const void *weights, float *grad_embeddings, float *grad_weights, void *workspace, uint64_t workspace_bytes,
                            void *stream);

uint64_t foc_mc_workspace_bytes(uint32_t nx, uint32_t ny, uint32_t nz);
int foc_mc_count(const float *volume, uint32_t nx, uint32_t ny, uint32_t nz, float thr, void *workspace, uint32_t *counts3,
                 void *stream);
int foc_mc_emit(const float *volume, uint32_t nx, uint32_t ny, uint32_t nz, float thr, const void *workspace,
                const float *origin3, const float *spacing3, float *vertices, float *normals, int32_t *triangles, void *stream);

uint64_t foc_lattice_cull_scratch_bytes(uint32_t count);
int foc_lattice_cull(const float *xs, const float *ys, const float *zs, uint32_t rx, uint32_t ry, uint32_t rz, uint32_t first,
                     uint32_t count, const float *world_to_object, const float *obj_aabb, float bound, const uint8_t *bitfield,
                     uint32_t cascade, uint32_t grid_size, uint64_t *mask, uint32_t *offsets, uint32_t *count_out, void *scratch,
                     uint64_t scratch_bytes, void *stream);
int foc_lattice_cull_emit(const float *xs, const float *ys, const float *zs, uint32_t rx, uint32_t ry, uint32_t rz, uint32_t first,
                          uint32_t count, const float *world_to_object, const uint64_t *mask, const uint32_t *offsets,
                          uint32_t m_occ, float *pos_c, void *stream);
int foc_volume_scatter_max(const float *sigma_c, const uint64_t *mask, const uint32_t *offsets, float gain, float *volume,
                           uint32_t n, void *stream);

int foc_points_cull(const float *points, uint32_t M, const float *world_to_object, const float *obj_aabb, float bound,
                    const uint8_t *bitfield, uint32_t cascade, uint32_t grid_size, uint64_t *mask, uint32_t *offsets,
                    uint32_t *count_out, void *scratch, uint64_t scratch_bytes, void *stream);
int foc_points_cull_emit(const float *points, uint32_t M, const float *world_to_object, float bound, const uint64_t *mask,
                         const uint32_t *offsets, uint32_t m_occ, float *pos_c, float *xn_c, void *stream);
int foc_surface_frame(const float *grad_raw_c, const float *pos_c, uint32_t m, const float *rot9, int mode, const float *eye_obj,
                      float *dirs_c, float *normal_c, void *stream);
int foc_scene_select(const float *sigma_c, const float *rgb_c, const float *normal_c, const uint64_t *mask, const uint32_t *offsets,
                     float gain, int32_t object_index, float *best_sigma, int32_t *best_id, float *best_rgb, float *best_normal,
                     uint32_t n, void *stream);

uint64_t foc_score_workspace_bytes(uint32_t H, uint32_t W, uint32_t B);
int foc_score_quantize(const float *image4, const float *depth, const float *gt, const float *bgs, uint32_t H, uint32_t W, uint32_t B,
                       uint8_t *pred_u8, uint8_t *gt_u8, uint8_t *depth_u8, void *stream);
int foc_score_view(const uint8_t *pred_u8, const uint8_t *gt_u8, uint32_t H, uint32_t W, uint32_t B, const double *taps,
                   uint32_t radius, double C1, double C2, double *out, void *workspace, uint64_t workspace_bytes, void *stream);

#define FOC_OPTIM_MAX_TENSORS 16
#define FOC_OPTIM_CHUNK 4096
#define FOC_OPTIM_STEP 0
#define FOC_OPTIM_CHECK 1
#define FOC_OPTIM_DECIDE 2
typedef struct FocOptimTensor {
    float *param, *grad, *exp_avg, *exp_avg_sq, *step;
    const float *lr_tensor;
    int64_t n;
    double lr, beta1, beta2, eps, weight_decay;
} FocOptimTensor;
typedef struct FocOptimStep {
    uint32_t struct_bytes;
    uint32_t tensor_bytes;
    int32_t n_tensors;
    uint32_t phase, zero_grads;
    int32_t growth_interval;
    float growth_factor, backoff_factor;
    const FocOptimTensor *tensors;
    float *scale;
    int32_t *growth_tracker;
    const float *grad_scale, *found_inf;
    void *workspace;
    uint64_t workspace_bytes;
} FocOptimStep;
size_t foc_optim_workspace_bytes(int n_tensors);
int foc_optim_step(const FocOptimStep *step, void *stream);

#define FOC_U8 2
#define FOC_LOSS_MSE 0
#define FOC_LOSS_HUBER 1
#define FOC_PHOTO_LOSS_MAX_WGS 256
int foc_philox4x32_10(const uint32_t *ctr, const uint32_t *key, uint32_t *out);
uint64_t foc_batch_workspace_bytes(void);
int foc_batch_sample(const void *images, int image_dtype, uint32_t V, uint32_t H, uint32_t W, uint32_t C, const float *poses, float fx,
                     float fy, float cx, float cy, const int32_t *order, int64_t *step, uint64_t seed, uint32_t N,
                     const int64_t *inds_coarse, int random_bg, int linear, int64_t *inds, float *rays_o, float *rays_d, float *bg_color,
                     float *gt_rgb, int32_t *view, void *workspace, uint64_t workspace_bytes, uint32_t workgroups, void *stream);
int foc_view_rays(const float *pose, float fx, float fy, float cx, float cy, uint32_t H, uint32_t W, float *rays_o, float *rays_d,
                  void *stream);
uint64_t foc_photo_loss_workspace_bytes(void);
int foc_photo_loss(const void *pred, int pred_dtype, const float *gt, uint32_t N, int kind, float delta, float *error_map, uint32_t V,
                   const int32_t *view, const int64_t *inds_coarse, float *ray_loss, float *grad, float *loss, void *workspace,
                   uint64_t workspace_bytes, void *stream);

#ifdef __cplusplus
}
#endif
#endif
```

Before: 1.318 billion.

## Fold training-path launches: fused near/far+sample kernel, self-cleaning counts, batched half casts

Adds one kernel that computes ray near/far, SH encoding and normalized sample positions in a single launch for the training path, replacing two separate launches. The binned grid backward now zeroes its counts after the scan, so the next forward can skip the counts memset when the workspace is known clean. A new prepare step casts the embedding table and MLP weights to half and zeroes the grad table in one batched kernel. The tradeoff is more epoch-tracking state in Python, with a risk of stale counts if that bookkeeping goes wrong.

```diff
diff --git a/focnerf_amd/backend.py b/focnerf_amd/backend.py
--- a/focnerf_amd/backend.py
+++ b/focnerf_amd/backend.py
@@ -172,12 +172,14 @@
 
     _pre = {}
 
+    self_cleaning_counts = True
+
     @staticmethod
     def _pre_state(device):
         idx = device.index if device.index is not None else torch.cuda.current_device()
         st = _gridencoder._pre.get(idx)
         if st is None:
-            st = _gridencoder._pre[idx] = dict(ticket=0, key=None)
+            st = _gridencoder._pre[idx] = dict(ticket=0, key=None, epoch=0)
         return idx, st
 
     @staticmethod
@@ -185,6 +187,26 @@
         _, st = _gridencoder._pre_state(device)
         st["ticket"] += 1
         st["key"] = None
+        st["epoch"] += 1
+
+    @staticmethod
+    def _spend_precount(device):
+        _, st = _gridencoder._pre_state(device)
+        st["ticket"] += 1
+        st["key"] = None
+
+    @staticmethod
+    def _counts_clean(ws):
+        _, st = _gridencoder._pre_state(ws.device)
+        return _gridencoder.self_cleaning_counts and getattr(ws, "_foc_counts_clean", None) == st["epoch"]
+
+    @staticmethod
+    def _counts_in_flight(ws):
+        ws._foc_counts_clean = None
+
+    @staticmethod
+    def _counts_settled(ws):
+        ws._foc_counts_clean = _gridencoder._pre_state(ws.device)[1]["epoch"]
 
     @staticmethod
     def binned_workspace_bytes(offsets, B, D, C, L, S, H, gridtype, dt, count_ahead=False):
@@ -224,15 +246,18 @@
             raise RuntimeError("grid_encode_forward_counted: outputs must be [L,B,C] of the embeddings' dtype")
         ws = _scratch.get("grid_bwd", ws_bytes, inputs.device)
         host = _gridencoder._host_offsets(offsets)
+        clean = _gridencoder._counts_clean(ws)
+        _gridencoder._counts_in_flight(ws)
         if standalone:
             check(lib.foc_grid_encode_backward_count(ptr(inputs), ptr(offsets), B, D, C, L, float(S), H, gridtype, int(bool(align_corners)), interp, dt,
                                                      host, ptr(ws), ws_bytes, stream_of(inputs)), "grid_encode_backward_count")
             check(lib.foc_grid_encode_forward(ptr(inputs), ptr(embeddings), ptr(offsets), ptr(outputs), B, D, C, L, float(S), H, None, gridtype,
                                               int(bool(align_corners)), interp, dt, None, stream_of(inputs)), "grid_encode_forward")
         else:
-            check(lib.foc_grid_encode_forward_counted(ptr(inputs), ptr(embeddings), ptr(offsets), ptr(outputs), B, D, C, L, float(S), H, gridtype,
-                                                      int(bool(align_corners)), interp, dt, host, ptr(ws), ws_bytes, stream_of(inputs)),
-                  "grid_encode_forward_counted")
+            fn = lib.foc_grid_encode_forward_counted_clean if clean else lib.foc_grid_encode_forward_counted
+            check(fn(ptr(inputs), ptr(embeddings), ptr(offsets), ptr(outputs), B, D, C, L, float(S), H, gridtype, int(bool(align_corners)), interp, dt,
+                     host, ptr(ws), ws_bytes, stream_of(inputs)), "grid_encode_forward_counted")
+        _gridencoder._counts_settled(ws)
         return _gridencoder.issue_precount_ticket(inputs, B, L, dt, ws)
 
     @staticmethod
@@ -256,10 +281,14 @@
             ws = _scratch.get("grid_bwd", ws_bytes, grad.device)
             counted = _gridencoder._precount_valid(precount, inputs, B, L, dt, ws)
             fn = lib.foc_grid_encode_backward_binned_counted if counted else lib.foc_grid_encode_backward_binned
+            if not counted:
+                _gridencoder._counts_in_flight(ws)
             check(fn(ptr(grad), ptr(inputs), ptr(embeddings), ptr(offsets), ptr(grad_embeddings), B, D, C, L, float(S), H,
                      ptr(dy_dx), ptr(grad_inputs), gridtype, int(bool(align_corners)), interp, dt, int(bool(grad_bl)),
                      _gridencoder._host_offsets(offsets), ptr(ws), ws_bytes, stream_of(inputs)), "grid_encode_backward_binned")
-            _gridencoder._invalidate_precount(grad.device)
+            _gridencoder._spend_precount(grad.device)
+            if not counted:
+                _gridencoder._counts_settled(ws)
             return
         check(lib.foc_grid_encode_backward(ptr(grad), ptr(inputs), ptr(embeddings), ptr(offsets), ptr(grad_embeddings), B, D, C, L, float(S), H,
                                            ptr(dy_dx), ptr(grad_inputs), gridtype, int(bool(align_corners)), interp, dt, int(bool(grad_bl)),
diff --git a/focnerf_amd/csrc/fixedstep.hip b/focnerf_amd/csrc/fixedstep.hip
--- a/focnerf_amd/csrc/fixedstep.hip
+++ b/focnerf_amd/csrc/fixedstep.hip
@@ -33,6 +33,59 @@
             h8 *dst = reinterpret_cast<h8 *>(ray_sh + (uint64_t)n * 16);
             dst[0] = lo; dst[1] = hi;
         }
+    }
+}
+
+#define FS_TRAIN_ROWS 4u
+#define FS_TRAIN_TILE (256u * FS_TRAIN_ROWS)
+template <bool VEC>
+__global__ void __launch_bounds__(256) k_fs_sample_train(const float *__restrict__ rays_o, const float *__restrict__ rays_d, const float *__restrict__ aabb,
+                                                         float min_near, const float *__restrict__ noise, uint32_t N, uint32_t T, float bound,
+                                                         float *__restrict__ nears, float *__restrict__ fars, float *__restrict__ enc_in,
+                                                         _Float16 *__restrict__ ray_sh) {
+    __shared__ float4 s_pos4[FS_TRAIN_TILE * 3 / 4];
+    __shared__ float s_near[FS_TRAIN_TILE / 2 + 2], s_far[FS_TRAIN_TILE / 2 + 2];
+    float *s_pos = reinterpret_cast<float *>(s_pos4);
+    const uint64_t total = (uint64_t)N * T, n_tiles = (total + FS_TRAIN_TILE - 1) / FS_TRAIN_TILE;
+    const FsBox box = fs_box(aabb);
+    const float two_b = 2 * bound;
+    for (uint64_t tile = blockIdx.x; tile < n_tiles; tile += gridDim.x) {
+        const uint64_t base = tile * FS_TRAIN_TILE;
+        const uint32_t rows = (uint32_t)min((uint64_t)FS_TRAIN_TILE, total - base);
+        const uint32_t n0 = (uint32_t)(base / T), r0 = (uint32_t)(base - (uint64_t)n0 * T);
+        const uint32_t n_rays = (r0 + rows - 1) / T + 1;
+        for (uint32_t k = threadIdx.x; k < n_rays; k += 256) {
+            const uint32_t n = n0 + k;
+            const float dx = rays_d[n * 3], dy = rays_d[n * 3 + 1], dz = rays_d[n * 3 + 2];
+            float near, far;
+            rm_near_far(rays_o[n * 3], rays_o[n * 3 + 1], rays_o[n * 3 + 2], dx, dy, dz, box.a0, box.a1, box.a2, box.a3, box.a4, box.a5, min_near, near, far);
+            s_near[k] = near; s_far[k] = far;
+            if (k > 0 || r0 == 0) {
+                nears[n] = near; fars[n] = far;
+                h8 lo, hi;
+                foc_sh16_h(dx, dy, dz, lo, hi);
+                h8 *dst = reinterpret_cast<h8 *>(ray_sh + (uint64_t)n * 16);
+                dst[0] = lo; dst[1] = hi;
+            }
+        }
+        __syncthreads();
+#pragma unroll
+        for (uint32_t j = 0; j < FS_TRAIN_ROWS; j++) {
+            const uint32_t r = j * 256 + threadIdx.x;
+            if (r < rows) {
+                const uint32_t q = r0 + r, k = q / T, i = q - k * T, n = n0 + k;
+                const FsGeom g = fs_geom_of(s_near[k], s_far[k], T);
+                const float z = fs_z(g, i, T, noise, base + r);
+                float x, y, w;
+                fs_point(rays_o[n * 3], rays_o[n * 3 + 1], rays_o[n * 3 + 2], rays_d[n * 3], rays_d[n * 3 + 1], rays_d[n * 3 + 2], z, box, x, y, w);
+                s_pos[r * 3] = fs_norm(x, bound, two_b); s_pos[r * 3 + 1] = fs_norm(y, bound, two_b); s_pos[r * 3 + 2] = fs_norm(w, bound, two_b);
+            }
+        }
+        __syncthreads();
+        float *out = enc_in + base * 3;
+        const uint32_t n_floats = rows * 3, n_vec = VEC ? n_floats / 4 : 0u;
+        for (uint32_t v = threadIdx.x; v < n_vec; v += 256) reinterpret_cast<float4 *>(out)[v] = s_pos4[v];
+        for (uint32_t f = n_vec * 4 + threadIdx.x; f < n_floats; f += 256) out[f] = s_pos[f];
     }
 }
 
@@ -405,6 +458,24 @@
     return FOC_OK;
 }
 
+int foc_fixed_sample_train(const float *rays_o, const float *rays_d, const float *aabb, float min_near, const float *noise, uint32_t N, uint32_t T,
+                           float bound, float *nears, float *fars, float *enc_in, void *ray_sh, void *stream) {
+    FocDeviceGuard foc_guard_(stream, rays_o);
+    if (N == 0) return FOC_OK;
+    FOC_REQUIRE(rays_o && rays_d && aabb && nears && fars && enc_in && ray_sh, FOC_E_INVALID, "fixed_sample_train: null pointer");
+    FOC_REQUIRE(T >= 2, FOC_E_INVALID, "fixed_sample_train: T must be >= 2");
+    const uint64_t tiles = ((uint64_t)N * T + FS_TRAIN_TILE - 1) / FS_TRAIN_TILE;
+    const dim3 grid(foc_grid_1d(tiles, 1, 256 * 16));
+    if ((reinterpret_cast<uintptr_t>(enc_in) & 15u) == 0)
+        hipLaunchKernelGGL((k_fs_sample_train<true>), grid, dim3(256), 0, (hipStream_t)stream, rays_o, rays_d, aabb, min_near, noise, N, T, bound, nears, fars,
+                           enc_in, (_Float16 *)ray_sh);
+    else
+        hipLaunchKernelGGL((k_fs_sample_train<false>), grid, dim3(256), 0, (hipStream_t)stream, rays_o, rays_d, aabb, min_near, noise, N, T, bound, nears, fars,
+                           enc_in, (_Float16 *)ray_sh);
+    FOC_CHECK_LAUNCH("fixed_sample_train");
+    return FOC_OK;
+}
+
 int foc_fixed_head_forward(const void *h, const float *rays_d, const float *nears, const float *fars, const float *noise, uint32_t N, uint32_t T,
                            float density_scale, float *sigma, float *trans, float *weights, float *weights_sum, float *depth, void *cin,
                            const void *obj_feat, uint32_t cin_width, void *stream) {
diff --git a/focnerf_amd/csrc/fs_common.h b/focnerf_amd/csrc/fs_common.h
--- a/focnerf_amd/csrc/fs_common.h
+++ b/focnerf_amd/csrc/fs_common.h
@@ -9,13 +9,16 @@
     return (uint64_t)(n / FS_RAY_BLOCK) * FS_RAY_BLOCK * T + (uint64_t)i * FS_RAY_BLOCK + n % FS_RAY_BLOCK;
 }
 
-__device__ __forceinline__ FsGeom fs_geom(const float *__restrict__ nears, const float *__restrict__ fars, uint32_t n, uint32_t T) {
+__device__ __forceinline__ FsGeom fs_geom_of(float near, float far, uint32_t T) {
     FsGeom g;
-    g.near = nears[n]; g.far = fars[n];
+    g.near = near; g.far = far;
     g.span = g.far - g.near;
     g.sample_dist = g.span / (float)T;
     g.step = 1.0f / (float)(T - 1);
     return g;
+}
+__device__ __forceinline__ FsGeom fs_geom(const float *__restrict__ nears, const float *__restrict__ fars, uint32_t n, uint32_t T) {
+    return fs_geom_of(nears[n], fars[n], T);
 }
 __device__ __forceinline__ float fs_z0(const FsGeom &g, uint32_t i, uint32_t T) {
     const float lin = (i < T / 2) ? (g.step * (float)i) : fmaf(-g.step, (float)(T - 1 - i), 1.0f);
diff --git a/focnerf_amd/csrc/gridencoder.hip b/focnerf_amd/csrc/gridencoder.hip
--- a/focnerf_amd/csrc/gridencoder.hip
+++ b/focnerf_amd/csrc/gridencoder.hip
@@ -14,6 +14,7 @@
     uint32_t base[GE_MAX_LEVELS * GB_MAX_SEGS + 1];
     uint32_t cursor[GE_MAX_LEVELS * GB_MAX_SEGS];
     uint32_t chunk_prefix[GE_MAX_LEVELS * GB_MAX_SEGS + 1];
+    uint32_t live_counts[GE_MAX_LEVELS * GB_MAX_SEGS];
 };
 
 struct GbSizes { uint32_t size[GE_MAX_LEVELS]; };
@@ -131,6 +132,7 @@
         for (uint32_t i = lo; i < hi; i++) {
             const uint32_t c = hdr->counts[i];
             hdr->base[i] = r; hdr->chunk_prefix[i] = k;
+            hdr->live_counts[i] = c; hdr->counts[i] = 0u;
             r += c; k += (c + GB_CHUNK - 1) / GB_CHUNK;
         }
         if (threadIdx.x == 255) { hdr->base[n] = r; hdr->chunk_prefix[n] = k; }
@@ -285,7 +287,7 @@
             const uint32_t wi = slot * n_wg + tile;
             nsb = sb;
             nw0 = wg_base[wi];
-            nw1 = *(tile + 1 < n_wg ? &wg_base[wi + 1u] : &hdr->counts[slot]);
+            nw1 = *(tile + 1 < n_wg ? &wg_base[wi + 1u] : &hdr->live_counts[slot]);
         }
     };
     auto setup_tables = [&](uint32_t pbn) {
@@ -438,7 +440,7 @@
     __syncthreads();
     for (uint32_t i = threadIdx.x; i < n; i += GB_RTHREADS) {
         const uint32_t p0 = hdr->chunk_prefix[i], p1 = hdr->chunk_prefix[i + 1];
-        const uint32_t cnt = hdr->counts[i];
+        const uint32_t cnt = hdr->live_counts[i];
         const uint64_t b0 = hdr->base[i];
         if (p0 <= chunk_id && chunk_id < p1) {
             const uint32_t c = chunk_id - p0;
@@ -776,10 +778,10 @@
 
 template <typename T>
 static int gb_forward_counted(const float *inputs, const void *emb, const int32_t *offsets, void *outputs, uint32_t B, uint32_t L, const GeLevels &lv,
-                              uint32_t gridtype, bool ac, uint32_t interp, void *workspace, hipStream_t st) {
+                              uint32_t gridtype, bool ac, uint32_t interp, void *workspace, bool clean, hipStream_t st) {
     GbHeader *hdr = reinterpret_cast<GbHeader *>(workspace);
     void *recs = reinterpret_cast<char *>(workspace) + ((sizeof(GbHeader) + 255) & ~(uint64_t)255);
-    if (foc_zero_async(hdr->counts, sizeof(hdr->counts), st) != hipSuccess) { foc_set_error("grid_encode_forward_counted: memset failed"); return FOC_E_LAUNCH; }
+    if (!clean && foc_zero_async(hdr->counts, sizeof(hdr->counts), st) != hipSuccess) { foc_set_error("grid_encode_forward_counted: memset failed"); return FOC_E_LAUNCH; }
     const uint32_t n_tiles = foc_div_up(B, GB_PM_TILE), chunks = foc_div_up(B, 256);
     const uint32_t lc = ge_small_levels(L, lv);
     const uint32_t groups = lc >= 2u ? L - lc + 1u : L;
@@ -970,10 +972,9 @@
     return gb_count(inputs, offsets, B, L, lv, gridtype, align_corners != 0, interp, dtype, workspace, (hipStream_t)stream);
 }
 
-int foc_grid_encode_forward_counted(const float *inputs, const void *embeddings, const int32_t *offsets, void *outputs, uint32_t B, uint32_t D, uint32_t C,
+static int gb_forward_counted_entry(const float *inputs, const void *embeddings, const int32_t *offsets, void *outputs, uint32_t B, uint32_t D, uint32_t C,
                                     uint32_t L, float S, uint32_t H, uint32_t gridtype, int align_corners, uint32_t interp, int dtype,
-                                    const int32_t *offsets_host, void *workspace, uint64_t workspace_bytes, void *stream) {
-    FocDeviceGuard foc_guard_(stream, inputs);
+                                    const int32_t *offsets_host, void *workspace, uint64_t workspace_bytes, bool clean, void *stream) {
     if (B == 0) return FOC_OK;
     FOC_REQUIRE(inputs && embeddings && offsets && outputs && workspace && offsets_host, FOC_E_INVALID, "grid_encode_forward_counted: null pointer");
     const int rc = gb_check(B, D, C, L, S, H, gridtype, interp, dtype, offsets_host, workspace_bytes);
@@ -981,8 +982,24 @@
     GeLevels lv;
     ge_make_levels(L, S, H, lv);
     hipStream_t st = (hipStream_t)stream;
-    if (dtype == FOC_F32) return gb_forward_counted<float>(inputs, embeddings, offsets, outputs, B, L, lv, gridtype, align_corners != 0, interp, workspace, st);
-    return gb_forward_counted<__half>(inputs, embeddings, offsets, outputs, B, L, lv, gridtype, align_corners != 0, interp, workspace, st);
+    if (dtype == FOC_F32) return gb_forward_counted<float>(inputs, embeddings, offsets, outputs, B, L, lv, gridtype, align_corners != 0, interp, workspace, clean, st);
+    return gb_forward_counted<__half>(inputs, embeddings, offsets, outputs, B, L, lv, gridtype, align_corners != 0, interp, workspace, clean, st);
+}
+
+int foc_grid_encode_forward_counted(const float *inputs, const void *embeddings, const int32_t *offsets, void *outputs, uint32_t B, uint32_t D, uint32_t C,
+                                    uint32_t L, float S, uint32_t H, uint32_t gridtype, int align_corners, uint32_t interp, int dtype,
+                                    const int32_t *offsets_host, void *workspace, uint64_t workspace_bytes, void *stream) {
+    FocDeviceGuard foc_guard_(stream, inputs);
+    return gb_forward_counted_entry(inputs, embeddings, offsets, outputs, B, D, C, L, S, H, gridtype, align_corners, interp, dtype, offsets_host, workspace,
+                                    workspace_bytes, false, stream);
+}
+
+int foc_grid_encode_forward_counted_clean(const float *inputs, const void *embeddings, const int32_t *offsets, void *outputs, uint32_t B, uint32_t D, uint32_t C,
+                                          uint32_t L, float S, uint32_t H, uint32_t gridtype, int align_corners, uint32_t interp, int dtype,
+                                          const int32_t *offsets_host, void *workspace, uint64_t workspace_bytes, void *stream) {
+    FocDeviceGuard foc_guard_(stream, inputs);
+    return gb_forward_counted_entry(inputs, embeddings, offsets, outputs, B, D, C, L, S, H, gridtype, align_corners, interp, dtype, offsets_host, workspace,
+                                    workspace_bytes, true, stream);
 }
 
 static int gb_entry(const void *grad, const float *inputs, const int32_t *offsets, void *grad_embeddings,
diff --git a/focnerf_amd/csrc/prepare.hip b/focnerf_amd/csrc/prepare.hip
--- /dev/null
+++ b/focnerf_amd/csrc/prepare.hip
@@ -0,0 +1,110 @@
+#include "common.h"
+
+#define HCZ_MAX_COPIES 4
+#define HCZ_UNROLL 2u
+#define HCZ_WG_GROUPS (256u * HCZ_UNROLL)
+
+typedef _Float16 hcz_h8 __attribute__((ext_vector_type(8)));
+
+struct HczJob {
+    const float *src;
+    char *dst;
+    uint64_t n;
+    uint64_t groups;
+    uint32_t head;
+    uint32_t block0;
+    uint32_t src_vec;
+};
+struct HczJobs { HczJob j[HCZ_MAX_COPIES + 1]; uint32_t count; };
+
+__global__ void __launch_bounds__(256) k_half_copy_zero(HczJobs jobs) {
+    uint32_t k = 0;
+    while (k + 1 < jobs.count && blockIdx.x >= jobs.j[k + 1].block0) k++;
+    const HczJob &job = jobs.j[k];
+    const uint32_t wg = blockIdx.x - job.block0;
+    if (job.src) {
+        _Float16 *dst = reinterpret_cast<_Float16 *>(job.dst);
+        const float *src = job.src;
+        if (wg == 0) {
+            const uint64_t tail0 = job.head + job.groups * 8u;
+            if (threadIdx.x < job.head) dst[threadIdx.x] = (_Float16)src[threadIdx.x];
+            if (tail0 + threadIdx.x < job.n) dst[tail0 + threadIdx.x] = (_Float16)src[tail0 + threadIdx.x];
+        }
+        src += job.head; dst += job.head;
+#pragma unroll
+        for (uint32_t u = 0; u < HCZ_UNROLL; u++) {
+            const uint64_t g = (uint64_t)wg * HCZ_WG_GROUPS + u * 256u + threadIdx.x;
+            if (g < job.groups) {
+                float v[8];
+                if (job.src_vec) {
+                    const float4 a = reinterpret_cast<const float4 *>(src)[g * 2], b = reinterpret_cast<const float4 *>(src)[g * 2 + 1];
+                    v[0] = a.x; v[1] = a.y; v[2] = a.z; v[3] = a.w; v[4] = b.x; v[5] = b.y; v[6] = b.z; v[7] = b.w;
+                } else {
+#pragma unroll
+                    for (int e = 0; e < 8; e++) v[e] = src[g * 8 + e];
+                }
+                hcz_h8 o;
+#pragma unroll
+                for (int e = 0; e < 8; e++) o[e] = (_Float16)v[e];
+                reinterpret_cast<hcz_h8 *>(dst)[g] = o;
+            }
+        }
+    } else {
+        char *dst = job.dst;
+        if (wg == 0) {
+            const uint64_t tail0 = job.head + job.groups * 16u;
+            if (threadIdx.x < job.head) dst[threadIdx.x] = 0;
+            if (tail0 + threadIdx.x < job.n) dst[tail0 + threadIdx.x] = 0;
+        }
+        uint4 *body = reinterpret_cast<uint4 *>(dst + job.head);
+#pragma unroll
+        for (uint32_t u = 0; u < HCZ_UNROLL; u++) {
+            const uint64_t g = (uint64_t)wg * HCZ_WG_GROUPS + u * 256u + threadIdx.x;
+            if (g < job.groups) body[g] = make_uint4(0u, 0u, 0u, 0u);
+        }
+    }
+}
+
+static bool hcz_add(HczJobs &jobs, uint64_t &blocks, const float *src, void *dst, uint64_t n, uint32_t unit) {
+    if (n == 0) return true;
+    const uint32_t per = 16u / unit;
+    HczJob &j = jobs.j[jobs.count];
+    j.src = src; j.dst = reinterpret_cast<char *>(dst); j.n = n;
+    const uint64_t to_line = ((16u - (uint32_t)(reinterpret_cast<uintptr_t>(dst) & 15u)) & 15u) / unit;
+    j.head = (uint32_t)(to_line < n ? to_line : n);
+    j.groups = (n - j.head) / per;
+    j.src_vec = src && (reinterpret_cast<uintptr_t>(src + j.head) & 15u) == 0 ? 1u : 0u;
+    j.block0 = (uint32_t)blocks;
+    const uint64_t wgs = (j.groups + HCZ_WG_GROUPS - 1) / HCZ_WG_GROUPS;
+    blocks += wgs ? wgs : 1;
+    jobs.count++;
+    return blocks < (1ull << 31);
+}
+
+extern "C" {
+
+int foc_half_copy_zero(const float *src0, void *dst0, uint64_t n0, const float *src1, void *dst1, uint64_t n1, const float *src2, void *dst2, uint64_t n2,
+                       const float *src3, void *dst3, uint64_t n3, void *zero_ptr, uint64_t zero_bytes, void *stream) {
+    const float *srcs[HCZ_MAX_COPIES] = {src0, src1, src2, src3};
+    void *dsts[HCZ_MAX_COPIES] = {dst0, dst1, dst2, dst3};
+    const uint64_t ns[HCZ_MAX_COPIES] = {n0, n1, n2, n3};
+    const void *first = zero_bytes ? zero_ptr : nullptr;
+    for (int i = HCZ_MAX_COPIES - 1; i >= 0; i--) if (ns[i]) first = srcs[i];
+    FocDeviceGuard foc_guard_(stream, first);
+    HczJobs jobs = {};
+    uint64_t blocks = 0;
+    for (int i = 0; i < HCZ_MAX_COPIES; i++) {
+        FOC_REQUIRE(ns[i] == 0 || (srcs[i] && dsts[i]), FOC_E_INVALID, "half_copy_zero: null pointer (conversion %d)", i);
+        FOC_REQUIRE(ns[i] == 0 || ((reinterpret_cast<uintptr_t>(srcs[i]) & 3u) == 0 && (reinterpret_cast<uintptr_t>(dsts[i]) & 1u) == 0), FOC_E_INVALID,
+                    "half_copy_zero: conversion %d: the source must be 4-byte aligned, the destination 2-byte aligned", i);
+        FOC_REQUIRE(hcz_add(jobs, blocks, srcs[i], dsts[i], ns[i], 2), FOC_E_INVALID, "half_copy_zero: too many elements for one launch");
+    }
+    FOC_REQUIRE(zero_bytes == 0 || zero_ptr, FOC_E_INVALID, "half_copy_zero: null pointer (clear)");
+    FOC_REQUIRE(hcz_add(jobs, blocks, nullptr, zero_ptr, zero_bytes, 1), FOC_E_INVALID, "half_copy_zero: too many bytes for one launch");
+    if (jobs.count == 0) return FOC_OK;
+    hipLaunchKernelGGL(k_half_copy_zero, dim3((uint32_t)blocks), dim3(256), 0, (hipStream_t)stream, jobs);
+    FOC_CHECK_LAUNCH("half_copy_zero");
+    return FOC_OK;
+}
+
+}
diff --git a/focnerf_amd/csrc/raymarching.hip b/focnerf_amd/csrc/raymarching.hip
--- a/focnerf_amd/csrc/raymarching.hip
+++ b/focnerf_amd/csrc/raymarching.hip
@@ -8,30 +8,6 @@
 #define RM_RPI   0.3183098861837907f
 
 __device__ __forceinline__ float rm_sign(float x) { return copysignf(1.0f, x); }
-
-__device__ __forceinline__ void rm_near_far(float ox, float oy, float oz, float dx, float dy, float dz, float a0, float a1, float a2, float a3, float a4, float a5,
-                                            float min_near, float &near_out, float &far_out) {
-    const float rdx = 1 / dx, rdy = 1 / dy, rdz = 1 / dz;
-    float near = (a0 - ox) * rdx, far = (a3 - ox) * rdx, t;
-    if (near > far) { t = near; near = far; far = t; }
-    float near_y = (a1 - oy) * rdy, far_y = (a4 - oy) * rdy;
-    if (near_y > far_y) { t = near_y; near_y = far_y; far_y = t; }
-    bool miss = (near > far_y || near_y > far);
-    if (!miss) {
-        if (near_y > near) near = near_y;
-        if (far_y < far) far = far_y;
-        float near_z = (a2 - oz) * rdz, far_z = (a5 - oz) * rdz;
-        if (near_z > far_z) { t = near_z; near_z = far_z; far_z = t; }
-        miss = (near > far_z || near_z > far);
-        if (!miss) {
-            if (near_z > near) near = near_z;
-            if (far_z < far) far = far_z;
-            if (near < min_near) near = min_near;
-        }
-    }
-    near_out = miss ? FLT_MAX : near;
-    far_out = miss ? FLT_MAX : far;
-}
 
 __global__ void __launch_bounds__(256) k_near_far_from_aabb(const float *__restrict__ rays_o, const float *__restrict__ rays_d,
                                      const float *__restrict__ aabb, uint32_t N, float min_near,
diff --git a/focnerf_amd/csrc/sample_math.h b/focnerf_amd/csrc/sample_math.h
--- a/focnerf_amd/csrc/sample_math.h
+++ b/focnerf_amd/csrc/sample_math.h
@@ -1,7 +1,32 @@
 #pragma once
 #include "common.h"
+#include <float.h>
 
 typedef _Float16 h8 __attribute__((ext_vector_type(8)));
+
+__device__ __forceinline__ void rm_near_far(float ox, float oy, float oz, float dx, float dy, float dz, float a0, float a1, float a2, float a3, float a4, float a5,
+                                            float min_near, float &near_out, float &far_out) {
+    const float rdx = 1 / dx, rdy = 1 / dy, rdz = 1 / dz;
+    float near = (a0 - ox) * rdx, far = (a3 - ox) * rdx, t;
+    if (near > far) { t = near; near = far; far = t; }
+    float near_y = (a1 - oy) * rdy, far_y = (a4 - oy) * rdy;
+    if (near_y > far_y) { t = near_y; near_y = far_y; far_y = t; }
+    bool miss = (near > far_y || near_y > far);
+    if (!miss) {
+        if (near_y > near) near = near_y;
+        if (far_y < far) far = far_y;
+        float near_z = (a2 - oz) * rdz, far_z = (a5 - oz) * rdz;
+        if (near_z > far_z) { t = near_z; near_z = far_z; far_z = t; }
+        miss = (near > far_z || near_z > far);
+        if (!miss) {
+            if (near_z > near) near = near_z;
+            if (far_z < far) far = far_z;
+            if (near < min_near) near = min_near;
+        }
+    }
+    near_out = miss ? FLT_MAX : near;
+    far_out = miss ? FLT_MAX : far;
+}
 
 __device__ __forceinline__ void foc_sh16(float x, float y, float z, float (&o)[16]) {
     const float xy = x * y, xz = x * z, yz = y * z, x2 = x * x, y2 = y * y, z2 = z * z;
diff --git a/focnerf_amd/field.py b/focnerf_amd/field.py
--- a/focnerf_amd/field.py
+++ b/focnerf_amd/field.py
@@ -209,7 +209,7 @@
 class _hashgrid_mlp(Function):
     @staticmethod
     @custom_fwd(device_type="cuda")
-    def forward(ctx, x, embeddings, weights, offsets, grid, sigma, training, colour=None):
+    def forward(ctx, x, embeddings, weights, offsets, grid, sigma, training, colour=None, grad_table=None):
         x = x.contiguous().float()
         B = x.shape[0]
         if colour is not None:
@@ -242,6 +242,8 @@
             ctx.save_for_backward(x, emb, w, offsets, enc)
             ctx.cfg = (grid, sigma, B, L)
             ctx.ticket = ticket
+            ctx.grad_table = grad_table if (grad_table is not None and grad_table.dtype == emb.dtype and grad_table.shape == emb.shape
+                                            and grad_table.device == emb.device and grad_table.is_contiguous()) else None
         if c is None:
             return h
         ctx.mark_non_differentiable(c)
@@ -254,16 +256,18 @@
         x, emb, w, offsets, enc = ctx.saved_tensors
         grid, sigma, B, L = ctx.cfg
         if grad_h is None:
-            return (None,) * 8
+            return (None,) * 9
         grad_h = grad_h.contiguous().half()
         g_enc = torch.empty_like(enc)
         g_w = torch.empty_like(w)
         _ffmlp.ffmlp_backward_planar(grad_h, enc, w, B, sigma.input_dim, 16, sigma.hidden_dim, sigma.num_layers, sigma.activation,
                                      sigma.output_activation, True, g_enc, g_w)
-        g_emb = torch.zeros_like(emb)
+        g_emb, ctx.grad_table = getattr(ctx, "grad_table", None), None
+        if g_emb is None:
+            g_emb = torch.zeros_like(emb)
         _gridencoder.grid_encode_backward(g_enc, x, emb, offsets, g_emb, B, 3, 2, L, grid.log2_scale, grid.base_resolution, None, None, *grid.tail(),
                                           grad_bl=False, precount=ctx.ticket)
-        return None, g_emb, g_w, None, None, None, None, None
+        return None, g_emb, g_w, None, None, None, None, None, None
 
 
 @torch.no_grad()
@@ -292,11 +296,11 @@
     return sigma, rgb
 
 
-def hashgrid_mlp(encoder, mlp, x, bound=1, colour=None):
+def hashgrid_mlp(encoder, mlp, x, bound=1, colour=None, grad_table=None):
     prefix = list(x.shape[:-1])
     xn = (x if bound is None else (x + bound) / (2 * bound)).view(-1, 3)
     h = _hashgrid_mlp.apply(xn, encoder.embeddings, mlp.weights, encoder.offsets, encoder.spec(), MlpShape.of(mlp), mlp.training and torch.is_grad_enabled(),
-                            colour)
+                            colour, *(() if grad_table is None else (grad_table,)))
     if colour is not None:
         h, c = h
         return h.view(prefix + [16]), c
diff --git a/focnerf_amd/fixedstep.py b/focnerf_amd/fixedstep.py
--- a/focnerf_amd/fixedstep.py
+++ b/focnerf_amd/fixedstep.py
@@ -30,6 +30,65 @@
     if want_ray_sh:
         return enc_in, xyzs, ray_sh
     return enc_in, xyzs
+
+
+fold_train_launches = True
+
+
+def fixed_sample_train(rays_o, rays_d, aabb, min_near, noise, T, bound):
+    N, dev = rays_o.shape[0], rays_o.device
+    aabb = aabb.contiguous()
+    if aabb.dtype != torch.float32 or rays_o.dtype != torch.float32 or rays_d.dtype != torch.float32:
+        raise RuntimeError("fixed_sample_train: rays and aabb must be float32")
+    nears, fars = torch.empty(N, dtype=torch.float32, device=dev), torch.empty(N, dtype=torch.float32, device=dev)
+    enc_in = torch.empty(N * T, 3, dtype=torch.float32, device=dev)
+    ray_sh = torch.empty(N, 16, dtype=torch.float16, device=dev)
+    check(lib.foc_fixed_sample_train(ptr(rays_o), ptr(rays_d), ptr(aabb), float(min_near), ptr(noise), N, T, float(bound), ptr(nears), ptr(fars),
+                                     ptr(enc_in), ptr(ray_sh), stream_of(rays_o)), "fixed_sample_train")
+    return nears, fars, enc_in, ray_sh
+
+
+class train_prepare:
+
+    def __init__(self, table, blobs):
+        self.table, self.blobs, self.grad_table = table, blobs, None
+
+    def __enter__(self):
+        from . import field
+        self._scope = field.half_cache_scope()
+        self._scope.__enter__()
+        try:
+            self._launch(field)
+        except BaseException:
+            self._scope.__exit__(None, None, None)
+            raise
+        return self
+
+    def __exit__(self, *exc):
+        return self._scope.__exit__(*exc)
+
+    def _launch(self, field):
+        scope = field._half_scope
+        todo = []
+        for p in (self.table,) + tuple(self.blobs):
+            hit = scope.get(id(p))
+            if (p.dtype == torch.float32 and p.is_cuda and p.is_contiguous() and p.numel() > 0 and not (hit is not None and hit[0] is p)
+                    and all(q is not p for q, _ in todo)):
+                todo.append((p, torch.empty(p.shape, dtype=torch.float16, device=p.device)))
+        if not todo or todo[0][0] is not self.table or any(p.device != self.table.device for p, _ in todo):
+            return
+        self.grad_table = todo[0][1].new_empty(todo[0][1].shape)
+        args = []
+        for p, h in todo + [(None, None)] * (4 - len(todo)):
+            args += [ptr(p), ptr(h), p.numel() if p is not None else 0]
+        check(lib.foc_half_copy_zero(*args, ptr(self.grad_table), self.grad_table.numel() * 2, stream_of(self.table)), "half_copy_zero")
+        ev = st = None
+        if self._scope._outer is not None:
+            ev = torch.cuda.Event()
+            ev.record(torch.cuda.current_stream(self.table.device))
+            st = field._raw_stream_of(self.table.device)
+        for p, h in todo:
+            scope[id(p)] = (p, h, ev, st)
 
 
 def ray_sh_rows(rays_d):
@@ -263,7 +322,6 @@
     N, T = rays_o.shape[0], int(num_steps)
     dev = rays_o.device
     aabb = model.aabb_train if model.training else model.aabb_infer
-    nears, fars = raymarching.near_far_from_aabb(rays_o, rays_d, aabb, model.min_near)
     noise = torch.rand(N * T, dtype=torch.float32, device=dev) if perturb else None
     from .field import field_plan, field_infer
     plan = field_plan(model)
@@ -275,8 +333,13 @@
         raise ValueError("render_fixed_steps: distortion=True needs the training route (gradients enabled): the inference paths form no "
                          "differentiable weights; call it under torch.enable_grad() with model.train()")
     rb = ray_block_default() if fused_infer else 0
-    enc_in, _, ray_sh = fixed_sample(rays_o, rays_d, nears, fars, aabb, noise, T, model.bound, want_ray_sh=True) if want_tail else \
-        fixed_sample(rays_o, rays_d, nears, fars, aabb, noise, T, model.bound, ray_block=rb) + (None,)
+    fold = want_tail and fold_train_launches and N > 0 and T >= 2
+    if fold:
+        nears, fars, enc_in, ray_sh = fixed_sample_train(rays_o, rays_d, aabb, model.min_near, noise, T, model.bound)
+    else:
+        nears, fars = raymarching.near_far_from_aabb(rays_o, rays_d, aabb, model.min_near)
+        enc_in, _, ray_sh = fixed_sample(rays_o, rays_d, nears, fars, aabb, noise, T, model.bound, want_ray_sh=True) if want_tail else \
+            fixed_sample(rays_o, rays_d, nears, fars, aabb, noise, T, model.bound, ray_block=rb) + (None,)
 
     if fused_infer:
         obj_feat = model.encode_object_feature(yolo_details, dev) if plan.uses_object_feature else None
@@ -310,7 +373,14 @@
     from .field import hashgrid_mlp, fused_mlp
     c_pre = obj_feat = None
     cweights = fused_mlp(model, "color_net").weights if want_tail else None
-    with torch.autocast("cuda", dtype=torch.float16):
+    import contextlib
+    prep = None
+    if fold and plan.field and plan.train_forward:
+        sn = fused_mlp(model, "sigma_net")
+        if not isinstance(getattr(type(sn), "weights", None), property) and all(isinstance(p, torch.nn.Parameter)
+                                                                                 for p in (enc.embeddings, sn.weights, cweights)):
+            prep = train_prepare(enc.embeddings, (sn.weights, cweights))
+    with (prep if prep is not None else contextlib.nullcontext()), torch.autocast("cuda", dtype=torch.float16):
         if plan.uses_object_feature:
             obj_feat = model.encode_object_feature(yolo_details, dev)
         if plan.field:
@@ -319,7 +389,7 @@
                 from .field import _half_of
                 wc16 = _half_of(cweights)
                 colour = (wc16, plan.colour, ray_sh, T, _C_WIDTH, obj_feat, plan.colour_input_pad)
-            h = hashgrid_mlp(enc, fused_mlp(model, "sigma_net"), enc_in, None, colour)
+            h = hashgrid_mlp(enc, fused_mlp(model, "sigma_net"), enc_in, None, colour, grad_table=prep.grad_table if prep is not None else None)
             if colour is not None:
                 h, c_pre = h
         else:
diff --git a/include/focnerf.h b/include/focnerf.h
--- a/include/focnerf.h
+++ b/include/focnerf.h
@@ -163,6 +163,10 @@
                                    uint32_t L, float S, uint32_t H, uint32_t gridtype, int align_corners,
                                    uint32_t interp, int dtype, const int32_t *offsets_host, void *workspace,
                                    uint64_t workspace_bytes, void *stream);
+int foc_grid_encode_forward_counted_clean(const float *inputs, const void *embeddings, const int32_t *offsets, void *outputs,
+                                          uint32_t B, uint32_t D, uint32_t C, uint32_t L, float S, uint32_t H,
+                                          uint32_t gridtype, int align_corners, uint32_t interp, int dtype,
+                                          const int32_t *offsets_host, void *workspace, uint64_t workspace_bytes, void *stream);
 int foc_grid_encode_backward_binned_counted(const void *grad, const float *inputs, const void *embeddings,
                                             const int32_t *offsets, void *grad_embeddings,
                                             uint32_t B, uint32_t D, uint32_t C, uint32_t L, float S, uint32_t H,
@@ -315,6 +319,10 @@
 int foc_fixed_sample(const float *rays_o, const float *rays_d, const float *nears, const float *fars,
                      const float *aabb, const float *noise, uint32_t N, uint32_t T, float bound,
                      float *xyzs, float *enc_in, void *ray_sh, uint32_t ray_block, void *stream);
+
+int foc_fixed_sample_train(const float *rays_o, const float *rays_d, const float *aabb, float min_near,
+                           const float *noise, uint32_t N, uint32_t T, float bound,
+                           float *nears, float *fars, float *enc_in, void *ray_sh, void *stream);
 
 int foc_fixed_head_forward(const void *h, const float *rays_d, const float *nears, const float *fars,
                            const float *noise, uint32_t N, uint32_t T, float density_scale,
@@ -569,6 +577,10 @@
 size_t foc_optim_workspace_bytes(int n_tensors);
 int foc_optim_step(const FocOptimStep *step, void *stream);
 
+int foc_half_copy_zero(const float *src0, void *dst0, uint64_t n0, const float *src1, void *dst1, uint64_t n1,
+                       const float *src2, void *dst2, uint64_t n2, const float *src3, void *dst3, uint64_t n3,
+                       void *zero_ptr, uint64_t zero_bytes, void *stream);
+
 #define FOC_U8 2
 #define FOC_LOSS_MSE 0
 #define FOC_LOSS_HUBER 1
```

Measured after the change: 1.324 billion (median of 4 runs). About the same (+0.4%).
